# astooke/accel_rl

Measured on AMD Instinct MI355X. Metric: env-steps/sec (whole node), 256-env PPO Atari, higher is better.
Workload: dtype f32; 1 GPU; PPO breakout, 256 envs/GPU, horizon 5, spec-1 CNN (fp32), minibatch 512/GPU x 4 epochs, adam; synthetic fixed-frame emulator; hipGraph rollout; total_envs=256, global_minibatch=512, parallelism=single

## Files before the change

### accel_rl_amd/_build.py

```python
import os
import shutil
import subprocess

PKG_DIR = os.path.dirname(os.path.abspath(__file__))
ROOT = os.path.dirname(PKG_DIR)
CSRC = os.path.join(PKG_DIR, "csrc")
LIB_PATH = os.path.join(PKG_DIR, "libaccel_rl_hip.so")
SOURCES = ["mfma_conv_p1.hip", "mfma_conv_p2.hip", "mfma_conv_p3.hip", "mfma_conv_p4.hip", "mfma_conv_p5.hip", "mfma_conv_p6.hip",
           "mfma_conv_p7.hip", "mfma_conv_p8.hip", "mfma_conv.hip", "img_conv.hip", "batch_ops.hip", "scan.hip", "env.hip", "serve_step.hip", "optim.hip", "learner.hip", "replay.hip",
           "dqn.hip", "lstm.hip", "gru.hip", "noisy.hip", "traj.hip", "handover.hip", "iqn.hip"]
ARCH = "gfx950"


def _flags_stamp():
    return os.path.join(CSRC, "_obj", ".flags")


def _stale():
    if not os.path.exists(LIB_PATH):
        return True
    extra = os.environ.get("ARL_HIPCC_FLAGS", "")
    stamp = _flags_stamp()
    if os.path.exists(stamp) and open(stamp).read().split("||")[-1] != extra:
        return True
    t = os.path.getmtime(LIB_PATH)
    deps = [os.path.join(CSRC, f) for f in os.listdir(CSRC) if f.endswith((".hip", ".h"))]
    deps += [os.path.join(ROOT, "include", h) for h in ("accel_rl_hip.h", "accel_rl_hip_dev.h")]
    return any(os.path.getmtime(d) > t for d in deps)


def build_extension(force=False, verbose=False):
    if not force and not _stale():
        return LIB_PATH
    import fcntl
    lock_path = os.path.join(PKG_DIR, ".build.lock")
    try:
        lock = open(lock_path, "w")
    except PermissionError as e:
        raise RuntimeError("libaccel_rl_hip.so is missing or older than its sources, and %s is not writable: build it "
                           "where the tree can be written (python accel_rl_amd/_build.py)" % PKG_DIR) from e
    with lock:
        fcntl.flock(lock, fcntl.LOCK_EX)
# ... 55 lines not shown
```

### accel_rl_amd/_lib.py

```python
import ctypes as C
import os

import torch

_PKG = os.path.dirname(os.path.abspath(__file__))
LIB_PATH = os.path.join(_PKG, "libaccel_rl_hip.so")

ARL_ABI_VERSION = 4
PROMO_NEP50, PROMO_LEGACY, PROMO_ASSOC = 0, 1, 2
PPO_TIE_THEANO, PPO_TIE_MATH, PPO_TIE_BOTH = 0, 1, 2
OPT_ADAM, OPT_RMSPROP = 0, 1
MAX_ACTIONS = 18
REPLAY_MAX_HORIZON = 16
RAW_H, RAW_W, OBS_H, OBS_W = 210, 160, 104, 80
OPT_PARTIALS = 1024

_vp, _i32, _i64, _f32, _f64 = C.c_void_p, C.c_int32, C.c_int64, C.c_float, C.c_double


class ArlGame(C.Structure):
    _fields_ = [("bank", _vp), ("n_frames", _i32), ("n_actions", _i32),
                ("action_set", _i32 * MAX_ACTIONS), ("start_lives", _i32),
                ("life_period", _i32), ("frame_skip", _i32), ("n_stack", _i32),
                ("clip_reward", _i32), ("episodic_lives", _i32), ("resample_mode", _i32)]
# ... 132 lines not shown
    "arl_pg_head_infer": (_i32, [_vp, _vp, _vp, _i64, _i32, _i32, _vp, _vp, _vp]),
    "arl_pg_head_loss": (_i32, [_vp] * 11 + [_i64, _i32, _i32, _i32, _i32, _f32, _f32, _f32, _i32] + [_vp] * 7),
    "arl_pg_head_loss_parts": (_i32, [_vp] * 11 + [_i64, _i32, _i32, _i32, _i32, _f32, _f32, _f32, _i32] + [_vp] * 7 +
                               [_vp, _i32, _vp]),
    "arl_conv_workspace_bytes": (_i64, []),
    "arl_conv2d_fwd": (_i32, [_vp, _vp, _vp, _vp, C.POINTER(ArlConvGeom), _i32, _vp, _vp]),
    "arl_conv2d_bwd_data": (_i32, [_vp, _vp, _vp, _vp, _vp, C.POINTER(ArlConvGeom), C.POINTER(ArlCorunJob), C.POINTER(_i32), _vp]),
    "arl_conv2d_dgrad_weights": (_i32, [C.POINTER(ArlDgradWt), _i32, _vp]),
    "arl_conv2d_bwd_weight": (_i32, [_vp, _vp, _vp, C.POINTER(ArlConvGeom), _vp, _vp]),
    "arl_conv2d_bwd_weight_parts": (_i32, [_vp, _vp, _vp, C.POINTER(ArlConvGeom), _vp, _i64, C.POINTER(ArlFoldItem),
                                           _vp, C.POINTER(ArlFoldItem), _vp]),
    "arl_fold_many": (_i32, [C.POINTER(ArlFoldItem), _i32, _vp]),
    "arl_conv2d_fwd_parts": (_i32, [_vp, _vp, _vp, _vp, C.POINTER(ArlConvGeom), _i32, _vp, C.POINTER(ArlFoldItem), _vp]),
    "arl_serve_conv1_supported": (_i32, [C.POINTER(ArlGame), C.POINTER(ArlConvGeom)]),
    "arl_rollout_begin_conv1": (_i32, [C.POINTER(ArlGame), C.POINTER(ArlEnvState), C.POINTER(ArlRollout),
                                       C.POINTER(ArlServeConv1), _vp]),
    "arl_env_step_served": (_i32, [C.POINTER(ArlGame), C.POINTER(ArlEnvState), C.POINTER(ArlRollout),
                                   C.POINTER(ArlServeHead), C.POINTER(ArlServeConv1), _vp, _i32, _f64, _f64, _i32, _vp]),
    "arl_conv2d_u8_fwd": (_i32, [_vp, _i64, _vp, _f32, _vp, _vp, _vp, C.POINTER(ArlConvGeom), _i32, _vp]),
    "arl_conv2d_u8_bwd_weight_parts": (_i32, [_vp, _vp, _i64, _vp, _f32, _vp, C.POINTER(ArlConvGeom), _vp, _i64,
                                              C.POINTER(ArlFoldItem), _vp, C.POINTER(ArlFoldItem), _vp]),
    "arl_conv2d_bwd_pair": (_i32, [_vp, _vp, _vp, _vp, _vp, _vp, _vp, C.POINTER(ArlConvGeom), _vp, _i64,
                                   C.POINTER(ArlFoldItem), _vp, C.POINTER(ArlFoldItem), C.POINTER(ArlCorunJob),
                                   C.POINTER(_i32), _vp]),
    "arl_conv2d_bwd_weight_plan": (_i32, [_vp, _vp, _vp, C.POINTER(ArlConvGeom), _vp, _i64, C.POINTER(ArlFoldItem),
                                          _vp, C.POINTER(ArlFoldItem), C.POINTER(ArlWgradPlan)]),
    "arl_conv2d_u8_bwd_weight_plan": (_i32, [_vp, _vp, _i64, _vp, _f32, _vp, C.POINTER(ArlConvGeom), _vp, _i64,
                                             C.POINTER(ArlFoldItem), _vp, C.POINTER(ArlFoldItem),
                                             C.POINTER(ArlWgradPlan)]),
    "arl_conv2d_bwd_pair_plan": (_i32, [_vp, _vp, _vp, _vp, _vp, _vp, _vp, C.POINTER(ArlConvGeom), _vp, _i64,
                                        C.POINTER(ArlFoldItem), _vp, C.POINTER(ArlFoldItem), C.POINTER(ArlCorunJob),
                                        C.POINTER(_i32), C.POINTER(ArlWgradPlan), _vp]),
    "arl_conv2d_bwd_weight_group": (_i32, [C.POINTER(ArlWgradPlan), _i32, _vp]),
    "arl_relu_bwd_bias_parts": (_i32, [_vp, _vp, _i64, _i32, _vp, _vp, C.POINTER(ArlFoldItem), _vp]),
    "arl_replay_append": (_i32, [C.POINTER(ArlReplay), _vp, _vp, _vp, _vp, _i32, _i32, _f64, _i32, _vp]),
    "arl_replay_extract": (_i32, [C.POINTER(ArlReplay), _vp, _vp, _i64, _vp, _vp, _vp, _vp, _vp, _vp]),
    "arl_sumtree_find": (_i32, [_vp, _i32, _vp, _i64, _vp, _vp]),
    "arl_sumtree_add": (_i32, [_vp, _i32, _vp, _vp, _i64, _vp]),
    "arl_sumtree_gather": (_i32, [_vp, _vp, _i64, _f64, _vp, _vp]),
    "arl_sumtree_sample": (_i32, [_vp, _i32, _vp, _i32, _i32, _i32, _vp, _vp, _vp, _vp, _vp, _vp]),
    "arl_sumtree_sample_batch": (_i32, [_vp, _i32, _vp, _i32, _i32, _i32, _vp, _vp, _vp, _vp, _vp, _f64, _vp, _vp, _i32, _vp]),
    "arl_sumtree_update_pow": (_i32, [_vp, _i32, _vp, _vp, _vp, _f64, _i64, _vp]),
    "arl_is_weights": (_i32, [_vp, _i64, _f64, _vp, _vp]),
    "arl_priority_diffs": (_i32, [_vp, _vp, _i64, _f64, _vp, _vp]),
    "arl_catdqn_act": (_i32, [_vp, _vp, _vp, _i64, _i32, _i32, _i32, _i32, _vp, _vp, _vp]),
    "arl_catdqn_loss": (_i32, [_vp] * 8 + [_i64, _i32, _i32, _i32, _i32, _f32, _f32, _f32, _vp, _vp, _vp, _vp]),
    "arl_catdqn_loss_parts": (_i32, [_vp] * 8 + [_i64, _i32, _i32, _i32, _i32, _f32, _f32, _f32, _vp, _vp, _vp, _vp, _i32,
                               _vp]),
    "arl_qrdqn_act": (_i32, [_vp, _vp, _i64, _i32, _i32, _i32, _i32, _vp, _vp, _vp]),
    "arl_qrdqn_loss": (_i32, [_vp] * 7 + [_i64, _i32, _i32, _i32, _i32, _f32, _f32, _vp, _vp, _vp, _vp]),
    "arl_iqn_embed": (_i32, [_vp, _vp, _i64, _i64, _i64, _i32, _vp, _vp, _vp]),
    "arl_iqn_merge_fwd": (_i32, [_vp, _vp, _i64, _i32, _i32, _vp, _vp]),
    "arl_iqn_merge_bwd": (_i32, [_vp, _vp, _vp, _i64, _i32, _i32, _vp, _vp, _vp]),
    "arl_iqn_act": (_i32, [_vp, _vp, _i64, _i32, _i32, _i32, _vp, _vp, _vp, _i64, _vp]),
    "arl_iqn_loss": (_i32, [_vp] * 8 + [_i64, _i32, _i32, _i32, _i32, _f32, _f32, _vp, _vp, _vp, _vp, _i64, _vp]),
    "arl_dqn_act": (_i32, [_vp, _vp, _i64, _i32, _i32, _i32, _vp, _vp, _vp]),
    "arl_dqn_loss": (_i32, [_vp] * 7 + [_i64, _i32, _i32, _i32, _f32, _f32, _vp, _vp, _vp, _vp]),
    "arl_lstm_cell_fwd": (_i32, [_vp, _i64, _vp, _vp, _i64, _i64, _i32, _vp, _i64, _vp, _i64, _vp, _i64, _vp]),
    "arl_lstm_cell_bwd": (_i32, [_vp, _i64, _vp, _vp, _vp, _i64, _vp, _i64, _vp, _i64, _i64, _i32, _vp, _i64, _vp, _vp]),
    "arl_gru_cell_fwd": (_i32, [_vp, _i64, _vp, _vp, _i64, _i64, _i32, _vp, _i64, _vp, _i64, _vp]),
    "arl_gru_cell_bwd": (_i32, [_vp, _i64, _vp, _vp, _vp, _i64, _vp, _i64, _i64, _i32, _vp, _i64, _vp, _i64, _vp, _vp]),
    "arl_rnn_cell_fwd": (_i32, [_vp, _i64, _vp, _i64, _i32, _vp, _i64, _vp]),
    "arl_rnn_cell_bwd": (_i32, [_vp, _i64, _vp, _vp, _i64, _i64, _i32, _vp, _i64, _vp]),
    "arl_seq_handover": (_i32, [_vp, _i64, _vp, _i64, _vp, _vp, _i64, _i64, _i64, _i32, _vp, _vp, _i64, _vp, _i64, _vp]),
    "arl_lstm_cell_bwd_reset": (_i32, [_vp, _i64, _vp, _vp, _vp, _i64, _vp, _i64, _vp, _i64, _i64, _i32, _vp, _i64, _vp,
                                       _vp, _vp, _i64, _i64, _vp]),
# ... 382 lines not shown
    batch, hid = h.shape
    _check(load().arl_pg_head_loss(
        ptr(h), w_head.data_ptr(), b_head.data_ptr(), ptr(actions), ptr(advantages), ptr(returns),
        ptr(old_prob), ptr(valids), ptr(idx), ptr(lr_mult), ptr(inv_count), batch, hid, n_actions,
        kind, int(tie_rule), float(clip_param), float(v_loss_coeff), float(ent_loss_coeff), int(bool(relu_mask_dh)), ptr(dout), ptr(dh),
        dw_head.data_ptr(), db_head.data_ptr(), ptr(loss4), ptr(workspace), stream_ptr(stream)),
        "arl_pg_head_loss")



def conv_geom(batch, in_h, in_w, in_c, out_c, kh, kw, stride, pad_h, pad_w, route=None):
    return ArlConvGeom(batch, in_h, in_w, in_c, out_c, kh, kw, stride, pad_h, pad_w,
                       default_route if route is None else route)


def dense_geom(batch, fan_in, units, route=None):
    return ArlConvGeom(batch, 1, 1, fan_in, units, 1, 1, 1, 0, 0, default_route if route is None else route)


def with_route(geom, route=None):
    g = ArlConvGeom.from_buffer_copy(geom)
    g.route = default_route if route is None else route
    return g


def conv_out_hw(g):
    return ((g.in_h + 2 * g.pad_h - g.kh) // g.stride + 1, (g.in_w + 2 * g.pad_w - g.kw) // g.stride + 1)


def conv_workspace(device):
    return torch.empty(load().arl_conv_workspace_bytes() // 4, dtype=torch.float32, device=device)


def conv2d_fwd(x, w, bias, y, geom, relu, workspace, stream=None):
    for t, n in ((x, "x"), (w, "w"), (y, "y")):
        _want(t, torch.float32, n)
    ho, wo = conv_out_hw(geom)
    assert x.numel() == geom.batch * geom.in_h * geom.in_w * geom.in_c, "x size"
    assert w.numel() == geom.out_c * geom.kh * geom.kw * geom.in_c, "w size"
    assert y.numel() == geom.batch * ho * wo * geom.out_c, "y size"
    _check(load().arl_conv2d_fwd(x.data_ptr(), w.data_ptr(), None if bias is None else bias.data_ptr(),
                                 y.data_ptr(), C.byref(geom), int(bool(relu)), ptr(workspace),
                                 stream_ptr(stream)), "arl_conv2d_fwd")


def conv2d_fwd_parts(x, w, bias, y, geom, relu, workspace, stream=None):
    for t, n in ((x, "x"), (w, "w"), (y, "y")):
        _want(t, torch.float32, n)
    ho, wo = conv_out_hw(geom)
    assert x.numel() == geom.batch * geom.in_h * geom.in_w * geom.in_c, "x size"
    assert w.numel() == geom.out_c * geom.kh * geom.kw * geom.in_c, "w size"
    assert y.numel() == geom.batch * ho * wo * geom.out_c, "y size"
    item = ArlFoldItem()
    _check(load().arl_conv2d_fwd_parts(x.data_ptr(), w.data_ptr(), None if bias is None else bias.data_ptr(),
                                       y.data_ptr(), C.byref(geom), int(bool(relu)), ptr(workspace), C.byref(item),
                                       stream_ptr(stream)), "arl_conv2d_fwd_parts")
    return item


def conv2d_u8_supported(in_h, in_w, out_c, kh, kw, stride, pad_h, pad_w):
    return (pad_h == 0 and pad_w == 0 and stride % 4 == 0 and in_w % 4 == 0 and (in_h * in_w) % 4 == 0 and
            kw in (4, 8, 16) and kh % (16 // kw) == 0 and out_c % 4 == 0 and out_c <= 32)


def _u8_rows(obs, idx, geom):
    _want(obs, torch.uint8, "obs")
    assert obs.is_contiguous() and obs.numel() == obs.shape[0] * geom.in_c * geom.in_h * geom.in_w, "obs shape"
    if idx is not None:
        _want(idx, torch.int32, "idx")
        assert idx.numel() == geom.batch, "idx length"
    else:
        assert obs.shape[0] == geom.batch, "obs rows"


def conv2d_u8_fwd(obs, idx, scale, w, bias, y, geom, relu, stream=None):
    _u8_rows(obs, idx, geom)
    ho, wo = conv_out_hw(geom)
    assert w.numel() == geom.out_c * geom.kh * geom.kw * geom.in_c, "w size"
    assert y.numel() == geom.batch * ho * wo * geom.out_c, "y size"
    _check(load().arl_conv2d_u8_fwd(obs.data_ptr(), obs.shape[0], ptr(idx), float(scale), w.data_ptr(), ptr(bias),
                                    y.data_ptr(), C.byref(geom), int(bool(relu)), stream_ptr(stream)),
           "arl_conv2d_u8_fwd")


def conv2d_dgrad_weights(layers, stream=None):
    assert 0 < len(layers) <= DGRAD_WT_MAX
    items = (ArlDgradWt * len(layers))()
    for it, (w, wt, geom) in zip(items, layers):
        _want(w, torch.float32, "w")
        _want(wt, torch.float32, "wt")
        assert w.numel() == wt.numel() == geom.out_c * geom.kh * geom.kw * geom.in_c, "w / wt size"
        it.w, it.wt, it.geom = ptr(w), ptr(wt), C.pointer(geom)
    _check(load().arl_conv2d_dgrad_weights(items, len(layers), stream_ptr(stream)), "arl_conv2d_dgrad_weights")


def conv2d_bwd_data(dy, w, mask, dx, geom, stream=None, corun=None, wt=None):
    ho, wo = conv_out_hw(geom)
    assert dy.numel() == geom.batch * ho * wo * geom.out_c, "dy size"
    assert dx.numel() == geom.batch * geom.in_h * geom.in_w * geom.in_c, "dx size"
    assert mask is None or mask.numel() == dx.numel()
    taken = _i32(0)
    _check(load().arl_conv2d_bwd_data(dy.data_ptr(), w.data_ptr(), ptr(wt), None if mask is None else mask.data_ptr(),
                                      dx.data_ptr(), C.byref(geom), None if corun is None else C.byref(corun),
                                      C.byref(taken), stream_ptr(stream)), "arl_conv2d_bwd_data")
    return bool(taken.value)


def conv2d_bwd_weight(dy, x, dw, geom, workspace, stream=None):
    ho, wo = conv_out_hw(geom)
    assert dy.numel() == geom.batch * ho * wo * geom.out_c, "dy size"
    assert x.numel() == geom.batch * geom.in_h * geom.in_w * geom.in_c, "x size"
    assert dw.numel() == geom.out_c * geom.kh * geom.kw * geom.in_c, "dw size"
    _check(load().arl_conv2d_bwd_weight(dy.data_ptr(), x.data_ptr(), dw.data_ptr(), C.byref(geom),
                                        ptr(workspace), stream_ptr(stream)), "arl_conv2d_bwd_weight")


class FoldList(object):

    def __init__(self):
        self._items = (ArlFoldItem * FOLD_MAX_ITEMS)()
        self._n = 0
        self._plans = (ArlWgradPlan * WGRAD_GROUP_MAX)()
        self._n_plans = 0
        self.last_dw_in_place = False
        self.corun_taken = False

    def _next(self):
        assert self._n < FOLD_MAX_ITEMS, "too many pending folds"
        self._n += 1
        return C.byref(self._items[self._n - 1])

    def _bias_slot(self, dbias):
        if dbias is None:
            return None, None
# ... 25 lines not shown
        assert dw.numel() == geom.out_c * geom.kh * geom.kw * geom.in_c, "dw size"
        item = self._next()
        pb, ib = self._bias_slot(dbias)
        if defer:
            _check(load().arl_conv2d_bwd_weight_plan(dy.data_ptr(), x.data_ptr(), dw.data_ptr(), C.byref(geom),
                                                     ptr(workspace), workspace.numel() * workspace.element_size(),
                                                     item, pb, ib, self._next_plan(stream)), "arl_conv2d_bwd_weight_plan")
            return self._bias_done(dbias)
        _check(load().arl_conv2d_bwd_weight_parts(dy.data_ptr(), x.data_ptr(), dw.data_ptr(), C.byref(geom),
                                                  ptr(workspace), workspace.numel() * workspace.element_size(),
                                                  item, pb, ib, stream_ptr(stream)), "arl_conv2d_bwd_weight_parts")
        return self._bias_done(dbias)

    def conv2d_u8_bwd_weight(self, dy, obs, idx, scale, dw, geom, workspace, dbias=None, stream=None, defer=False):
        _u8_rows(obs, idx, geom)
        ho, wo = conv_out_hw(geom)
        assert dy.numel() == geom.batch * ho * wo * geom.out_c, "dy size"
        assert dw.numel() == geom.out_c * geom.kh * geom.kw * geom.in_c, "dw size"
        item = self._next()
        pb, ib = self._bias_slot(dbias)
        if defer:
            _check(load().arl_conv2d_u8_bwd_weight_plan(dy.data_ptr(), obs.data_ptr(), obs.shape[0], ptr(idx),
                                                        float(scale), dw.data_ptr(), C.byref(geom), ptr(workspace),
                                                        workspace.numel() * workspace.element_size(), item, pb, ib,
                                                        self._next_plan(stream)), "arl_conv2d_u8_bwd_weight_plan")
            return self._bias_done(dbias)
        _check(load().arl_conv2d_u8_bwd_weight_parts(dy.data_ptr(), obs.data_ptr(), obs.shape[0], ptr(idx),
                                                     float(scale), dw.data_ptr(), C.byref(geom), ptr(workspace),
                                                     workspace.numel() * workspace.element_size(), item, pb, ib,
                                                     stream_ptr(stream)), "arl_conv2d_u8_bwd_weight_parts")
        return self._bias_done(dbias)

    def conv2d_bwd_pair(self, dy, w, mask, dx, x, dw, geom, workspace, dbias=None, stream=None, corun=None, wt=None,
                        defer=False):
        ho, wo = conv_out_hw(geom)
        assert dy.numel() == geom.batch * ho * wo * geom.out_c, "dy size"
        assert x.numel() == dx.numel() == geom.batch * geom.in_h * geom.in_w * geom.in_c, "x / dx size"
        assert dw.numel() == w.numel() == geom.out_c * geom.kh * geom.kw * geom.in_c, "w / dw size"
        item = self._next()
        slot = self._n - 1
        pb, ib = self._bias_slot(dbias)
        taken = _i32(0)
        if defer:
            _check(load().arl_conv2d_bwd_pair_plan(dy.data_ptr(), w.data_ptr(), ptr(wt), ptr(mask), dx.data_ptr(),
                                                   x.data_ptr(), dw.data_ptr(), C.byref(geom), ptr(workspace),
                                                   workspace.numel() * workspace.element_size(), item, pb, ib,
                                                   None if corun is None else C.byref(corun), C.byref(taken),
                                                   self._next_plan(stream), stream_ptr(stream)),
                   "arl_conv2d_bwd_pair_plan")
        else:
            _check(load().arl_conv2d_bwd_pair(dy.data_ptr(), w.data_ptr(), ptr(wt), ptr(mask), dx.data_ptr(), x.data_ptr(),
                                              dw.data_ptr(), C.byref(geom), ptr(workspace),
                                              workspace.numel() * workspace.element_size(), item, pb, ib,
                                              None if corun is None else C.byref(corun), C.byref(taken),
                                              stream_ptr(stream)), "arl_conv2d_bwd_pair")
        self.corun_taken = bool(taken.value)
        self.last_dw_in_place = self._items[slot].splits == 0
        return self._bias_done(dbias)

    def relu_bwd_bias_grad(self, dy, y, rows, channels, dbias, workspace, stream=None):
        _check(load().arl_relu_bwd_bias_parts(dy.data_ptr(), y.data_ptr(), rows, channels, dbias.data_ptr(),
                                              ptr(workspace), self._next(), stream_ptr(stream)),
               "arl_relu_bwd_bias_parts")

    def pg_head_loss(self, h, w_head, b_head, actions, advantages, returns, old_prob, valids, idx, lr_mult,
                     inv_count, n_actions, kind, clip_param, v_loss_coeff, ent_loss_coeff,
                     dout, dh, dw_head, db_head, loss4, workspace, stream=None, relu_mask_dh=False,
                 tie_rule=PPO_TIE_THEANO, dgrad_weights=None):
        batch, hid = h.shape
        assert self._n + 3 <= FOLD_MAX_ITEMS, "too many pending folds"
        first = C.byref(self._items[self._n])
        self._n += 3
        wt_items, n_wt = None, 0
        if dgrad_weights:
            n_wt = len(dgrad_weights)
            assert n_wt <= DGRAD_WT_MAX
# ... 452 lines not shown
```

### accel_rl_amd/csrc/img_conv.hip

```cpp
#include "mfma_conv_impl.h"
#include "img_conv_dev.h"

namespace arlc {

__global__ __launch_bounds__(C1_NT) void conv1_img_kernel(const Conv1ImgArgs a) {
    extern __shared__ __attribute__((aligned(16))) char lds[];
    constexpr int MAXLD = (C1_MAX_IMG / 16 + C1_NT - 1) / C1_NT;
    const int tid = threadIdx.x, lane = tid & 63;
    const int wave = __builtin_amdgcn_readfirstlane(tid >> 6);
    const int half = lane >> 5;
    const int C = a.C, H = a.H, W = a.W, npix = C * H * W, K = C * 64, nsteps = K / 16;
    char* const sW = lds;
    char* const sI = lds + nsteps * 3072;
    const int n16 = npix / 16;
    u32x4 ireg[MAXLD];
    auto img_issue = [&](int img) {
        int row = a.idx ? a.idx[img] : img;
        row = (unsigned)row < (unsigned)a.obs_rows ? row : 0;
        const u32x4* src = reinterpret_cast<const u32x4*>(a.obs + (size_t)row * npix);
#pragma unroll
        for (int i = 0; i < MAXLD; ++i)
            if (tid + C1_NT * i < n16) ireg[i] = src[tid + C1_NT * i];
    };
    auto img_store = [&](int buf, int img) {
// ... 3 lines not shown
            if (tid + C1_NT * i < n16) *reinterpret_cast<u32x4*>(d + (tid + C1_NT * i) * 16) = ireg[i];
        if (a.copy_out) {
            u32x4* o = reinterpret_cast<u32x4*>(a.copy_out + (long long)img * a.copy_stride);
#pragma unroll
            for (int i = 0; i < MAXLD; ++i)
                if (tid + C1_NT * i < n16) o[tid + C1_NT * i] = ireg[i];
        }
    };
    if (a.zero_word && blockIdx.x == 0 && tid == 0) *a.zero_word = 0;
    img_issue(blockIdx.x);
    for (int f = tid; f < nsteps * 64; f += C1_NT) conv1_w_store(sW, f, conv1_w_load(a.w, K, f, a.NF));
    const int rows = a.OH * a.OW, tiles = (rows + 31) / 32;
    float4 bq[4];
    conv1_bias_quads(a.bias, half, bq, a.NF);
    img_store(0, blockIdx.x);
    if (blockIdx.x + gridDim.x < (unsigned)a.n_img) img_issue(blockIdx.x + gridDim.x);
    __syncthreads();
    int buf = 0;
    for (int img = blockIdx.x; img < a.n_img; img += gridDim.x, buf ^= 1) {
        const char* im = sI + buf * npix;
        for (int tp = wave; tp < tiles; tp += C1_NW) conv1_tile(a, im, sW, img, tp, lane, bq);
        if (img + (int)gridDim.x < a.n_img) {
            img_store(buf ^ 1, img + (int)gridDim.x);
            if (img + 2 * (int)gridDim.x < a.n_img) img_issue(img + 2 * gridDim.x);
        }
        __syncthreads();
    }
}

bool g_no_img_kernels = false;

int launch_conv1_img(const unsigned char* obs, int64_t obs_rows, const int32_t* idx, float scale, const float* w, const float* bias, float* y,
                     int64_t batch, int C, int H, int W, int K, int kh, int kw, int stride, int Ho, int Wo, int relu,
                     hipStream_t s, unsigned char* copy_out, long long copy_stride, int* zero_word) {
    const int npix = C * H * W;
    const size_t lds = (size_t)(C * 64 / 16) * 3072 + 2 * (size_t)npix;
    if (g_no_img_kernels || !t_ctx.split || t_ctx.split == 1 || (K != 32 && K != 16) || kh != 8 || kw != 8 || npix % 16 != 0 || npix > C1_MAX_IMG ||
        lds > 160 * 1024 || ((uintptr_t)obs & 15) || (W & 3) || (stride & 3) || batch > 0x7fffffff)
        return -1;
    Conv1ImgArgs a = {obs, idx, w, bias, y, scale, (int)batch, C, H, W, Ho, Wo, stride, relu, K,
                      (int)(obs_rows < 0x7fffffff ? obs_rows : 0x7fffffff), copy_out, copy_stride, zero_word};
    {
        hipError_t e = hipFuncSetAttribute(reinterpret_cast<const void*>(conv1_img_kernel),
                                           hipFuncAttributeMaxDynamicSharedMemorySize, 160 * 1024);
        if (e != hipSuccess) { arl::set_error("hipFuncSetAttribute(conv1_img_kernel): %s", hipGetErrorString(e)); return (int)e; }
    }
    const int cus = 256;
    hipLaunchKernelGGL(conv1_img_kernel, dim3((unsigned)(batch < cus ? batch : cus)), dim3(C1_NT), lds, s, a);
    return arl::check_launch("conv1_img_kernel");
}

int launch_conv1_img_begin(const arl_conv_geom* geom, const unsigned char* obs, int64_t n_img, float scale, const float* w,
                           const float* bias, float* y, int C, int relu, hipStream_t s, unsigned char* copy_out,
                           long long copy_stride, int* zero_word) {
    ARL_ROUTE_SCOPE(geom, nullptr);
    const int st = geom->stride;
    return launch_conv1_img(obs, n_img, nullptr, scale, w, bias, y, n_img, C, geom->in_h, geom->in_w, geom->out_c, geom->kh,
                            geom->kw, st, (geom->in_h - geom->kh) / st + 1, (geom->in_w - geom->kw) / st + 1, relu, s, copy_out,
                            copy_stride, zero_word);
}

}

extern "C" void arl_dev_conv_variant(int32_t v) { arlc::g_no_img_kernels = (v & 1) != 0; }
```

### accel_rl_amd/csrc/img_conv_dev.h

```cpp
#pragma once
#include "mfma_common.h"

namespace arlc {

struct Conv1ImgArgs {
    const unsigned char* obs;
    const int* idx;
    const float* w;
    const float* bias;
    float* y;
    float scale;
    int n_img, C, H, W, OH, OW, stride, relu;
    int NF;
    int obs_rows;
    unsigned char* copy_out;
    long long copy_stride;
    int* zero_word;
};

__device__ __forceinline__ u32x2 bytes_to_bf16x4(unsigned v) {
    const float4 f = bytes_to_f4(v);
    return u32x2{hi_pair(f.x, f.y), hi_pair(f.z, f.w)};
}

struct Conv1WFrag { float4 v0, v1; };
__device__ __forceinline__ Conv1WFrag conv1_w_load(const float* __restrict__ w, const int K, const int f, const int NF = 32) {
    const int s = f >> 6, fl = f & 63;
    if ((fl & 31) >= NF) return Conv1WFrag{make_float4(0.f, 0.f, 0.f, 0.f), make_float4(0.f, 0.f, 0.f, 0.f)};
    const float* src = w + (size_t)(fl & 31) * K + s * 16 + (fl >> 5) * 8;
    return Conv1WFrag{*reinterpret_cast<const float4*>(src), *reinterpret_cast<const float4*>(src + 4)};
}
__device__ __forceinline__ void conv1_w_store(char* sW, const int f, const Conv1WFrag& v) {
    const int s = f >> 6, fl = f & 63;
    unsigned h[4], m[4], l[4];
    split_pair(v.v0.x, v.v0.y, h[0], m[0], l[0]);
    split_pair(v.v0.z, v.v0.w, h[1], m[1], l[1]);
    split_pair(v.v1.x, v.v1.y, h[2], m[2], l[2]);
    split_pair(v.v1.z, v.v1.w, h[3], m[3], l[3]);
    char* d = sW + s * 3072 + fl * 16;
    *reinterpret_cast<u32x4*>(d) = u32x4{h[0], h[1], h[2], h[3]};
    *reinterpret_cast<u32x4*>(d + 1024) = u32x4{m[0], m[1], m[2], m[3]};
    *reinterpret_cast<u32x4*>(d + 2048) = u32x4{l[0], l[1], l[2], l[3]};
}

__device__ __forceinline__ void conv1_bias_quads(const float* __restrict__ bias, const int half, float4 (&bq)[4],
                                                 const int NF = 32) {
#pragma unroll
    for (int q = 0; q < 4; ++q) {
        bq[q] = make_float4(0.f, 0.f, 0.f, 0.f);
        if (bias && 8 * q + 4 * half < NF) bq[q] = *reinterpret_cast<const float4*>(bias + 8 * q + 4 * half);
    }
}

__device__ __forceinline__ void conv1_tile(const Conv1ImgArgs& a, const char* im, const char* sW, const int img,
                                           const int tp, const int lane, const float4 (&bq)[4]) {
    constexpr int KH = 8;
    const int N = a.NF;
    const int l31 = lane & 31, half = lane >> 5;
    const int H = a.H, W = a.W, nsteps = a.C * 64 / 16;
    const int rows = a.OH * a.OW;
    const int m = tp * 32 + l31;
    const int mm = m < rows ? m : 0;
    const int oy = mm / a.OW, ox = mm - oy * a.OW;
    const unsigned off = (unsigned)((oy * a.stride + half) * W + ox * a.stride);
    f32x16 acc;
#pragma unroll
    for (int v = 0; v < 16; ++v) acc[v] = 0.f;
    const char* wl = sW + lane * 16;
#pragma unroll 2
    for (int s = 0; s < nsteps; ++s) {
        const unsigned po = (unsigned)(((s / (KH / 2)) * H + 2 * (s % (KH / 2))) * W);
        u32x4 fb[3];
#pragma unroll
        for (int pl = 0; pl < 3; ++pl) fb[pl] = *reinterpret_cast<const u32x4*>(wl + s * 3072 + pl * 1024);
        const unsigned* q = reinterpret_cast<const unsigned*>(im + po + off);
        const u32x2 lo = bytes_to_bf16x4(q[0]), hi = bytes_to_bf16x4(q[1]);
        const u32x4 fa = u32x4{lo.x, lo.y, hi.x, hi.y};
#pragma unroll
        for (int pl = 2; pl >= 0; --pl) acc = mfma_bf16(fb[pl], fa, acc);
    }
    if (m < rows) {
        float* dst = a.y + ((size_t)img * rows + m) * N + 4 * half;
#pragma unroll
        for (int q = 0; q < 4; ++q) {
            if (8 * q + 4 * half >= N) continue;
            float4 v = make_float4(acc[4 * q] * a.scale + bq[q].x, acc[4 * q + 1] * a.scale + bq[q].y,
                                   acc[4 * q + 2] * a.scale + bq[q].z, acc[4 * q + 3] * a.scale + bq[q].w);
            if (a.relu) { v.x = fmaxf(v.x, 0.f); v.y = fmaxf(v.y, 0.f); v.z = fmaxf(v.z, 0.f); v.w = fmaxf(v.w, 0.f); }
            *reinterpret_cast<float4*>(dst + 8 * q) = v;
        }
    }
}

constexpr int C1_NW = 16, C1_NT = C1_NW * 64, C1_MAX_IMG = 40960;

}
```

### accel_rl_amd/csrc/mfma_common.h

```cpp

#pragma once
#include "arl_optim_dev.h"

#if defined(__HIP_DEVICE_COMPILE__) && !defined(__gfx950__)
#error "accel_rl_amd's MFMA kernels are written for gfx950 (MI355X) only: build with --offload-arch=gfx950"
#endif

#include <stdlib.h>
#include <type_traits>

namespace arlc {

typedef float f32x16 __attribute__((ext_vector_type(16)));
typedef float f32x4 __attribute__((ext_vector_type(4)));

struct GatherDesc {
    const float* src;
    unsigned src_bytes;
    int Hs, Ws, Cs;
    int out_h, out_w;
    int mul, add_y, add_x;
    int taps_x, step;
    int taps_y, rmin, dmin, origin;
    unsigned mg_w, mg_h;
    const unsigned char* src8;
    const int* idx;
    float scale;
    int plane, img_bytes, kh8, kw8;
};

struct WeightDesc {
    const float* w;
    unsigned w_bytes;
    int ld, kc, taps_x, i0, j0, si, kw, c;
    int cls;
};

struct OutDesc {
    float* out;
    const float* bias;
    const float* mask;
    unsigned out_bytes;
    int relu, dense;
    int OH, OW, omul, oadd_y, oadd_x;
};

struct GemmArgs {
    GatherDesc g;
    WeightDesc b;
    OutDesc o;
    int M, N, K;
    int k_per_split;
    int64_t split_stride;
    unsigned long long* trace;
    int n_par;
    int xcd;
    struct Parity {
        int M, out_h, out_w, add_y, add_x, rmin, dmin, origin, i0, j0, oadd_y, oadd_x;
        unsigned src_bytes, mg_w, mg_h;
    } par[4];
};

#define ARL_ARG1(x) asm volatile("" :: "s"(x))
__device__ __forceinline__ void pin_gemm_args(const struct GemmArgs& a);

__device__ __forceinline__ int xcd_chunk(int id, int n) {
    const int q = n >> 3, r = n & 7, x = id & 7, j = id >> 3;
    return (x < r ? x * (q + 1) : r * (q + 1) + (x - r) * q) + j;
}

__device__ __forceinline__ void pin_gemm_args(const GemmArgs& a) {
    asm volatile("" :: "s"(a.g.src), "s"(a.g.src_bytes), "s"(a.g.Hs), "s"(a.g.Ws), "s"(a.g.Cs), "s"(a.g.out_h), "s"(a.g.out_w),
                 "s"(a.g.mul), "s"(a.g.add_y), "s"(a.g.add_x), "s"(a.g.taps_x), "s"(a.g.step), "s"(a.g.taps_y), "s"(a.g.rmin),
                 "s"(a.g.dmin), "s"(a.g.origin), "s"(a.g.mg_w), "s"(a.g.mg_h));
    asm volatile("" :: "s"(a.b.w), "s"(a.b.w_bytes), "s"(a.b.ld), "s"(a.b.kc), "s"(a.b.taps_x), "s"(a.b.i0), "s"(a.b.j0),
                 "s"(a.b.si), "s"(a.b.kw), "s"(a.b.c), "s"(a.b.cls));
    asm volatile("" :: "s"(a.o.out), "s"(a.o.bias), "s"(a.o.mask), "s"(a.o.out_bytes), "s"(a.o.relu), "s"(a.o.dense), "s"(a.o.OH),
// ... 32 lines not shown
                const int rc = i * 32 + (v & 3) + 8 * (v >> 2);
                float val = acc[i][j][v] + bj;
                if (relu) val = fmaxf(val, 0.f);
                if (full || row0 + rc < rows_total)
                    __builtin_amdgcn_raw_buffer_store_b32(__float_as_uint(val), rs, voff, (unsigned)(rc * N) << 2, 0);
            }
    }
}

constexpr unsigned HI16 = 0xffff0000u;
__device__ __forceinline__ unsigned hi_pair(float x0, float x1) {
    return __builtin_amdgcn_perm(__float_as_uint(x1), __float_as_uint(x0), 0x07060302u);
}
__device__ __forceinline__ float lo_part(float x) { return x - __uint_as_float(__float_as_uint(x) & HI16); }
__device__ __forceinline__ void split_pair(float x0, float x1, unsigned& h, unsigned& m, unsigned& l) {
    h = hi_pair(x0, x1);
    const float r0 = lo_part(x0), r1 = lo_part(x1);
    m = hi_pair(r0, r1);
    l = hi_pair(lo_part(r0), lo_part(r1));
}
typedef unsigned int u32x2 __attribute__((ext_vector_type(2)));
typedef __bf16 bf16x2_t __attribute__((ext_vector_type(2)));
typedef float f32x2_t __attribute__((ext_vector_type(2)));
__device__ __forceinline__ unsigned rne_pair(float x0, float x1) {
    const f32x2_t v = {x0, x1};
    return __builtin_bit_cast(unsigned, __builtin_convertvector(v, bf16x2_t));
}
constexpr int planes_of(int split) { return split == 1 ? 1 : 3; }
template <int NP> __device__ __forceinline__ void split_pair_n(float x0, float x1, unsigned& h, unsigned& m, unsigned& l) {
    if constexpr (NP == 1) h = rne_pair(x0, x1);
    else split_pair(x0, x1, h, m, l);
}

template <int TM, int TN, bool SCALED = false>
__device__ __forceinline__ void store_tiles_quads(const f32x16 (&acc)[TM][TN], __amdgpu_buffer_rsrc_t rs,
                                                  const long long (&row_off)[TM], int N, int col_base, int lane,
                                                  const float4 (&bias_q)[TN][4], const float* mask, int relu,
                                                  const float4 (*pre)[TM] = nullptr, float scale = 1.f) {
    const int half = lane >> 5;
#pragma unroll
    for (int j = 0; j < TN; ++j) {
        float4 mk[4][TM];
        if (mask && pre) {
#pragma unroll
            for (int q = 0; q < 4; ++q)
#pragma unroll
                for (int i = 0; i < TM; ++i) mk[q][i] = pre[q][i];
        } else if (mask) {
#pragma unroll
            for (int q = 0; q < 4; ++q)
#pragma unroll
                for (int i = 0; i < TM; ++i) {
                    const int n = col_base + j * 32 + 8 * q + 4 * half;
                    mk[q][i] = make_float4(1.f, 1.f, 1.f, 1.f);
                    if (row_off[i] >= 0 && n < N) mk[q][i] = *reinterpret_cast<const float4*>(mask + row_off[i] + n);
                }
        }
#pragma unroll
        for (int q = 0; q < 4; ++q) {
            const int n = col_base + j * 32 + 8 * q + 4 * half;
            const float4 bq = bias_q[j][q];
#pragma unroll
            for (int i = 0; i < TM; ++i) {
                const bool ok = row_off[i] >= 0 && n < N;
                float4 val = SCALED
                    ? make_float4(acc[i][j][4 * q] * scale + bq.x, acc[i][j][4 * q + 1] * scale + bq.y,
                                  acc[i][j][4 * q + 2] * scale + bq.z, acc[i][j][4 * q + 3] * scale + bq.w)
                    : make_float4(acc[i][j][4 * q] + bq.x, acc[i][j][4 * q + 1] + bq.y,
                                  acc[i][j][4 * q + 2] + bq.z, acc[i][j][4 * q + 3] + bq.w);
                if (relu) { val.x = fmaxf(val.x, 0.f); val.y = fmaxf(val.y, 0.f); val.z = fmaxf(val.z, 0.f); val.w = fmaxf(val.w, 0.f); }
                const unsigned voff = ok ? (unsigned)((row_off[i] + n) << 2) : OOB;
                if (mask) {
                    const float4 m = mk[q][i];
                    if (!(m.x > 0.f)) val.x = 0.f;
                    if (!(m.y > 0.f)) val.y = 0.f;
                    if (!(m.z > 0.f)) val.z = 0.f;
                    if (!(m.w > 0.f)) val.w = 0.f;
                }
                u32x4 raw = {__float_as_uint(val.x), __float_as_uint(val.y), __float_as_uint(val.z), __float_as_uint(val.w)};
                __builtin_amdgcn_raw_buffer_store_b128(raw, rs, voff, 0, 0);
            }
        }
    }
}

struct WgradArgs {
    const float* dy;
    GatherDesc g;
    float* part;
    unsigned dy_bytes;
    int K_out, N, Mred;
    int m_per_split;
    int adv_b, adv_y, adv_x;
    float* bias_part;
    unsigned long long* trace;
    int xcd;
};

__device__ __forceinline__ float4 buf_ld4s(__amdgpu_buffer_rsrc_t rsrc, unsigned voff, unsigned soff) {
    const u32x4 v = __builtin_amdgcn_raw_buffer_load_b128(rsrc, voff, soff, 0);
    return make_float4(__uint_as_float(v.x), __uint_as_float(v.y), __uint_as_float(v.z), __uint_as_float(v.w));
}
__device__ __forceinline__ u32x4 buf_ld4u(__amdgpu_buffer_rsrc_t rsrc, unsigned voff, unsigned soff) {
    return __builtin_amdgcn_raw_buffer_load_b128(rsrc, voff, soff, 0);
}
__device__ __forceinline__ u32x2 buf_ld2s(__amdgpu_buffer_rsrc_t rsrc, unsigned voff, unsigned soff) {
    return __builtin_amdgcn_raw_buffer_load_b64(rsrc, voff, soff, 0);
}
__device__ __forceinline__ unsigned buf_ld1s(__amdgpu_buffer_rsrc_t rsrc, unsigned voff, unsigned soff) {
    return __builtin_amdgcn_raw_buffer_load_b32(rsrc, voff, soff, 0);
}
__device__ __forceinline__ float4 bytes_to_f4(unsigned v) {
    return make_float4((float)(v & 0xffu), (float)((v >> 8) & 0xffu), (float)((v >> 16) & 0xffu), (float)(v >> 24));
// ... 42 lines not shown
```

### accel_rl_amd/csrc/mfma_conv.hip

```cpp
#include "mfma_conv_impl.h"
#include "dgrad_wt_dev.h"

using namespace arlc;

namespace arlc {
thread_local CallCtx t_ctx = {9, nullptr, false};
unsigned long long* g_trace = nullptr;
bool g_force_generic = false;
int g_fwd_tile = -1;
}

namespace {
constexpr int FOLD_WIDE = 128, FOLD_THREADS = 1024;
int g_fold_wide = FOLD_WIDE;
bool g_dgrad_wt = true;

struct FoldSlot { int64_t i; int zg, zgn, row0, o; };
__device__ __forceinline__ FoldSlot fold_slot(int splits, int local_block, int wide_from) {
    FoldSlot f;
    const int tid = threadIdx.x;
    f.o = tid & 15;
    if (splits >= wide_from) { f.zg = tid >> 4; f.zgn = 64; f.row0 = 0; f.i = (int64_t)local_block * 16 + f.o; }
    else {
        const int grp = tid >> 8;
// ... 48 lines not shown
    }
}

struct FoldManyArgs {
    arl_fold_item items[ARL_FOLD_MAX_ITEMS];
    int block_start[ARL_FOLD_MAX_ITEMS + 1];
    int n, wide_from;
};

__global__ __launch_bounds__(FOLD_THREADS) void fold_many_kernel(const FoldManyArgs a) {
    __shared__ float4 lds[64][16];
    int it = 0;
    while (it + 1 < a.n && (int)blockIdx.x >= a.block_start[it + 1]) ++it;
    const float4* part = reinterpret_cast<const float4*>(a.items[it].part);
    float4* out = reinterpret_cast<float4*>(a.items[it].out);
    const int64_t total4 = a.items[it].total >> 2;
    const int splits = a.items[it].splits;
    const FoldSlot f = fold_slot(splits, (int)blockIdx.x - a.block_start[it], a.wide_from);
    const float4 s = fold_sum(part, splits, total4, f, lds);
    const int64_t i = f.i;
    if (f.zg == 0 && i < total4) {
        const int64_t valid = a.items[it].valid;
        if (valid <= 0 || 4 * i + 3 < valid) {
            out[i] = s;
        } else {
            float* o1 = reinterpret_cast<float*>(out + i);
            if (4 * i < valid) o1[0] = s.x;
            if (4 * i + 1 < valid) o1[1] = s.y;
            if (4 * i + 2 < valid) o1[2] = s.z;
        }
    }
}

int launch_fold(const float* part, int splits, int64_t total, const float* bias, int n_bias, int relu,
                float* out, hipStream_t s, const float* mask = nullptr) {
    const int64_t total4 = total >> 2;
    hipLaunchKernelGGL(fold_splits_kernel, dim3((unsigned)fold_blocks(splits, total4)), dim3(FOLD_THREADS), 0, s,
                       (const float4*)part, splits, total4, (const float4*)bias, n_bias >> 2, relu,
                       (const float4*)mask, (float4*)out, g_fold_wide);
    return arl::check_launch("fold_splits_kernel");
}

}

extern "C" int64_t arl_conv_workspace_bytes(void) { return (int64_t)64 << 20; }

extern "C" void arl_dev_conv_trace_buffer(void* device_u64_or_null) { g_trace = (unsigned long long*)device_u64_or_null; }

extern "C" void arl_dev_conv_force_generic(int32_t on) { g_force_generic = on != 0; }

extern "C" void arl_dev_fold_wide_from(int32_t splits) { g_fold_wide = splits > 0 ? splits : FOLD_WIDE; }

extern "C" void arl_dev_fwd_tile(int32_t v) { g_fwd_tile = ((v >= 0 && v <= 2) || v == 6 || v == 7) ? v : -1; }

extern "C" void arl_dev_dgrad_wt(int32_t on) { g_dgrad_wt = on != 0; }

extern "C" int arl_corun_job_init(arl_corun_job* job, const arl_opt_state* opt, int32_t method, float learning_rate,
                                  float avg_factor, float beta1_or_rho, float beta2, float epsilon, int32_t k,
                                  float* step_pp, double* norm_parts, int64_t hole_first, int64_t hole_count) {
    ARL_REQUIRE(job, ARL_E_ARG, "null pointer");
    CorunJob* j = reinterpret_cast<CorunJob*>(job);
    int rc = arl::make_opt_seg(&j->seg, opt, method, learning_rate, avg_factor, beta1_or_rho, beta2, epsilon, k,
                               step_pp, norm_parts, hole_first, hole_count, 1, &j->blocks);
    if (rc) return rc;
    j->host_blocks = 256;
    if (const char* e = getenv("ARL_CORUN_BLOCKS")) j->host_blocks = atoi(e) > 0 ? atoi(e) : 256;
    return 0;
}

extern "C" int arl_corun_job_run(const arl_corun_job* job, void* stream) {
    ARL_REQUIRE(job, ARL_E_ARG, "null pointer");
    const CorunJob* j = reinterpret_cast<const CorunJob*>(job);
    return arl::launch_opt_seg(j->seg, j->blocks, (hipStream_t)stream);
}

namespace {
int fwd_impl(const float* x, const float* w, const float* bias_or_null, float* y, const arl_conv_geom* geom, int32_t relu,
             void* workspace, void* stream, arl_fold_item* parts = nullptr) {
    Geom g;
    int rc = check_geom(geom, &g);
    if (rc) return rc;
    ARL_REQUIRE(x && w && y && workspace, ARL_E_ARG, "null pointer");
    ARL_REQUIRE(arl::aligned16(x) && arl::aligned16(w) && arl::aligned16(y) && arl::aligned16(workspace) &&
                    (!bias_or_null || arl::aligned16(bias_or_null)), ARL_E_ALIGN, "16-byte alignment");
    hipStream_t s = (hipStream_t)stream;
    GemmArgs a = {};
    a.g.src = x; a.g.Hs = g.H; a.g.Ws = g.W; a.g.Cs = g.C; a.g.out_h = g.Ho; a.g.out_w = g.Wo;
    a.g.mul = g.stride; a.g.add_y = -g.pad_h; a.g.add_x = -g.pad_w; a.g.taps_x = g.kw; a.g.step = 1;
    a.M = (int)(g.batch * g.Ho * g.Wo); a.N = g.K; a.K = g.kh * g.kw * g.C;
    a.g.src_bytes = (unsigned)(g.batch * g.H * g.W * g.C * 4);
    a.b.w = w; a.b.ld = a.K; a.b.w_bytes = (unsigned)((int64_t)a.N * a.K * 4);
    a.o.dense = 1; a.trace = g_trace; a.xcd = 1;
    int splits = 1, per = round_up(a.K, BKT);
    const bool small = a.N >= 128 && (int64_t)a.M * a.N <= (int64_t)1 << 20;
    const bool small32 = small && !g_split;
    if (small) plan_split(((a.M + (small32 ? 31 : 63)) / (small32 ? 32 : 64)) * ((a.N + 63) / 64), a.K, &splits, &per, 3 * TARGET_WGS);
    const int tiles128 = ((a.M + 127) / 128) * ((a.N + 127) / 128);
    if (!small && a.N >= 128 && tiles128 * 4 <= TARGET_WGS * 3) plan_split(tiles128, a.K, &splits, &per, TARGET_WGS);
    auto cu_fill = [](int t) { return (double)t / (double)(((t + TARGET_WGS - 1) / TARGET_WGS) * TARGET_WGS); };
    const int tiles64 = ((a.M + 63) / 64) * ((a.N + 63) / 64);
    const bool fill64 = !small && a.N >= 128 && splits == 1 && g_split && g_fwd_tile != 7 &&
                        (g_fwd_tile == 6 || 0.85 * cu_fill(tiles64) > cu_fill(tiles128));
    a.k_per_split = per;
    if (splits > 1) {
        ARL_REQUIRE((int64_t)splits * a.M * a.N * 4 <= arl_conv_workspace_bytes(), ARL_E_RANGE, "workspace too small");
        a.o.out = (float*)workspace; a.split_stride = (int64_t)a.M * a.N;
    } else {
        a.o.out = y; a.o.bias = bias_or_null; a.o.relu = relu;
    }
    constexpr int FBK = 32;
    const bool single_tap = g.C % FBK == 0;
    const bool multi_tap = !single_tap && FBK % g.C == 0 && g.kw % (FBK / g.C) == 0;
    const bool has_pad = g.pad_h > 0 || g.pad_w > 0;
    const bool fast = !g_force_generic && a.K % FBK == 0 && per % FBK == 0 && (single_tap || multi_tap) &&
                      (!has_pad || g.kh * g.kw <= 32) && a.N % 4 == 0;
    if (fast) {
        a.o.out_bytes = (unsigned)((int64_t)a.M * a.N * 4);
        a.g.mg_w = div_magic((int64_t)a.M + 256, a.g.out_w); a.g.mg_h = div_magic((int64_t)a.M + 256, a.g.out_h);
        a.g.taps_y = g.kh; a.g.dmin = 0;
        a.g.rmin = (a.g.add_y * g.W + a.g.add_x) * g.C;
        a.g.origin = a.g.rmin + a.g.dmin;
        a.g.src_bytes = (unsigned)(g.batch * g.H * g.W * g.C * 4 - (int64_t)a.g.origin * 4);
        if (a.N <= 16 && a.K % 16 == 0 && per % 16 == 0 && (g.C % 16 == 0 || (16 % g.C == 0 && g.kw % (16 / g.C) == 0)))
            rc = launch_igemm<4, 1, 2, 1, 16, true, true>(a, splits, multi_tap, has_pad, s);
        else if (g_split && a.N <= 32) rc = launch_igemm_split<4, 1, 1, 1, FBK, true, false, 2>(a, multi_tap, has_pad, s, splits);
        else if (g_split && a.N <= 64) {
            const int v = (g_fwd_tile >= 0 && g_fwd_tile <= 2) ? g_fwd_tile : (2 * ((a.M + 127) / 128) <= TARGET_WGS ? 1 : 0);
            if (v == 1) rc = launch_igemm_split<4, 1, 1, 1, FBK, true, false, 2>(a, multi_tap, has_pad, s, splits);
            else if (v == 2) rc = launch_igemm_split<2, 2, 1, 1, FBK, true, false, 3>(a, multi_tap, has_pad, s, splits);
            else rc = launch_igemm_split<4, 1, 1, 2, FBK, true, false, 2>(a, multi_tap, has_pad, s, splits);
        }
        else if (g_split && (small || fill64)) rc = launch_igemm_split<2, 2, 1, 1, FBK, true, false, 3>(a, multi_tap, has_pad, s, splits);
        else if (g_split) rc = launch_igemm_split<2, 2, 2, 2, FBK, true, false, 1>(a, multi_tap, has_pad, s, splits);
        else if (a.N <= 32 && a.K % 16 == 0 && per % 16 == 0 && (g.C % 16 == 0 || (16 % g.C == 0 && g.kw % (16 / g.C) == 0)))
            rc = launch_igemm<4, 1, 1, 1, 16, true>(a, splits, multi_tap, has_pad, s);
        else if (a.N <= 32) rc = launch_igemm<4, 1, 1, 1, FBK, true>(a, splits, multi_tap, has_pad, s);
        else if (a.N <= 64 && splits == 1) rc = launch_n64<true>(a, multi_tap, has_pad, s);
        else if (a.N <= 64) rc = launch_igemm<2, 2, 1, 1, FBK, true>(a, splits, multi_tap, has_pad, s);
        else if (small32) rc = launch_igemm_occ<1, 4, 2, 1, 32, true, true, 5>(a, multi_tap, has_pad, s, splits);
        else if (small) rc = launch_igemm<2, 2, 1, 1, FBK, true>(a, splits, multi_tap, has_pad, s);
        else rc = launch_igemm<2, 2, 2, 2, FBK, true>(a, splits, multi_tap, has_pad, s);
    } else {
        if (a.N <= 32) rc = launch_rowgather<4, 1, 2, 1, 16, true>(a, splits, s);
        else if (a.N <= 64) rc = launch_rowgather<2, 2, 2, 1, 16, true>(a, splits, s);
        else if (small) rc = launch_rowgather<2, 2, 1, 1, 16, true>(a, splits, s);
        else rc = launch_rowgather<2, 2, 2, 2, 16, true>(a, splits, s);
    }
    if (parts) {
        parts->part = splits == 1 ? y : (const float*)workspace; parts->out = y; parts->total = (int64_t)a.M * a.N;
        parts->splits = splits == 1 ? 0 : splits; parts->valid = 0;
        return rc;
    }
    if (rc || splits == 1) return rc;
    return launch_fold((const float*)workspace, splits, (int64_t)a.M * a.N, bias_or_null, a.N, relu, y, s);
}
}

namespace arlc {
int fold_wide_from() { return g_fold_wide; }
}

extern "C" int arl_conv2d_fwd_parts(const float* x, const float* w, const float* bias_or_null, float* y,
                                    const arl_conv_geom* geom, int32_t relu, void* workspace, arl_fold_item* item,
                                    void* stream) {
    ARL_REQUIRE(item, ARL_E_ARG, "null pointer");
    ARL_ROUTE_SCOPE(geom, nullptr);
    return fwd_impl(x, w, bias_or_null, y, geom, relu, workspace, stream, item);
}

extern "C" int arl_conv2d_fwd(const float* x, const float* w, const float* bias_or_null, float* y,
                              const arl_conv_geom* geom, int32_t relu, void* workspace, void* stream) {
    ARL_ROUTE_SCOPE(geom, nullptr);
    return fwd_impl(x, w, bias_or_null, y, geom, relu, workspace, stream);
}

namespace {
int dgrad_impl(const float* dy, const float* w, const float* mask_or_null, float* dx, const arl_conv_geom* geom,
               DgradPlan* plan_only, void* stream, void* workspace = nullptr, int64_t workspace_bytes = 0,
               const float* wt = nullptr) {
    Geom g;
    int rc = check_geom(geom, &g);
    if (rc) return rc;
    ARL_REQUIRE(dy && w && dx, ARL_E_ARG, "null pointer");
    ARL_REQUIRE(g.kh % g.stride == 0 && g.kw % g.stride == 0, ARL_E_RANGE,
                "data gradient needs kernel size divisible by stride");
    ARL_REQUIRE(arl::aligned16(dy) && arl::aligned16(w) && arl::aligned16(dx) &&
                    (!mask_or_null || arl::aligned16(mask_or_null)) && (!wt || arl::aligned16(wt)), ARL_E_ALIGN,
                "16-byte alignment");
    hipStream_t s = (hipStream_t)stream;
    const int st = g.stride;
    constexpr int FBK = 32;
    const int taps_y = g.kh / st, taps_x = g.kw / st;
    const bool has_pad = !(g.kh == 1 && g.kw == 1 && g.pad_h == 0 && g.pad_w == 0);
    const bool fast = !g_force_generic && g.K % FBK == 0 && taps_y * taps_x <= 32 && st * st <= 4 && g.C % 4 == 0;
    auto describe = [&](int ph, int pw) {
        const int i0 = (ph + g.pad_h) % st, j0 = (pw + g.pad_w) % st;
        GemmArgs a = {};
        a.g.src = dy; a.g.Hs = g.Ho; a.g.Ws = g.Wo; a.g.Cs = g.K;
        a.g.out_h = (g.H - ph + st - 1) / st; a.g.out_w = (g.W - pw + st - 1) / st;
        a.g.mul = 1; a.g.add_y = (ph + g.pad_h - i0) / st; a.g.add_x = (pw + g.pad_w - j0) / st;
        a.g.taps_x = taps_x; a.g.taps_y = taps_y; a.g.step = -1;
        a.M = (int)(g.batch * a.g.out_h * a.g.out_w); a.N = g.C; a.K = taps_y * taps_x * g.K;
        a.g.src_bytes = (unsigned)(g.batch * g.Ho * g.Wo * g.K * 4);
        a.b.w_bytes = (unsigned)((int64_t)g.K * g.kh * g.kw * g.C * 4);
        a.b.w = w; a.b.ld = g.kh * g.kw * g.C; a.b.kc = g.K; a.b.taps_x = taps_x;
        a.b.i0 = i0; a.b.j0 = j0; a.b.si = st; a.b.kw = g.kw; a.b.c = g.C;
        a.o.out = dx; a.o.mask = mask_or_null; a.o.dense = (st == 1);
        a.o.out_bytes = (unsigned)(g.batch * g.H * g.W * g.C * 4);
        a.o.OH = g.H; a.o.OW = g.W; a.o.omul = st; a.o.oadd_y = ph; a.o.oadd_x = pw;
        a.k_per_split = round_up(a.K, BKT);
        a.trace = g_trace; a.xcd = 1;
        if (fast) {
            a.g.rmin = (a.g.add_y * g.Wo + a.g.add_x) * g.K;
            a.g.dmin = -((taps_y - 1) * g.Wo + (taps_x - 1)) * g.K;
            a.g.origin = a.g.rmin + a.g.dmin;
            a.g.src_bytes = (unsigned)(g.batch * g.Ho * g.Wo * g.K * 4 - (int64_t)a.g.origin * 4);
            a.g.mg_w = div_magic((int64_t)a.M + 256, a.g.out_w); a.g.mg_h = div_magic((int64_t)a.M + 256, a.g.out_h);
        }
        return a;
    };
    if (fast) {
        GemmArgs a = describe(0, 0);
        if (st > 1) {
            int n = 0, max_m = 0;
            for (int ph = 0; ph < st && ph < g.H; ++ph)
                for (int pw = 0; pw < st && pw < g.W; ++pw) {
                    const GemmArgs q = describe(ph, pw);
                    GemmArgs::Parity& e = a.par[n++];
                    e.M = q.M; e.out_h = q.g.out_h; e.out_w = q.g.out_w; e.add_y = q.g.add_y; e.add_x = q.g.add_x;
                    e.mg_w = q.g.mg_w; e.mg_h = q.g.mg_h;
                    e.rmin = q.g.rmin; e.dmin = q.g.dmin; e.origin = q.g.origin; e.src_bytes = q.g.src_bytes;
                    e.i0 = q.b.i0; e.j0 = q.b.j0; e.oadd_y = q.o.oadd_y; e.oadd_x = q.o.oadd_x;
                    if (q.M > max_m) max_m = q.M;
                }
            a.n_par = n; a.M = max_m;
            a.xcd = 0;
        }
        const bool small = st == 1 && a.N > 64 && (int64_t)a.M * a.N <= ((int64_t)1 << 20) && a.N % 4 == 0;
        if (plan_only) {
            plan_only->a = a; plan_only->fast = true; plan_only->has_pad = has_pad;
            plan_only->cfg = a.N <= 32 ? 0 : a.N <= 64 ? 1 : small ? 3 : 2;
            return 0;
        }
        if (small) {
            int splits = 1, per = a.k_per_split;
            if (workspace) plan_split(((a.M + 63) / 64) * ((a.N + 63) / 64), a.K, &splits, &per, 3 * TARGET_WGS);
            if ((int64_t)splits * a.M * a.N * 4 > workspace_bytes) { splits = 1; per = round_up(a.K, BKT); }
            a.k_per_split = per;
            if (splits > 1) {
                a.o.out = (float*)workspace; a.o.mask = nullptr; a.split_stride = (int64_t)a.M * a.N;
            }
            if (g_split) rc = launch_igemm_split<2, 2, 1, 1, FBK, false, false, 3>(a, false, has_pad, s, splits);
            else rc = launch_igemm<2, 2, 1, 1, FBK, false>(a, splits, false, has_pad, s);
            if (rc || splits == 1) return rc;
            return launch_fold((const float*)workspace, splits, (int64_t)a.M * a.N, nullptr, 4, 0, dx, s, mask_or_null);
        }
        if (wt && g_split && a.N > 16 && a.N <= 64 && g_dgrad_wt) {
            a.b.w = wt; a.b.ld = a.K; a.b.cls = a.N * a.K;
            const int tiles = ((a.M + 127) / 128) * (a.n_par ? a.n_par : 1);
            const int v = a.N <= 32 || ((g_fwd_tile >= 0 && g_fwd_tile <= 2) ? (g_fwd_tile == 1) : (2 * tiles <= TARGET_WGS));
            if (v) rc = launch_igemm_split<4, 1, 1, 1, FBK, true, false, 2>(a, false, has_pad, s);
            else rc = launch_igemm_split<4, 1, 1, 2, FBK, true, false, 2>(a, false, has_pad, s);
            return rc;
        }
        if (a.N <= 16) rc = launch_igemm<4, 1, 2, 1, 16, false, true>(a, 1, false, has_pad, s);
        else if (g_split && a.N <= 32) rc = launch_igemm_split<4, 1, 1, 1, FBK, false, false, 2>(a, false, has_pad, s);
        else if (g_split && a.N <= 64) {
            const int tiles = ((a.M + 127) / 128) * (a.n_par ? a.n_par : 1);
            const int v = (g_fwd_tile >= 0 && g_fwd_tile <= 2) ? (g_fwd_tile == 1) : (2 * tiles <= TARGET_WGS);
            if (v) rc = launch_igemm_split<4, 1, 1, 1, FBK, false, false, 2>(a, false, has_pad, s);
            else rc = launch_igemm_split<4, 1, 1, 2, FBK, false, false, 2>(a, false, has_pad, s);
        }
        else if (g_split) rc = launch_igemm_split<2, 2, 2, 2, FBK, false, false, 1>(a, false, has_pad, s);
        else if (a.N <= 32 && a.N > 16) rc = launch_igemm_occ<2, 2, 2, 1, 32, false, true, 5>(a, false, has_pad, s);
        else if (a.N <= 32) rc = launch_igemm<4, 1, 1, 1, 16, false>(a, 1, false, has_pad, s);
        else if (a.N <= 64) rc = launch_n64<false>(a, false, has_pad, s);
        else rc = launch_igemm<2, 2, 2, 2, FBK, false>(a, 1, false, has_pad, s);
        return rc;
    }
    if (plan_only) { plan_only->fast = false; return 0; }
    for (int ph = 0; ph < st && ph < g.H; ++ph) {
        for (int pw = 0; pw < st && pw < g.W; ++pw) {
            const GemmArgs a = describe(ph, pw);
            const bool uni = g.K % 16 == 0;
            if (a.N <= 32) rc = uni ? launch_rowgather<4, 1, 2, 1, 16, false, true>(a, 1, s) : launch_rowgather<4, 1, 2, 1, 16, false, false>(a, 1, s);
            else if (a.N <= 64) rc = uni ? launch_rowgather<2, 2, 2, 1, 16, false, true>(a, 1, s) : launch_rowgather<2, 2, 2, 1, 16, false, false>(a, 1, s);
            else rc = uni ? launch_rowgather<2, 2, 2, 2, 16, false, true>(a, 1, s) : launch_rowgather<2, 2, 2, 2, 16, false, false>(a, 1, s);
            if (rc) return rc;
        }
    }
    return 0;
}

int launch_wgrad_plan(const WgradPlan& p, hipStream_t s) {
    constexpr int FBK = 32;
    const WgradArgs& a = p.a;
    const int K = a.K_out, splits = p.splits;
    if (p.kind == WPLAN_U8) {
        if (p.cfg == 1) return launch_wgrad_split<1, 4, 1, 2, FBK, true, 2>(a, splits, false, s);
        if (p.cfg == 2) return launch_wgrad_split<1, 4, 1, 1, FBK, true, 2>(a, splits, false, s);
        const int bm = K <= 16 ? 16 : 32, bn = 128;
        const size_t lds = (size_t)2 * FBK * (bm + bn) * sizeof(float);
        const dim3 grid((a.N + bn - 1) / bn, (K + bm - 1) / bm, splits);
        if (p.cfg == 0) hipLaunchKernelGGL((wgrad_u8_kernel<1, 4, 1, 1, FBK, true>), grid, dim3(256), lds, s, a);
        else hipLaunchKernelGGL((wgrad_u8_kernel<1, 4, 1, 1, FBK, false>), grid, dim3(256), lds, s, a);
        return arl::check_launch("wgrad_u8_kernel");
    }
    if (p.fast) {
        if (K <= 16) return launch_wgrad_fast<1, 4, 1, 1, FBK, true>(a, splits, p.has_pad, s);
        if (g_split && K <= 32) return launch_wgrad_split<1, 4, 1, 1, FBK, false, 2>(a, splits, p.has_pad, s);
        if (g_split && K <= 64) return launch_wgrad_split<2, 2, 1, 1, FBK, false, 2>(a, splits, p.has_pad, s);
        if (g_split) return launch_wgrad_split<2, 2, 2, 2, FBK, false, 1>(a, splits, p.has_pad, s);
        if (K <= 32) return launch_wgrad_fast<1, 4, 1, 1, FBK>(a, splits, p.has_pad, s);
// ... 53 lines not shown
        ARL_REQUIRE((used + (int64_t)splits * a.K_out) * 4 <= workspace_bytes, ARL_E_RANGE, "workspace too small");
        a.bias_part = (float*)workspace + used;
        *bias_part_out = a.bias_part;
    }
    if (fast) {
        a.g.taps_y = g.kh; a.g.dmin = 0;
        a.g.rmin = (a.g.add_y * g.W + a.g.add_x) * g.C;
        a.g.origin = a.g.rmin;
        a.g.src_bytes = (unsigned)(g.batch * g.H * g.W * g.C * 4 - (int64_t)a.g.origin * 4);
        const int img = g.Ho * g.Wo;
        a.adv_b = WG_ROWS / img;
        a.adv_y = (WG_ROWS % img) / g.Wo;
        a.adv_x = (WG_ROWS % img) % g.Wo;
    }
    WgradPlan p = {};
    p.a = a; p.fast = fast; p.has_pad = has_pad; p.cfg = g.K <= 32 ? 0 : g.K <= 64 ? 1 : 2;
    p.splits = splits; p.total = total; p.kind = WPLAN_F32; p.route = g_split;
    *splits_out = splits;
    *total_out = total;
    if (plan_only) { *plan_only = p; return 0; }
    return launch_wgrad_plan(p, s);
}
}

extern "C" int arl_conv2d_bwd_data(const float* dy, const float* w, const float* wt_or_null, const float* mask_or_null,
                                   float* dx, const arl_conv_geom* geom, const arl_corun_job* job_or_null,
                                   int32_t* job_taken_or_null, void* stream) {
    ARL_ROUTE_SCOPE(geom, job_or_null);
    const int rc = dgrad_impl(dy, w, mask_or_null, dx, geom, nullptr, stream, nullptr, 0, wt_or_null);
    if (job_taken_or_null) *job_taken_or_null = t_ctx.corun_taken ? 1 : 0;
    return rc;
}

extern "C" int arl_conv2d_bwd_weight(const float* dy, const float* x, float* dw, const arl_conv_geom* geom,
                                     void* workspace, void* stream) {
    ARL_ROUTE_SCOPE(geom, nullptr);
    int splits = 1;
    int64_t total = 0;
    int rc = wgrad_impl(dy, x, dw, geom, workspace, arl_conv_workspace_bytes(), &splits, &total, nullptr, nullptr, stream);
    if (rc || splits == 1) return rc;
    return launch_fold((const float*)workspace, splits, total, nullptr, 4, 0, dw, (hipStream_t)stream);
}

namespace {
void bias_item(arl_fold_item* item, const float* bias_part, float* dbias, int splits, int channels) {
    item->part = bias_part; item->out = dbias; item->total = channels;
    item->splits = bias_part ? splits : -1;
    item->valid = 0;
}
int wgrad_parts_impl(const float* dy, const float* x, float* dw, const arl_conv_geom* geom,
                     void* workspace, int64_t workspace_bytes, arl_fold_item* item,
                     float* dbias_or_null, arl_fold_item* bias_item_or_null, void* stream,
                     WgradPlan* plan_only = nullptr) {
    ARL_REQUIRE(item && (!dbias_or_null || bias_item_or_null), ARL_E_ARG, "null pointer");
    ARL_REQUIRE(!dbias_or_null || arl::aligned16(dbias_or_null), ARL_E_ALIGN, "16-byte alignment");
    int splits = 1;
    int64_t total = 0;
    float* bias_part = nullptr;
    int rc = wgrad_impl(dy, x, dw, geom, workspace, workspace_bytes, &splits, &total,
                        dbias_or_null ? &bias_part : nullptr, plan_only, stream);
    item->part = (const float*)workspace; item->out = dw; item->total = total;
    item->splits = splits > 1 ? splits : 0;
    item->valid = 0;
    if (dbias_or_null) bias_item(bias_item_or_null, bias_part, dbias_or_null, splits, geom->out_c);
    return rc;
}
// ... 18 lines not shown
                            reinterpret_cast<WgradPlan*>(plan));
}

namespace {
struct U8Geom { int H, W, C, K, kh, kw, stride, Ho, Wo; int64_t batch; };

int check_u8(const uint8_t* obs, int64_t obs_rows, const arl_conv_geom* g, U8Geom* o) {
    ARL_REQUIRE(obs && g && obs_rows > 0, ARL_E_ARG, "null pointer");
    ARL_REQUIRE(g->batch > 0 && g->in_h > 0 && g->in_w > 0 && g->in_c > 0 && g->out_c > 0 && g->kh > 0 && g->kw > 0 &&
                    g->stride > 0, ARL_E_ARG, "conv: bad geometry");
    const int cpr = g->kw / 4;
    ARL_REQUIRE(g->pad_h == 0 && g->pad_w == 0 && g->stride % 4 == 0 && g->in_w % 4 == 0 &&
                    (g->in_h * g->in_w) % 4 == 0 && (g->kw == 4 || g->kw == 8 || g->kw == 16) && g->kh % (4 / cpr) == 0 &&
                    g->out_c % 4 == 0 && g->out_c <= 32 && ((uintptr_t)obs & 3) == 0,
                ARL_E_RANGE, "u8 conv: needs pad 0, stride % 4 == 0, width % 4 == 0, kw in {4, 8, 16}, <= 32 filters");
    o->H = g->in_h; o->W = g->in_w; o->C = g->in_c; o->K = g->out_c; o->kh = g->kh; o->kw = g->kw; o->stride = g->stride;
    o->Ho = (g->in_h - g->kh) / g->stride + 1; o->Wo = (g->in_w - g->kw) / g->stride + 1; o->batch = g->batch;
    const int64_t lim = (int64_t)OOB / 4;
    ARL_REQUIRE(o->Ho > 0 && o->Wo > 0 && g->batch * (int64_t)o->Ho * o->Wo * g->out_c < lim &&
                    obs_rows * (int64_t)g->in_c * g->in_h * g->in_w < (int64_t)OOB,
                ARL_E_RANGE, "conv: tensor larger than the 32-bit buffer offsets address");
    return 0;
}

void fill_u8(GatherDesc* d, const uint8_t* obs, int64_t obs_rows, const int32_t* idx, float scale, const U8Geom& g) {
    d->src8 = obs; d->idx = idx; d->scale = scale;
    d->plane = g.H * g.W; d->img_bytes = g.C * g.H * g.W; d->kh8 = g.kh; d->kw8 = g.kw;
    d->src_bytes = (unsigned)(obs_rows * d->img_bytes);
    d->Hs = g.H; d->Ws = g.W; d->Cs = 1; d->out_h = g.Ho; d->out_w = g.Wo;
    d->mul = g.stride; d->add_y = 0; d->add_x = 0; d->taps_x = g.kw; d->taps_y = g.kh; d->step = 1;
}
}

extern "C" int arl_conv2d_u8_fwd(const uint8_t* obs, int64_t obs_rows, const int32_t* idx_or_null, float scale,
                                 const float* w, const float* bias_or_null, float* y, const arl_conv_geom* geom,
                                 int32_t relu, void* stream) {
    ARL_REQUIRE(w && y, ARL_E_ARG, "null pointer");
    U8Geom g;
    int rc = check_u8(obs, obs_rows, geom, &g);
    if (rc) return rc;
    ARL_ROUTE_SCOPE(geom, nullptr);
    ARL_REQUIRE(arl::aligned16(w) && arl::aligned16(y) && (!bias_or_null || arl::aligned16(bias_or_null)), ARL_E_ALIGN,
                "16-byte alignment");
    if (!g_trace) {
        rc = launch_conv1_img(obs, obs_rows, idx_or_null, scale, w, bias_or_null, y, g.batch, g.C, g.H, g.W, g.K, g.kh, g.kw, g.stride,
                              g.Ho, g.Wo, relu, (hipStream_t)stream);
        if (rc >= 0) return rc;
    }
    GemmArgs a = {};
    fill_u8(&a.g, obs, obs_rows, idx_or_null, scale, g);
    a.M = (int)(g.batch * g.Ho * g.Wo); a.N = g.K; a.K = g.C * g.kh * g.kw;
    a.b.w = w; a.b.ld = a.K; a.b.w_bytes = (unsigned)((int64_t)a.N * a.K * 4);
    a.o.dense = 1; a.o.out = y; a.o.bias = bias_or_null; a.o.relu = relu;
    a.o.out_bytes = (unsigned)((int64_t)a.M * a.N * 4);
    a.k_per_split = a.K;
    a.g.mg_w = div_magic((int64_t)a.M + 256, a.g.out_w); a.g.mg_h = div_magic((int64_t)a.M + 256, a.g.out_h);
    a.trace = g_trace; a.xcd = 1;
    constexpr int BK = 16, BM = 128;
    const dim3 grid((a.M + BM - 1) / BM, 1, 1);
    if (a.N <= 16) {
        const size_t lds = (size_t)2 * (BM * (BK + 4) + 16 * (BK + 4)) * sizeof(float);
        hipLaunchKernelGGL((igemm_u8_kernel<4, 1, 2, 1, BK, true>), grid, dim3(256), lds, (hipStream_t)stream, a);
    } else if (g_split && g.kh % (8 / (g.kw >> 2)) == 0) {
        return launch_igemm_split<4, 1, 2, 1, 32, true, true, 2>(a, false, false, (hipStream_t)stream);
    } else if (g.kh % (8 / (g.kw >> 2)) == 0) {
        constexpr int PBM = 64, PBK = 32;
        const dim3 pgrid((a.M + PBM - 1) / PBM, 1, 1);
        const arl::OptSeg none = {};
        const size_t lds = (size_t)2 * (PBM * (PBK + 4) + 32 * (PBK + 4)) * sizeof(float);
        hipLaunchKernelGGL((igemm_occ_kernel<2, 2, 2, 1, PBK, true, false, false, true, 5, false, true>), pgrid, dim3(256),
                           lds, (hipStream_t)stream, a, none);
        return arl::check_launch("igemm_occ_kernel (u8)");
    } else {
        const size_t lds = (size_t)2 * (BM * (BK + 4) + 32 * (BK + 4)) * sizeof(float);
        hipLaunchKernelGGL((igemm_u8_kernel<4, 1, 1, 1, BK, false>), grid, dim3(256), lds, (hipStream_t)stream, a);
    }
    return arl::check_launch("igemm_u8_kernel");
}

namespace {
int wgrad_u8_impl(const float* dy, const uint8_t* obs, int64_t obs_rows, const int32_t* idx_or_null, float scale, float* dw,
                  const arl_conv_geom* geom, void* workspace, int64_t workspace_bytes, arl_fold_item* item,
                  float* dbias_or_null, arl_fold_item* bias_item_or_null, WgradPlan* plan_only, void* stream) {
    ARL_REQUIRE(dy && dw && workspace && item && (!dbias_or_null || bias_item_or_null), ARL_E_ARG, "null pointer");
    U8Geom g;
    int rc = check_u8(obs, obs_rows, geom, &g);
    if (rc) return rc;
    ARL_ROUTE_SCOPE(geom, nullptr);
    ARL_REQUIRE(arl::aligned16(dy) && arl::aligned16(dw) && arl::aligned16(workspace) &&
                    (!dbias_or_null || arl::aligned16(dbias_or_null)), ARL_E_ALIGN, "16-byte alignment");
    WgradArgs a = {};
    a.dy = dy;
    fill_u8(&a.g, obs, obs_rows, idx_or_null, scale, g);
    a.K_out = g.K; a.N = g.C * g.kh * g.kw; a.Mred = (int)(g.batch * g.Ho * g.Wo);
    a.dy_bytes = (unsigned)((int64_t)a.Mred * g.K * 4);
    a.trace = g_trace; a.xcd = 1;
    const bool wide = g.K > 16 && g_split && g.kw % 8 == 0 && a.N % 256 == 0;
    const int bm = g.K <= 16 ? 16 : 32, bn = wide ? 256 : 128;
    const int tiles = ((a.K_out + bm - 1) / bm) * ((a.N + bn - 1) / bn);
    int splits, per;
    plan_split(tiles, a.Mred, &splits, &per, (g.K <= 16 ? 4 : 2) * TARGET_WGS);
    a.m_per_split = per;
    const int64_t total = (int64_t)a.K_out * a.N;
    const int64_t used = splits > 1 ? (int64_t)splits * total : 0;
    ARL_REQUIRE((used + (int64_t)splits * a.K_out) * 4 <= workspace_bytes, ARL_E_RANGE, "workspace too small");
    a.part = splits > 1 ? (float*)workspace : dw;
    if (dbias_or_null) a.bias_part = (float*)workspace + used;
    const int img = g.Ho * g.Wo;
    a.adv_b = WG_ROWS / img; a.adv_y = (WG_ROWS % img) / g.Wo; a.adv_x = (WG_ROWS % img) % g.Wo;
    WgradPlan p = {};
// ... 4 lines not shown
    item->splits = splits > 1 ? splits : 0;
    item->valid = 0;
    if (dbias_or_null) bias_item(bias_item_or_null, a.bias_part, dbias_or_null, splits, g.K);
    if (plan_only) { *plan_only = p; return 0; }
    return launch_wgrad_plan(p, (hipStream_t)stream);
}
}

extern "C" int arl_conv2d_u8_bwd_weight_parts(const float* dy, const uint8_t* obs, int64_t obs_rows,
                                              const int32_t* idx_or_null, float scale, float* dw,
                                              const arl_conv_geom* geom, void* workspace, int64_t workspace_bytes,
                                              arl_fold_item* item, float* dbias_or_null,
                                              arl_fold_item* bias_item_or_null, void* stream) {
    return wgrad_u8_impl(dy, obs, obs_rows, idx_or_null, scale, dw, geom, workspace, workspace_bytes, item, dbias_or_null,
                         bias_item_or_null, nullptr, stream);
}

extern "C" int arl_conv2d_u8_bwd_weight_plan(const float* dy, const uint8_t* obs, int64_t obs_rows,
                                             const int32_t* idx_or_null, float scale, float* dw,
                                             const arl_conv_geom* geom, void* workspace, int64_t workspace_bytes,
                                             arl_fold_item* item, float* dbias_or_null,
                                             arl_fold_item* bias_item_or_null, arl_wgrad_plan* plan) {
    ARL_REQUIRE(plan, ARL_E_ARG, "null pointer");
    *plan = arl_wgrad_plan{};
    return wgrad_u8_impl(dy, obs, obs_rows, idx_or_null, scale, dw, geom, workspace, workspace_bytes, item, dbias_or_null,
                         bias_item_or_null, reinterpret_cast<WgradPlan*>(plan), nullptr);
}


namespace {
int pair_impl(const float* dy, const float* w, const float* wt_or_null, const float* mask_or_null, float* dx, const float* x,
              float* dw, const arl_conv_geom* geom, void* workspace, int64_t workspace_bytes, arl_fold_item* item,
              float* dbias_or_null, arl_fold_item* bias_item_or_null, const arl_corun_job* job_or_null,
              int32_t* job_taken_or_null, WgradPlan* defer, void* stream) {
    ARL_REQUIRE(item && geom && (!dbias_or_null || bias_item_or_null), ARL_E_ARG, "null pointer");
    if (job_taken_or_null) *job_taken_or_null = 0;
    ARL_ROUTE_SCOPE(geom, job_or_null);
    ARL_REQUIRE(!dbias_or_null || arl::aligned16(dbias_or_null), ARL_E_ALIGN, "16-byte alignment");
    DgradPlan dp = {};
    WgradPlan wp = {};
    int splits = 1;
    int64_t total = 0;
    float* bias_part = nullptr;
    int rc = dgrad_impl(dy, w, mask_or_null, dx, geom, &dp, stream);
    if (rc) return rc;
    rc = wgrad_impl(dy, x, dw, geom, workspace, workspace_bytes, &splits, &total,
                    dbias_or_null ? &bias_part : nullptr, &wp, stream);
    if (rc) return rc;
    const bool has_pad = dp.has_pad || wp.has_pad;
    const int64_t dgrad_tiles = (int64_t)((dp.a.M + 127) / 128) * ((dp.a.N + 127) / 128) * (dp.a.n_par ? dp.a.n_par : 1);
    const bool paired = dp.fast && wp.fast && dp.cfg == 2 && wp.cfg == 2 && dgrad_tiles <= 2 * TARGET_WGS &&
                        (!has_pad || geom->kh * geom->kw <= 32) && !g_trace;
    if (!paired) {
        const int64_t half = (workspace_bytes / 2) & ~(int64_t)15;
        rc = dgrad_impl(dy, w, mask_or_null, dx, geom, nullptr, stream, (char*)workspace + half, workspace_bytes - half,
                        wt_or_null);
        if (job_taken_or_null) *job_taken_or_null = t_ctx.corun_taken ? 1 : 0;
        if (rc) return rc;
        return wgrad_parts_impl(dy, x, dw, geom, workspace, half, item, dbias_or_null, bias_item_or_null, stream, defer);
    }
    hipStream_t s = (hipStream_t)stream;
    if (g_split) rc = launch_pair<2, 2, 2, 2, 2, 2, 2, 2, 16>(dp, wp, has_pad, s);
    else rc = launch_pair<2, 2, 2, 2, 2, 2, 2, 2>(dp, wp, has_pad, s);
    item->part = (const float*)workspace; item->out = dw; item->total = wp.total;
    item->splits = wp.splits > 1 ? wp.splits : 0;
    item->valid = 0;
    if (dbias_or_null) bias_item(bias_item_or_null, bias_part, dbias_or_null, wp.splits, geom->out_c);
    return rc;
}
}

extern "C" int arl_conv2d_bwd_pair(const float* dy, const float* w, const float* wt_or_null, const float* mask_or_null,
                                   float* dx, const float* x, float* dw, const arl_conv_geom* geom, void* workspace,
                                   int64_t workspace_bytes, arl_fold_item* item, float* dbias_or_null,
                                   arl_fold_item* bias_item_or_null, const arl_corun_job* job_or_null,
                                   int32_t* job_taken_or_null, void* stream) {
    return pair_impl(dy, w, wt_or_null, mask_or_null, dx, x, dw, geom, workspace, workspace_bytes, item, dbias_or_null,
                     bias_item_or_null, job_or_null, job_taken_or_null, nullptr, stream);
}

extern "C" int arl_conv2d_bwd_pair_plan(const float* dy, const float* w, const float* wt_or_null, const float* mask_or_null,
                                        float* dx, const float* x, float* dw, const arl_conv_geom* geom, void* workspace,
                                        int64_t workspace_bytes, arl_fold_item* item, float* dbias_or_null,
                                        arl_fold_item* bias_item_or_null, const arl_corun_job* job_or_null,
                                        int32_t* job_taken_or_null, arl_wgrad_plan* plan, void* stream) {
    ARL_REQUIRE(plan, ARL_E_ARG, "null pointer");
    *plan = arl_wgrad_plan{};
    return pair_impl(dy, w, wt_or_null, mask_or_null, dx, x, dw, geom, workspace, workspace_bytes, item, dbias_or_null,
                     bias_item_or_null, job_or_null, job_taken_or_null, reinterpret_cast<WgradPlan*>(plan), stream);
}

extern "C" int arl_conv2d_bwd_weight_group(const arl_wgrad_plan* plans, int32_t n, void* stream) {
    ARL_REQUIRE(plans || n == 0, ARL_E_ARG, "null pointer");
    ARL_REQUIRE(n >= 0 && n <= ARL_WGRAD_GROUP_MAX, ARL_E_RANGE, "0 .. ARL_WGRAD_GROUP_MAX plans");
    hipStream_t s = (hipStream_t)stream;
    const WgradPlan* pl[ARL_WGRAD_GROUP_MAX];
    for (int i = 0; i < n; ++i) pl[i] = reinterpret_cast<const WgradPlan*>(&plans[i]);
    auto body_of = [](const WgradPlan& p) {
        if (!p.route || g_trace) return -1;
        if (p.kind == WPLAN_U8) return p.cfg == 1 ? 2 : p.cfg == 2 ? 3 : -1;
        return p.kind == WPLAN_F32 && p.fast && p.cfg == 1 ? (p.has_pad ? 1 : 0) : -1;
    };
    int route = 0, n_el = 0, el[ARL_WGRAD_GROUP_MAX];
    for (int i = 0; i < n; ++i) {
        if (pl[i]->kind != WPLAN_F32 && pl[i]->kind != WPLAN_U8) continue;
        if (body_of(*pl[i]) >= 0 && !route) route = pl[i]->route;
        if (body_of(*pl[i]) >= 0 && pl[i]->route == route) el[n_el++] = i;
    }
    for (int i = 0; i < n; ++i) {
        if (pl[i]->kind != WPLAN_F32 && pl[i]->kind != WPLAN_U8) continue;
        bool grouped = false;
        for (int k = 0; k < n_el; ++k) grouped = grouped || el[k] == i;
        if (grouped && n_el > 1) continue;
        const CallScope scope(pl[i]->route);
        const int rc = launch_wgrad_plan(*pl[i], s);
        if (rc) return rc;
    }
    if (n_el < 2) return 0;
    for (int i = 1; i < n_el; ++i)
        for (int k = i; k > 0 && group_blocks(*pl[el[k]]) > group_blocks(*pl[el[k - 1]]); --k) std::swap(el[k], el[k - 1]);
    WgradGroupArgs g = {};
    size_t lds = 0;
// ... 87 lines not shown
```

### accel_rl_amd/csrc/mfma_dispatch.h

```cpp
#pragma once
#include "mfma_generic.h"
#include "mfma_igemm.h"
#include "mfma_wgrad.h"
#include "mfma_pair.h"

namespace arlc {

template <int WGM, int WGN, int TM, int TN, int BK, bool B_KC, bool TAP_UNIFORM = false>
int launch_rowgather(const GemmArgs& a, int splits, hipStream_t s) {
    constexpr int BM = WGM * TM * 32, BN = WGN * TN * 32;
    constexpr int A_SZ = BM * (BK + 4), B_SZ = B_KC ? BN * (BK + 4) : BK * BN;
    const size_t lds = (size_t)2 * (A_SZ + B_SZ) * sizeof(float);
    dim3 grid((a.M + BM - 1) / BM, (a.N + BN - 1) / BN, splits);
    hipLaunchKernelGGL((rowgather_gemm_kernel<WGM, WGN, TM, TN, BK, B_KC, TAP_UNIFORM>), grid, dim3(256), lds, s, a);
    return arl::check_launch("rowgather_gemm_kernel");
}

template <int WGM, int WGN, int TM, int TN, int BK>
int launch_wgrad(const WgradArgs& a, int splits, hipStream_t s) {
    constexpr int BM = WGM * TM * 32, BN = WGN * TN * 32;
    const size_t lds = (size_t)2 * BK * (BM + BN) * sizeof(float);
    dim3 grid((a.N + BN - 1) / BN, (a.K_out + BM - 1) / BM, splits);
    hipLaunchKernelGGL((wgrad_kernel<WGM, WGN, TM, TN, BK>), grid, dim3(256), lds, s, a);
    return arl::check_launch("wgrad_kernel");
// ... 60 lines not shown
}

template <int WGM, int WGN, int TM, int TN, int BK, bool B_KC, bool N16, int MINW>
int launch_igemm_occ(const GemmArgs& a, bool multi_tap, bool has_pad, hipStream_t s, int splits = 1) {
    constexpr int BM = WGM * TM * (N16 ? 16 : 32), BN = N16 ? WGN * 16 : WGN * TN * 32;
    constexpr int A_SZ = BM * (BK + 4), B_SZ = B_KC ? BN * (BK + 4) : BK * (N16 ? BN + 4 : BN);
    const size_t lds = (size_t)2 * (A_SZ + B_SZ) * sizeof(float);
    static_assert(lds_fits(2 * (A_SZ + B_SZ)), "<= 64 KiB of LDS");
    dim3 grid((a.M + BM - 1) / BM, (a.N + BN - 1) / BN, a.n_par ? a.n_par : splits);
    arl::OptSeg c = {};
    if constexpr (!B_KC) {
        if (!multi_tap && corun_take(&c, &grid)) {
            if (has_pad) hipLaunchKernelGGL((igemm_occ_kernel<WGM, WGN, TM, TN, BK, B_KC, false, true, N16, MINW, true>), grid, dim3(256), lds, s, a, c);
            else hipLaunchKernelGGL((igemm_occ_kernel<WGM, WGN, TM, TN, BK, B_KC, false, false, N16, MINW, true>), grid, dim3(256), lds, s, a, c);
            return arl::check_launch("igemm_occ_kernel (co-run)");
        }
    }
#define ARL_IGEMM_OCC(MT, HP) \
    hipLaunchKernelGGL((igemm_occ_kernel<WGM, WGN, TM, TN, BK, B_KC, MT, HP, N16, MINW>), grid, dim3(256), lds, s, a, c)
    if (multi_tap && has_pad) ARL_IGEMM_OCC(true, true);
    else if (multi_tap) ARL_IGEMM_OCC(true, false);
    else if (has_pad) ARL_IGEMM_OCC(false, true);
    else ARL_IGEMM_OCC(false, false);
#undef ARL_IGEMM_OCC
    return arl::check_launch("igemm_occ_kernel");
}

#ifdef ARL_NO_SPLIT6
#define ARL_BY_MODE(X1, X6, X9) do { X9; } while (0)
#else
#define ARL_BY_MODE(X1, X6, X9) do { if (g_split == 1) { X1; } else if (g_split == 6) { X6; } else { X9; } } while (0)
#endif

template <int WGM, int WGN, int TM, int TN, int BK, bool B_KC, bool U8, int MINW>
int launch_igemm_split(const GemmArgs& a, bool multi_tap, bool has_pad, hipStream_t s, int splits = 1) {
    constexpr int BM = WGM * TM * 32, BN = WGN * TN * 32;
    const int npl = planes_of(g_split);
    const size_t lds = (size_t)2 * ((U8 ? 1 : npl) * BM + npl * BN) * BK * 2;
    const size_t lds_dir = (size_t)2 * npl * BN * BK * 2;
    (void)lds_dir;
    dim3 grid((a.M + BM - 1) / BM, (a.N + BN - 1) / BN, a.n_par ? a.n_par : splits);
    arl::OptSeg c = {};
    int rc = 0;
#define ARL_SPLIT_K(MT, HP, SPL, CO, AD)                                                                   \
    do {                                                                                                   \
        auto k = igemm_split_kernel<WGM, WGN, TM, TN, BK, B_KC, MT, HP, U8, SPL, MINW, CO, AD>;            \
        const size_t lds_k = (AD) ? lds_dir : lds;                                                         \
        rc = allow_big_lds(k, lds_k + (CO ? 64 : 0));                                                      \
        if (!rc) hipLaunchKernelGGL(k, grid, dim3(256), lds_k, s, a, c);                                   \
    } while (0)
#define ARL_SPLIT_PIN(MT, HP, SPL, CO)                                                                     \
    do {                                                                                                   \
        constexpr bool AD = WGN == 1 && (U8 || !(MT));                                                     \
        ARL_SPLIT_K(MT, HP, SPL, CO, AD);                                                                  \
    } while (0)
#define ARL_SPLIT_MODE(MT, HP, CO)                                                                         \
    do {                                                                                                   \
        ARL_BY_MODE(ARL_SPLIT_PIN(MT, HP, 1, CO), ARL_SPLIT_PIN(MT, HP, 6, CO), ARL_SPLIT_PIN(MT, HP, 9, CO));                           \
    } while (0)
    if constexpr (U8) {
        ARL_SPLIT_MODE(false, false, false);
    } else {
        if constexpr (!B_KC || (WGM == 4 && WGN == 1 && TM == 1)) {
            if (!multi_tap && corun_take(&c, &grid)) {
                if (has_pad) ARL_SPLIT_MODE(false, true, true); else ARL_SPLIT_MODE(false, false, true);
                return rc ? rc : arl::check_launch("igemm_split_kernel (co-run)");
            }
        }
        if (multi_tap && has_pad) ARL_SPLIT_MODE(true, true, false);
        else if (multi_tap) ARL_SPLIT_MODE(true, false, false);
        else if (has_pad) ARL_SPLIT_MODE(false, true, false);
        else ARL_SPLIT_MODE(false, false, false);
    }
#undef ARL_SPLIT_PIN
#undef ARL_SPLIT_MODE
#undef ARL_SPLIT_K
    return rc ? rc : arl::check_launch("igemm_split_kernel");
}

template <int WGM, int WGN, int TM, int TN, int BK, bool M16 = false>
int launch_wgrad_fast(const WgradArgs& a, int splits, bool has_pad, hipStream_t s) {
    constexpr int BM = M16 ? 16 : WGM * TM * 32, BN = WGN * TN * 32;
    const size_t lds = (size_t)2 * BK * (BM + BN) * sizeof(float);
    dim3 grid((a.N + BN - 1) / BN, (a.K_out + BM - 1) / BM, splits);
    int rc;
    if (has_pad) {
        auto k = wgrad_fast_kernel<WGM, WGN, TM, TN, BK, true, M16>;
        rc = allow_big_lds(k, lds + 4096);
        if (!rc) hipLaunchKernelGGL(k, grid, dim3(256), lds, s, a);
    } else {
        auto k = wgrad_fast_kernel<WGM, WGN, TM, TN, BK, false, M16>;
        rc = allow_big_lds(k, lds + 4096);
        if (!rc) hipLaunchKernelGGL(k, grid, dim3(256), lds, s, a);
    }
    return rc ? rc : arl::check_launch("wgrad_fast_kernel");
}

template <int WGM, int WGN, int TM, int TN, int BK, bool U8, int MINW>
int launch_wgrad_split(const WgradArgs& a, int splits, bool has_pad, hipStream_t s) {
    constexpr int BM = WGM * TM * 32, BN = WGN * TN * 32;
    const int npl = planes_of(g_split);
    const size_t lds = (size_t)2 * (npl * BM + (U8 ? 1 : npl) * BN) * BK * 2;
    dim3 grid((a.N + BN - 1) / BN, (a.K_out + BM - 1) / BM, splits);
    int rc = 0;
#define ARL_WSPLIT(HP, SPL)                                                                                \
// ... 44 lines not shown
        g->batch * (int64_t)g->in_h * g->in_w * g->in_c >= lim ||
        (int64_t)g->out_c * g->kh * g->kw * g->in_c >= lim) {
        arl::set_error("conv: tensor larger than the 2 GiB the 32-bit buffer offsets address");
        return ARL_E_RANGE;
    }
    return 0;
}

inline int round_up(int x, int q) { return (x + q - 1) / q * q; }

inline unsigned div_magic(int64_t rows, int d) {
    if (d <= 1 || rows * (int64_t)d >= ((int64_t)1 << 32)) return 0;
    return (unsigned)((((uint64_t)1 << 32) + (uint64_t)d - 1) / (uint64_t)d);
}

template <bool B_KC>
int launch_n64(const GemmArgs& a, bool multi_tap, bool has_pad, hipStream_t s) {
    return launch_igemm_occ<1, 4, 2, 1, 32, B_KC, true, 5>(a, multi_tap, has_pad, s);
}

inline void plan_split(int tiles, int red, int* splits, int* per, int want = TARGET_WGS) {
    int s = tiles >= want ? 1 : want / tiles;
    const int max_s = (red + 4 * BKT - 1) / (4 * BKT);
    if (s > max_s) s = max_s;
    if (s < 1) s = 1;
    *per = round_up((red + s - 1) / s, BKT);
    *splits = (red + *per - 1) / *per;
}

struct DgradPlan { GemmArgs a; bool fast, has_pad; int cfg; };
constexpr int WPLAN_F32 = 1, WPLAN_U8 = 2;
struct WgradPlan { WgradArgs a; bool fast, has_pad; int cfg, splits; int64_t total; int kind, route; };

template <int DWGM, int DWGN, int DTM, int DTN, int WWGM, int WWGN, int WTM, int WTN, int BK = 32>
int launch_pair(const DgradPlan& d, const WgradPlan& w, bool has_pad, hipStream_t s) {
    constexpr int DBM = DWGM * DTM * 32, DBN = DWGN * DTN * 32, WBM = WWGM * WTM * 32, WBN = WWGN * WTN * 32;
    const size_t lds_d = (size_t)2 * (DBM * (BK + 4) + BK * DBN) * sizeof(float);
    const size_t lds_w = (size_t)2 * BK * (WBM + WBN) * sizeof(float);
    const size_t lds = lds_d > lds_w ? lds_d : lds_w;
    const int dgx = (d.a.M + DBM - 1) / DBM, dgy = (d.a.N + DBN - 1) / DBN, dgz = d.a.n_par ? d.a.n_par : 1;
    const int wgx = (w.a.N + WBN - 1) / WBN, wgy = (w.a.K_out + WBM - 1) / WBM, wgz = w.splits;
    const int n_ig = dgx * dgy * dgz, n_wg = wgx * wgy * wgz;
    int rc;
    if (g_split) {
        const size_t lds_s = (size_t)2 * planes_of(g_split) * ((DBM + DBN) > (WBM + WBN) ? (DBM + DBN) : (WBM + WBN)) * BK * 2;
#define ARL_PSPLIT(HP, SPL)                                                                                \
    do {                                                                                                   \
        auto k = bwd_pair_kernel<DWGM, DWGN, DTM, DTN, WWGM, WWGN, WTM, WTN, BK, HP, SPL>;                 \
        rc = allow_big_lds(k, lds_s + 4096);                                                               \
        if (!rc) hipLaunchKernelGGL(k, dim3(n_ig + n_wg), dim3(256), lds_s, s, d.a, w.a, dgx, dgy, n_ig, wgx, wgy); \
    } while (0)
        if (has_pad) ARL_BY_MODE(ARL_PSPLIT(true, 1), ARL_PSPLIT(true, 6), ARL_PSPLIT(true, 9));
        else ARL_BY_MODE(ARL_PSPLIT(false, 1), ARL_PSPLIT(false, 6), ARL_PSPLIT(false, 9));
#undef ARL_PSPLIT
    } else if (has_pad) {
        auto k = bwd_pair_kernel<DWGM, DWGN, DTM, DTN, WWGM, WWGN, WTM, WTN, BK, true>;
        rc = allow_big_lds(k, lds + 4096);
        if (!rc) hipLaunchKernelGGL(k, dim3(n_ig + n_wg), dim3(256), lds, s, d.a, w.a, dgx, dgy, n_ig, wgx, wgy);
    } else {
        auto k = bwd_pair_kernel<DWGM, DWGN, DTM, DTN, WWGM, WWGN, WTM, WTN, BK, false>;
        rc = allow_big_lds(k, lds + 4096);
        if (!rc) hipLaunchKernelGGL(k, dim3(n_ig + n_wg), dim3(256), lds, s, d.a, w.a, dgx, dgy, n_ig, wgx, wgy);
    }
    return rc ? rc : arl::check_launch("bwd_pair_kernel");
}


int launch_conv1_img(const unsigned char* obs, int64_t obs_rows, const int32_t* idx, float scale, const float* w, const float* bias, float* y,
                     int64_t batch, int C, int H, int W, int K, int kh, int kw, int stride, int Ho, int Wo, int relu,
                     hipStream_t s, unsigned char* copy_out = nullptr, long long copy_stride = 0, int* zero_word = nullptr);

#define ARL_GA const GemmArgs&, bool, bool, hipStream_t, int
#define ARL_P1(T) \
    T int launch_igemm_split<4, 1, 2, 1, 32, true, true, 2>(ARL_GA); \
    T int launch_igemm_split<4, 1, 1, 2, 32, true, false, 2>(ARL_GA); \
    T int launch_igemm_split<4, 1, 1, 1, 32, true, false, 2>(ARL_GA);
#define ARL_P2(T) \
    T int launch_igemm_split<2, 2, 2, 2, 32, true, false, 1>(ARL_GA); \
    T int launch_igemm_split<2, 2, 1, 1, 32, true, false, 3>(ARL_GA); \
    T int launch_igemm_split<2, 2, 1, 1, 32, false, false, 3>(ARL_GA);
#define ARL_P3(T) \
    T int launch_igemm_split<4, 1, 1, 2, 32, false, false, 2>(ARL_GA); \
    T int launch_igemm_split<4, 1, 1, 1, 32, false, false, 2>(ARL_GA); \
    T int launch_igemm_split<2, 2, 2, 2, 32, false, false, 1>(ARL_GA);
#define ARL_P4(T) \
    T int launch_wgrad_split<2, 2, 2, 2, 32, false, 1>(const WgradArgs&, int, bool, hipStream_t); \
    T int launch_wgrad_split<2, 2, 1, 1, 32, false, 2>(const WgradArgs&, int, bool, hipStream_t); \
    T int launch_wgrad_split<1, 4, 1, 1, 32, false, 2>(const WgradArgs&, int, bool, hipStream_t); \
    T int launch_wgrad_split<1, 4, 1, 1, 32, true, 2>(const WgradArgs&, int, bool, hipStream_t); \
    T int launch_wgrad_split<1, 4, 1, 2, 32, true, 2>(const WgradArgs&, int, bool, hipStream_t);
#define ARL_P5(T) \
    T int launch_pair<2, 2, 2, 2, 2, 2, 2, 2, 32>(const DgradPlan&, const WgradPlan&, bool, hipStream_t); \
    T int launch_pair<2, 2, 2, 2, 2, 2, 2, 2, 16>(const DgradPlan&, const WgradPlan&, bool, hipStream_t);
#define ARL_P6(T) \
    T int launch_igemm<2, 2, 1, 1, 32, true, false>(const GemmArgs&, int, bool, bool, hipStream_t); \
    T int launch_igemm<2, 2, 1, 1, 32, false, false>(const GemmArgs&, int, bool, bool, hipStream_t); \
    T int launch_igemm<2, 2, 2, 2, 32, true, false>(const GemmArgs&, int, bool, bool, hipStream_t); \
    T int launch_igemm<2, 2, 2, 2, 32, false, false>(const GemmArgs&, int, bool, bool, hipStream_t); \
    T int launch_igemm<4, 1, 2, 1, 16, true, true>(const GemmArgs&, int, bool, bool, hipStream_t); \
    T int launch_igemm<4, 1, 2, 1, 16, false, true>(const GemmArgs&, int, bool, bool, hipStream_t); \
    T int launch_igemm<4, 1, 1, 1, 32, true, false>(const GemmArgs&, int, bool, bool, hipStream_t); \
    T int launch_igemm<4, 1, 1, 1, 16, true, false>(const GemmArgs&, int, bool, bool, hipStream_t); \
    T int launch_igemm<4, 1, 1, 1, 16, false, false>(const GemmArgs&, int, bool, bool, hipStream_t);
#define ARL_P7(T) \
    T int launch_igemm_occ<2, 2, 2, 1, 32, false, true, 5>(ARL_GA); \
    T int launch_igemm_occ<1, 4, 2, 1, 32, true, true, 5>(ARL_GA); \
    T int launch_igemm_occ<1, 4, 2, 1, 32, false, true, 5>(ARL_GA); \
    T int launch_wgrad_fast<2, 2, 2, 2, 32, false>(const WgradArgs&, int, bool, hipStream_t); \
    T int launch_wgrad_fast<2, 2, 1, 1, 32, false>(const WgradArgs&, int, bool, hipStream_t); \
    T int launch_wgrad_fast<1, 4, 1, 1, 32, false>(const WgradArgs&, int, bool, hipStream_t); \
    T int launch_wgrad_fast<1, 4, 1, 1, 32, true>(const WgradArgs&, int, bool, hipStream_t);
#ifndef ARL_CONV_PART
#define ARL_CONV_PART 0
#endif
int launch_wgrad_group(const WgradGroupArgs& g, int groups, size_t lds, hipStream_t s);
#if ARL_CONV_PART == 8
int launch_wgrad_group(const WgradGroupArgs& g, int groups, size_t lds, hipStream_t s) {
    int rc = 0;
#define ARL_WGROUP(SPL)                                                                                    \
    do {                                                                                                   \
        auto k = wgrad_group_kernel<SPL>;                                                                  \
        rc = allow_big_lds(k, lds + 4096);                                                                 \
        if (!rc) hipLaunchKernelGGL(k, dim3((unsigned)groups * 8), dim3(256), lds, s, g);                  \
    } while (0)
    ARL_BY_MODE(ARL_WGROUP(1), ARL_WGROUP(6), ARL_WGROUP(9));
#undef ARL_WGROUP
    return rc ? rc : arl::check_launch("wgrad_group_kernel");
}
#endif
#define ARL_T_DEF template
#define ARL_T_EXT extern template
#if ARL_CONV_PART == 1
ARL_P1(ARL_T_DEF)
#else
ARL_P1(ARL_T_EXT)
#endif
#if ARL_CONV_PART == 2
ARL_P2(ARL_T_DEF)
#else
ARL_P2(ARL_T_EXT)
#endif
#if ARL_CONV_PART == 3
ARL_P3(ARL_T_DEF)
#else
ARL_P3(ARL_T_EXT)
#endif
#if ARL_CONV_PART == 4
ARL_P4(ARL_T_DEF)
#else
ARL_P4(ARL_T_EXT)
#endif
#if ARL_CONV_PART == 5
ARL_P5(ARL_T_DEF)
#else
ARL_P5(ARL_T_EXT)
#endif
#if ARL_CONV_PART == 6
ARL_P6(ARL_T_DEF)
#else
ARL_P6(ARL_T_EXT)
#endif
#if ARL_CONV_PART == 7
ARL_P7(ARL_T_DEF)
#else
ARL_P7(ARL_T_EXT)
#endif

}
```

### accel_rl_amd/csrc/mfma_igemm.h

```cpp
#pragma once
#include "mfma_common.h"

namespace arlc {

template <int WGM, int WGN, int TM, int TN, int BK, bool B_KC, bool MULTI_TAP, bool HAS_PAD, bool N16 = false,
          bool U8 = false, int SPLIT = 0, bool ADIR = false>
__device__ __forceinline__ void igemm_body(const GemmArgs& a, const int bx, const int by, const int bz, float* smem) {
    constexpr bool SP = SPLIT != 0;
    static_assert(!ADIR || (SP && WGN == 1 && !MULTI_TAP), "direct operand: split kernels, one wave per row tile");
    constexpr int MT = N16 ? 16 : 32;
    constexpr int BM = WGM * TM * MT, BN = N16 ? WGN * 16 : WGN * TN * 32, CH = BK / 4;
    constexpr int LDA = BK + 4;
    constexpr int LDB = B_KC ? BK + 4 : (N16 ? BN + 4 : BN);
    static_assert(!N16 || (TN == 1 && BK % 16 == 0), "16-wide tiles: one column tile per wave");
    static_assert(!SP || (!N16 && BK % 16 == 0), "split products: 32-wide tiles, two LDS stages");
    constexpr int ROWS_PER_PASS = 256 / CH;
    constexpr int RA = (BM + ROWS_PER_PASS - 1) / ROWS_PER_PASS;
    constexpr int A_SZ = BM * LDA, B_SZ = B_KC ? BN * LDB : BK * LDB;
    constexpr int NST = 2;
    constexpr int NB4 = B_KC ? BN * CH : BK * BN / 4;
    constexpr int NPAIR = (BK / 2) * (BN / 4);
    constexpr int RB = (SP && !B_KC) ? 2 * ((NPAIR + 255) / 256) : (NB4 + 255) / 256;
    static_assert(WGM * WGN == 4 && BK % 8 == 0, "tile shape");
    float* sA = smem;
    float* sB = smem + NST * A_SZ;
    constexpr int PA = U8 ? 1 : planes_of(SPLIT), PB = planes_of(SPLIT), ROWB = BK * 2, NS = BK / 8;
    constexpr int LPA = ADIR ? 0 : PA;
    constexpr int SPA = BM * ROWB, SPB = BN * ROWB, STAGE = LPA * SPA + PB * SPB;
    char* const sS = reinterpret_cast<char*>(smem);

    const int tid = threadIdx.x, lane = tid & 63, wave = tid >> 6;
    const int wm = wave / WGN, wn = wave % WGN;
    const int l31 = lane & 31, half = lane >> 5;
    const int m0 = bx * BM, n0 = by * BN;
    GatherDesc g = a.g;
    int M = a.M, w_i0 = a.b.i0, w_j0 = a.b.j0, oadd_y = a.o.oadd_y, oadd_x = a.o.oadd_x;
    if (a.n_par) {
        const GemmArgs::Parity& q = a.par[bz];
        M = q.M; g.out_h = q.out_h; g.out_w = q.out_w; g.add_y = q.add_y; g.add_x = q.add_x;
        g.mg_w = q.mg_w; g.mg_h = q.mg_h;
        g.rmin = q.rmin; g.dmin = q.dmin; g.origin = q.origin; g.src_bytes = q.src_bytes;
        w_i0 = q.i0; w_j0 = q.j0; oadd_y = q.oadd_y; oadd_x = q.oadd_x;
        if (m0 >= M) return;
    }
    const int kbeg = a.n_par ? 0 : bz * a.k_per_split;
    const int kend = (kbeg + a.k_per_split < a.K) ? kbeg + a.k_per_split : a.K;
    const int Cs = g.Cs, taps_x = g.taps_x, Ws = g.Ws, step = g.step;
// ... 299 lines not shown
#pragma unroll
            for (int v = 0; v < 16; ++v) acc[i][j][v] = 0.f;
#pragma unroll
        for (int v = 0; v < 4; ++v) acc16[i][v] = 0.f;
    }

    float4 bias_q[TN][4];
#pragma unroll
    for (int j = 0; j < TN; ++j)
#pragma unroll
        for (int q = 0; q < 4; ++q) {
            const int n = N16 ? n0 + wn * 16 + 4 * quad : n0 + wn * TN * 32 + j * 32 + 8 * q + 4 * half;
            bias_q[j][q] = make_float4(0.f, 0.f, 0.f, 0.f);
            if (a.o.bias && n < a.N && (!N16 || q == 0)) bias_q[j][q] = *reinterpret_cast<const float4*>(a.o.bias + n);
        }
    long long row_off[TM];
    auto decode_out_rows = [&]() {
#pragma unroll
        for (int i = 0; i < TM; ++i) {
            const int m = m0 + (wm * TM + i) * MT + (N16 ? l15 : l31);
            if (a.o.dense) {
                row_off[i] = m < M ? (long long)m * a.N : -1;
            } else {
                const int t = div_u(m, g.out_w, g.mg_w), ox = m - t * g.out_w;
                const int b = div_u(t, g.out_h, g.mg_h), oy = t - b * g.out_h;
                row_off[i] = m < M ? ((long long)(b * a.o.OH + oy * a.o.omul + oadd_y) * a.o.OW + ox * a.o.omul + oadd_x) * a.N
                                   : -1;
            }
        }
    };
    constexpr bool PRE_MASK = TN == 1 && TM <= 2;
    if (PRE_MASK) decode_out_rows();
    float4 mk_pre[4][TM];
    auto issue_mask_loads = [&]() {
        if (!(PRE_MASK && a.o.mask)) return;
#pragma unroll
        for (int q = 0; q < (N16 ? 1 : 4); ++q)
#pragma unroll
            for (int i = 0; i < TM; ++i) {
                const int n = N16 ? n0 + wn * 16 + 4 * quad : n0 + wn * TN * 32 + 8 * q + 4 * half;
                mk_pre[q][i] = make_float4(1.f, 1.f, 1.f, 1.f);
                if (row_off[i] >= 0 && n < a.N) mk_pre[q][i] = *reinterpret_cast<const float4*>(a.o.mask + row_off[i] + n);
            }
    };
    const int nk = (kend - kbeg) / BK;
    constexpr int STEPS = (N16 || SP) ? BK / 16 : BK / 8;
    auto mfma_steps = [&](auto buf_c, auto lo_c, auto hi_c) {
        constexpr int buf = decltype(buf_c)::value, LO = decltype(lo_c)::value, HI = decltype(hi_c)::value;
        if constexpr (SP) {
            const char* cA = sS + buf * STAGE + (wm * TM * 32) * ROWB + l31 * ROWB;
            const char* cB = sS + buf * STAGE + LPA * SPA + (B_KC ? (wn * TN * 32) * ROWB + l31 * ROWB
                                                                  : (half * 4 * BN + wn * TN * 32 + l31) * 4);
            const int swz = kc_swz<NS>(l31);
#pragma unroll
            for (int ks = LO; ks < HI; ++ks) {
                const int slot = ((2 * ks + half) ^ swz) << 4;
                u32x4 fa[TM][3], fb[TN][3];
#pragma unroll
                for (int i = 0; i < TM; ++i)
#pragma unroll
                    for (int pl = 0; pl < PA; ++pl) {
                        if constexpr (ADIR) fa[i][pl] = fd_[buf][i][ks][pl];
                        else fa[i][pl] = *reinterpret_cast<const u32x4*>(cA + pl * SPA + i * 32 * ROWB + slot);
                    }
#pragma unroll
                for (int j = 0; j < TN; ++j)
#pragma unroll
// ... 167 lines not shown
            k_tile(C1{}, kt + 1);
        }
    }
    }

    if (a.trace) tr2 = __builtin_readcyclecounter();
    float* out = a.o.out + (a.n_par ? 0 : (int64_t)bz * a.split_stride);
    {
        const __amdgpu_buffer_rsrc_t rsO = make_rsrc(out, a.o.out_bytes);
        if (!PRE_MASK) decode_out_rows();
        if constexpr (N16) {
            const int n = n0 + wn * 16 + 4 * quad;
            const float4 bq = bias_q[0][0];
#pragma unroll
            for (int i = 0; i < TM; ++i) {
                const bool ok = row_off[i] >= 0 && n < a.N;
                float4 val = U8 ? make_float4(acc16[i][0] * g.scale + bq.x, acc16[i][1] * g.scale + bq.y,
                                              acc16[i][2] * g.scale + bq.z, acc16[i][3] * g.scale + bq.w)
                                : make_float4(acc16[i][0] + bq.x, acc16[i][1] + bq.y, acc16[i][2] + bq.z, acc16[i][3] + bq.w);
                if (a.o.relu) { val.x = fmaxf(val.x, 0.f); val.y = fmaxf(val.y, 0.f); val.z = fmaxf(val.z, 0.f); val.w = fmaxf(val.w, 0.f); }
                if (a.o.mask) {
                    float4 mk = make_float4(1.f, 1.f, 1.f, 1.f);
                    if (PRE_MASK) mk = mk_pre[0][i < TM ? i : 0];
                    else if (ok) mk = *reinterpret_cast<const float4*>(a.o.mask + row_off[i] + n);
                    if (!(mk.x > 0.f)) val.x = 0.f;
                    if (!(mk.y > 0.f)) val.y = 0.f;
                    if (!(mk.z > 0.f)) val.z = 0.f;
                    if (!(mk.w > 0.f)) val.w = 0.f;
                }
                u32x4 raw = {__float_as_uint(val.x), __float_as_uint(val.y), __float_as_uint(val.z), __float_as_uint(val.w)};
                __builtin_amdgcn_raw_buffer_store_b128(raw, rsO, ok ? (unsigned)((row_off[i] + n) << 2) : OOB, 0, 0);
            }
        } else {
            store_tiles_quads<TM, TN, U8>(acc, rsO, row_off, a.N, n0 + wn * TN * 32, lane, bias_q, a.o.mask, a.o.relu,
                                          PRE_MASK ? mk_pre : nullptr, g.scale);
        }
    }
    if (a.trace && tid == 0) {
        unsigned long long* t = a.trace + ((size_t)(bz * gridDim.y + by) * gridDim.x + bx) * 8;
        t[0] = tr0; t[1] = tr1; t[2] = tr2; t[3] = __builtin_readcyclecounter();
        t[4] = rt0; t[5] = __builtin_amdgcn_s_memrealtime();
#ifdef ARL_PROLOGUE_STAMPS
        if constexpr (SP) { t[6] = st_a; t[7] = st_b; }
        else
#endif
        {
        t[6] = __builtin_amdgcn_s_getreg((31 << 11) | 4);
        t[7] = __builtin_amdgcn_s_getreg((31 << 11) | 20);
        }
    }
}

template <int WGM, int WGN, int TM, int TN, int BK, bool B_KC, bool MULTI_TAP, bool HAS_PAD, bool N16 = false>
__global__ __launch_bounds__(256) void igemm_kernel(const GemmArgs a) {
    extern __shared__ __attribute__((aligned(16))) float smem[];
    igemm_body<WGM, WGN, TM, TN, BK, B_KC, MULTI_TAP, HAS_PAD, N16>(a, blockIdx.x, blockIdx.y, blockIdx.z, smem);
}

template <int WGM, int WGN, int TM, int TN, int BK, bool B_KC, bool MULTI_TAP, bool HAS_PAD, bool U8, int SPLIT, int MINW,
          bool CORUN = false, bool ADIR = false>
__global__ __launch_bounds__(256, MINW) void igemm_split_kernel(const GemmArgs a, const arl::OptSeg c) {
    extern __shared__ __attribute__((aligned(16))) float smem[];
    pin_gemm_args(a);
    int bx = blockIdx.x;
    if constexpr (CORUN) {
        if (bx < c.co_blocks) {
            __shared__ double lds[8];
            if (blockIdx.y || blockIdx.z) return;
            if (c.method == ARL_OPT_ADAM) arl::opt_update_block<ARL_OPT_ADAM>(c, bx, c.co_blocks, lds);
            else arl::opt_update_block<ARL_OPT_RMSPROP>(c, bx, c.co_blocks, lds);
            return;
        }
        bx -= c.co_blocks;
    }
    int by = blockIdx.y, bz = blockIdx.z;
    if (!CORUN && a.xcd) {
        const int gx = gridDim.x, gy = gridDim.y;
        const int t = xcd_chunk((bz * gy + by) * gx + bx, gx * gy * (int)gridDim.z);
        bx = t % gx;
        const int u = t / gx;
        by = u % gy; bz = u / gy;
    }
    igemm_body<WGM, WGN, TM, TN, BK, B_KC, MULTI_TAP, HAS_PAD, false, U8, SPLIT, ADIR>(a, bx, by, bz, smem);
}

template <int WGM, int WGN, int TM, int TN, int BK, bool B_KC, bool MULTI_TAP, bool HAS_PAD, bool N16, int MINW, bool CORUN = false,
          bool U8 = false>
__global__ __launch_bounds__(256, MINW) void igemm_occ_kernel(const GemmArgs a, const arl::OptSeg c) {
    extern __shared__ __attribute__((aligned(16))) float smem[];
    if constexpr (CORUN) {
        if ((int)blockIdx.x < c.co_blocks) {
            __shared__ double lds[8];
            if (blockIdx.y || blockIdx.z) return;
            if (c.method == ARL_OPT_ADAM) arl::opt_update_block<ARL_OPT_ADAM>(c, (int)blockIdx.x, c.co_blocks, lds);
            else arl::opt_update_block<ARL_OPT_RMSPROP>(c, (int)blockIdx.x, c.co_blocks, lds);
            return;
        }
        igemm_body<WGM, WGN, TM, TN, BK, B_KC, MULTI_TAP, HAS_PAD, N16, U8>(a, blockIdx.x - c.co_blocks, blockIdx.y, blockIdx.z, smem);
        return;
    }
    igemm_body<WGM, WGN, TM, TN, BK, B_KC, MULTI_TAP, HAS_PAD, N16, U8>(a, blockIdx.x, blockIdx.y, blockIdx.z, smem);
}

template <int WGM, int WGN, int TM, int TN, int BK, bool N16>
__global__ __launch_bounds__(256) void igemm_u8_kernel(const GemmArgs a) {
    extern __shared__ __attribute__((aligned(16))) float smem[];
    igemm_body<WGM, WGN, TM, TN, BK, true, false, false, N16, true>(a, blockIdx.x, blockIdx.y, blockIdx.z, smem);
}

}
```

### accel_rl_amd/csrc/mfma_pair.h

```cpp
#pragma once
#include "mfma_igemm.h"
#include "mfma_wgrad.h"

namespace arlc {

template <int DWGM, int DWGN, int DTM, int DTN, int WWGM, int WWGN, int WTM, int WTN, int BK, bool HAS_PAD, int SPLIT = 0>
__global__ __launch_bounds__(256) void bwd_pair_kernel(const GemmArgs a, const WgradArgs w, const int dgx, const int dgy,
                                                       const int n_ig, const int wgx, const int wgy) {
    extern __shared__ __attribute__((aligned(16))) float smem[];
    int id = blockIdx.x;
    if (a.xcd) id = xcd_chunk(id, (int)gridDim.x);
    if (id < n_ig) {
        const int bx = id % dgx, t = id / dgx;
        igemm_body<DWGM, DWGN, DTM, DTN, BK, false, false, HAS_PAD, false, false, SPLIT>(a, bx, t % dgy, t / dgy, smem);
    } else {
        id -= n_ig;
        if (a.xcd) {
            const int by = id % wgy, t = id / wgy;
            wgrad_fast_body<WWGM, WWGN, WTM, WTN, BK, HAS_PAD, false, false, SPLIT>(w, t % wgx, by, t / wgx, smem);
        } else {
            const int bx = id % wgx, t = id / wgx;
            wgrad_fast_body<WWGM, WWGN, WTM, WTN, BK, HAS_PAD, false, false, SPLIT>(w, bx, t % wgy, t / wgy, smem);
        }
    }
}

}
```

### accel_rl_amd/policies/atari_cnn_policy.py

```python
import ctypes as C
import os

import numpy as np
import torch

from accel_rl_amd import _lib
from accel_rl_amd.distributions import Categorical
from accel_rl_amd.spaces import Discrete
from accel_rl_amd.util.seed import layer_rng

KIND_A2C, KIND_PPO = 0, 1


def _glorot_uniform(shape):
    receptive = int(np.prod(shape[2:]))
    fan_in, fan_out = shape[1] * receptive, shape[0] * receptive
    a = np.sqrt(6. / (fan_in + fan_out))
    return layer_rng().uniform(low=-a, high=a, size=shape).astype(np.float32)


def _norm_c(shape, std):
    out = np.random.randn(*shape).astype(np.float32)
    out *= std / np.sqrt(np.square(out).sum(axis=0, keepdims=True))
    return out
# ... 187 lines not shown
    def _scaled(self, obs_u8, idx=None, tag=""):
        if self._u8:
            return ObsRows(obs_u8, idx)
        return self._scaled_f32(obs_u8, idx, tag)

    def _scaled_f32(self, obs_u8, idx=None, tag=""):
        b = obs_u8.shape[0] if idx is None else idx.shape[0]
        c, h, w = self._obs_shape
        if c == 4:
            out = self._buffer(("x" + tag, b), (b, c, h, w), channels_last=True)
            _lib.gather_scale_obs_nhwc(obs_u8, idx, out, self._scale)
            return out
        tmp = self._buffer(("x_nchw" + tag, b), (b, c, h, w))
        _lib.gather_scale_obs(obs_u8, idx, tmp, self._scale)
        out = self._buffer(("x" + tag, b), (b, self._c_pad, h, w), channels_last=True)
        if self._c_pad != c:
            out.zero_()
        out[:, :c].copy_(tmp)
        return out

    def _layer_geoms(self, b):
        key = (b, _lib.default_route)
        gs = self._geoms.get(key)
        if gs is None:
            c, h, w = self._obs_shape
            conv = []
            for nf, ci, sz, st, pad, ho, wo in self._conv_geom:
                conv.append(_lib.conv_geom(b, h, w, ci, nf, sz, sz, st, pad[0], pad[1]))
                h, w = ho, wo
            dense = [_lib.dense_geom(b, fan_in, hs) for hs, fan_in in self._hid_geom]
            gs = self._geoms[key] = (conv, dense)
        return gs

    def _trunk(self, x, w=None, tag=""):
        b = x.shape[0]
        w = self._w if w is None else w
        conv_g, dense_g = self._layer_geoms(b)
        acts, a = [], x
        for i, (nf, ci, sz, st, pad, ho, wo) in enumerate(self._conv_geom):
            z = self._buffer(("act" + tag, i, b), (b, ho, wo, nf))
            if isinstance(a, ObsRows):
                _lib.conv2d_u8_fwd(a.obs, a.idx, self._scale, w[0], w[1], z, conv_g[0], True)
            else:
                _lib.conv2d_fwd(a, w[2 * i], w[2 * i + 1], z, conv_g[i], True, self._conv_ws)
            acts.append(z)
            a = z
        hids, k = [], 2 * self._n_conv
        for j, (hs, fan_in) in enumerate(self._hid_geom):
            hcur = self._buffer(("hid" + tag, j, b), (b, hs))
            _lib.conv2d_fwd(a, w[k], w[k + 1], hcur, dense_g[j], True, self._conv_ws)
            hids.append(hcur)
            a = hcur
            k += 2
        return acts, hids

    def prob_value(self, observations, rows=None):
        with torch.no_grad():
            x = self._scaled(observations, rows)
            b = x.shape[0]
            _, hids = self._trunk(x)
            prob = torch.empty((b, self.n_act), dtype=torch.float32, device=self.device)
            value = torch.empty(b, dtype=torch.float32, device=self.device)
            _lib.pg_head_infer(hids[-1], self.params[-2], self.params[-1], prob, value)
            return prob, value

    def serve_supported(self):
        return (type(self).prob_value is AtariCnnPolicy.prob_value and self._n_hid >= 1 and
                self._hid_geom[-1][0] <= 1024 and self.n_act <= _lib.MAX_ACTIONS)

    def serve_conv1(self, game, b):
        conv_g, _ = self._layer_geoms(b)
        if not (self._u8 and _lib.serve_conv1_supported(game, conv_g[0])):
            return None, None
        nf, ci, sz, st, pad, ho, wo = self._conv_geom[0]
        y1 = self._buffer(("act", 0, b), (b, ho, wo, nf))
        conv1 = _lib.ArlServeConv1()
        conv1.geom = C.pointer(conv_g[0])
# ... 22 lines not shown
                a = z
            k = 2 * self._n_conv
            for j, (hs, fan_in) in enumerate(self._hid_geom):
                hcur = self._buffer(("hid", j, b), (b, hs))
                if j + 1 < self._n_hid:
                    _lib.conv2d_fwd(a, w[k], w[k + 1], hcur, dense_g[j], True, self._conv_ws)
                else:
                    item = _lib.conv2d_fwd_parts(a, w[k], w[k + 1], hcur, dense_g[j], True, self._conv_ws)
                a = hcur
                k += 2
            head = _lib.ArlServeHead()
            head.hidden = item
            head.hidden_bias, head.hidden_relu, head.hid = w[k - 1].data_ptr(), 1, self._hid_geom[-1][0]
            head.w_head, head.b_head = w[self._k_head].data_ptr(), w[self._k_head + 1].data_ptr()
            conv1 = None
            if want_next and self._u8 and _lib.serve_conv1_supported(game, conv_g[0]):
                conv1 = _lib.ArlServeConv1()
                conv1.geom = C.pointer(conv_g[0])
                conv1.w, conv1.bias, conv1.y = w[0].data_ptr(), w[1].data_ptr(), y1.data_ptr()
                conv1.scale, conv1.relu = self._scale, 1
            return head, conv1, (y1 if conv1 is not None else None)

    def loss_and_grads(self, mb, kind, clip_param, v_loss_coeff, ent_loss_coeff, lr_mult,
                       inv_count=None, tie_rule=_lib.PPO_TIE_THEANO):
        with torch.no_grad():
            idx = mb.get("idx")
            rows = mb["observations"].shape[0] if idx is None else idx.shape[0]
            limit = self.rows_per_pass()
            if limit and rows >= 3 * limit:
                return self._loss_and_grads_in_passes(mb, rows, limit, kind, clip_param, v_loss_coeff, ent_loss_coeff,
                                                      lr_mult, inv_count, tie_rule)
            x = self._scaled(mb["observations"], idx)
            b = x.shape[0]
            acts, hids = self._trunk(x)
            g, k_head = self.grads, self._k_head
            hid = self._hid_geom[-1][0]
            dout = self._buffer(("dout", b), (b, self.n_act + 1))
            dh = self._buffer(("dh", b), (b, hid))
            loss4 = self._buffer(("loss", b), (4,))
            wts = self._dgrad_weight_items(b) if os.environ.get("ARL_WT_IN_HEAD", "1") != "0" else []
            self._folds.pg_head_loss(hids[-1], self.params[k_head], self.params[k_head + 1], mb["actions"],
                              mb["advantages"], mb["returns"], mb.get("old_prob"), mb.get("valids"),
                              idx, lr_mult, inv_count, self.n_act, kind, clip_param, v_loss_coeff,
                              ent_loss_coeff, dout, dh, g[k_head], g[k_head + 1], loss4, self._loss_ws,
                              relu_mask_dh=True, tie_rule=tie_rule, dgrad_weights=wts)
            self._wt_fresh = bool(wts)
            try:
                self._backward_trunk(x, acts, hids, dh, masked=True, split_hook=mb.get("split_hook"),
                                     dense_w_hook=mb.get("dense_w_hook"))
            finally:
                self._wt_fresh = False
            return loss4

    max_rows_per_pass = None
    CACHE_BYTES = 256 << 20

    def rows_per_pass(self):
        if not isinstance(self.max_rows_per_pass, str):
            return self.max_rows_per_pass
        per_row = int(np.prod(self._obs_shape)) + 8 * sum(nf * ho * wo for nf, ci, sz, st, pad, ho, wo in self._conv_geom)
        return max(256, (self.CACHE_BYTES // per_row + 128) // 256 * 256)

    def _loss_and_grads_in_passes(self, mb, rows, limit, kind, clip_param, v_loss_coeff, ent_loss_coeff, lr_mult,
                                  inv_count, tie_rule=_lib.PPO_TIE_THEANO):
        idx = mb.get("idx")
        if idx is None:
            idx = self._buffer(("all_rows", rows), (rows,), dtype=torch.int32)
            idx.copy_(torch.arange(rows, dtype=torch.int32, device=self.device))
        if inv_count is None:
            inv_count = self._buffer(("inv_rows", rows), (1,))
            inv_count.fill_(1.0 / rows)
        if not getattr(self, "_passes_logged", False):
            self._passes_logged = True
            from accel_rl_amd.util import logger
            logger.log("AtariCnnPolicy: minibatches of %d rows are walked in passes of %d (gradients accumulated in a fixed "
                       "order; max_rows_per_pass = None keeps one pass)" % (rows, limit))
        acc = self._buffer(("grad_acc",), tuple(self.flat_grads.shape))
        loss_acc = self._buffer(("loss_acc",), (4,))
        one = dict((k, v) for k, v in mb.items() if k not in ("split_hook", "dense_w_hook"))
        saved, self.max_rows_per_pass = self.max_rows_per_pass, None
        try:
            for k, lo in enumerate(range(0, rows, limit)):
                one["idx"] = idx[lo:min(lo + limit, rows)]
                loss4 = self.loss_and_grads(one, kind, clip_param, v_loss_coeff, ent_loss_coeff, lr_mult, inv_count,
# ... 38 lines not shown

    def _backward_convs(self, x, acts, d_act, masked=False, corun=None):
        b = x.shape[0]
        conv_g, _ = self._layer_geoms(b)
        if not getattr(self, "_wt_fresh", False):
            items = self._dgrad_weight_items(b)
            if items:
                _lib.conv2d_dgrad_weights(items)
        group = os.environ.get("ARL_WGRAD_GROUP", "1") != "0"
        for i in range(self._n_conv - 1, -1, -1):
            nf, ci, sz, st, pad, ho, wo = self._conv_geom[i]
            d_in = self._buffer(("dx_conv", i, b), tuple(acts[i - 1].shape)) if i > 0 else None
            self._layer_grads(d_act, masked, acts[i], b * ho * wo, nf, 2 * i, conv_g[i], acts[i - 1] if i > 0 else x, d_in,
                              corun=corun if i > 0 else None,
                              wt=self._wt.get(i) if _lib.default_route != _lib.ROUTE_FP32 else None, defer=group)
            if corun is not None and i > 0 and self._folds.corun_taken:
                corun = None
            d_act, masked = d_in, True
        self._folds.run_wgrads()
        if corun is not None:
            _lib.corun_job_run(corun)
        self._folds.run()

    def _layer_grads(self, d, masked, y, rows, channels, k, geom, inp, d_in, corun=None, wt=None, defer=False):
        folds, g = self._folds, self.grads
        if not masked:
            folds.relu_bwd_bias_grad(d, y, rows, channels, g[k + 1], self._fold_ws(("db", k)))
        dbias = g[k + 1] if masked else None
        if isinstance(inp, ObsRows):
            done = folds.conv2d_u8_bwd_weight(d, inp.obs, inp.idx, self._scale, self._g[k], geom,
                                              self._fold_ws(("dw", k)), dbias=dbias, defer=defer)
        elif d_in is not None:
            done = folds.conv2d_bwd_pair(d, self._w[k], inp, d_in, inp, self._g[k], geom, self._fold_ws(("dw", k)),
                                         dbias=dbias, corun=corun, wt=wt, defer=defer)
        else:
            done = folds.conv2d_bwd_weight(d, inp, self._g[k], geom, self._fold_ws(("dw", k)), dbias=dbias, defer=defer)
        if not done:
            folds.relu_bwd_bias_grad(d, y, rows, channels, g[k + 1], self._fold_ws(("db", k)))

    def _fold_ws(self, key):
        ws = self._fold_workspaces.get(key)
        if ws is None:
            ws = self._fold_workspaces[key] = (_lib.relu_bwd_workspace(self.device) if key[0] == "db"
                                               else _lib.conv_workspace(self.device))
        return ws

    def dist_info(self, observations, state_infos=None):
        return dict(prob=self.prob_value(observations)[0])

    def value(self, observations, state_infos=None):
        return self.prob_value(observations)[1]

    def dist_info_value(self, observations, state_infos=None):
        prob, value = self.prob_value(observations)
        return dict(prob=prob, value=value)

    def _sample(self, prob):
        b = prob.shape[0]
        u = torch.from_numpy(np.random.rand(b)).to(self.device)
        acts = torch.empty(b, dtype=torch.uint8, device=self.device)
        _lib.sample_categorical(prob.contiguous(), u, acts)
        return acts

    def get_actions(self, observations):
        prob, value = self.prob_value(observations)
        return self._sample(prob), dict(prob=prob, value=value)

# ... 66 lines not shown
```

### include/accel_rl_hip.h

```cpp
#ifndef ACCEL_RL_HIP_H
#define ACCEL_RL_HIP_H

#include <stdint.h>

#ifdef __cplusplus
extern "C" {
#endif

#define ARL_ABI_VERSION 4

#define ARL_E_ARG      (-1)
#define ARL_E_RANGE    (-2)
#define ARL_E_ALIGN    (-3)

#define ARL_PROMO_NEP50   0
#define ARL_PROMO_LEGACY  1
#define ARL_PROMO_ASSOC   2

int         arl_abi_version(void);
const char* arl_last_error(void);


int arl_gae_scan(const float* rewards, const float* values, const uint8_t* dones,
                 const float* last_values, double discount, double gae_lambda,
// ... 244 lines not shown

int arl_conv2d_bwd_pair(const float* dy, const float* w, const float* wt_or_null, const float* mask_or_null, float* dx,
                        const float* x, float* dw, const arl_conv_geom* geom, void* workspace,
                        int64_t workspace_bytes, arl_fold_item* item, float* dbias_or_null,
                        arl_fold_item* bias_item_or_null, const struct arl_corun_job* job_or_null,
                        int32_t* job_taken_or_null, void* stream);

int arl_conv2d_u8_fwd(const uint8_t* obs, int64_t obs_rows, const int32_t* idx_or_null, float scale,
                      const float* w, const float* bias_or_null, float* y, const arl_conv_geom* geom,
                      int32_t relu, void* stream);
int arl_conv2d_u8_bwd_weight_parts(const float* dy, const uint8_t* obs, int64_t obs_rows,
                                   const int32_t* idx_or_null, float scale, float* dw,
                                   const arl_conv_geom* geom, void* workspace, int64_t workspace_bytes,
                                   arl_fold_item* item, float* dbias_or_null,
                                   arl_fold_item* bias_item_or_null, void* stream);

#define ARL_WGRAD_GROUP_MAX 4
typedef struct arl_wgrad_plan { int64_t opaque[32]; } arl_wgrad_plan;
int arl_conv2d_bwd_weight_plan(const float* dy, const float* x, float* dw, const arl_conv_geom* geom,
                               void* workspace, int64_t workspace_bytes, arl_fold_item* item,
                               float* dbias_or_null, arl_fold_item* bias_item_or_null, arl_wgrad_plan* plan);
int arl_conv2d_u8_bwd_weight_plan(const float* dy, const uint8_t* obs, int64_t obs_rows,
                                  const int32_t* idx_or_null, float scale, float* dw,
                                  const arl_conv_geom* geom, void* workspace, int64_t workspace_bytes,
                                  arl_fold_item* item, float* dbias_or_null,
                                  arl_fold_item* bias_item_or_null, arl_wgrad_plan* plan);
int arl_conv2d_bwd_pair_plan(const float* dy, const float* w, const float* wt_or_null, const float* mask_or_null,
                             float* dx, const float* x, float* dw, const arl_conv_geom* geom, void* workspace,
                             int64_t workspace_bytes, arl_fold_item* item, float* dbias_or_null,
                             arl_fold_item* bias_item_or_null, const struct arl_corun_job* job_or_null,
                             int32_t* job_taken_or_null, arl_wgrad_plan* plan, void* stream);
int arl_conv2d_bwd_weight_group(const arl_wgrad_plan* plans, int32_t n, void* stream);


#define ARL_REPLAY_MAX_HORIZON 16

typedef struct arl_replay {
    int64_t  n_env;
    int32_t  size;
    int32_t  n_stack;
    int32_t  frame_bytes;
    int32_t  reward_horizon;
    uint8_t* frames;
    uint8_t* n_blanks;
    uint8_t* acts;
    uint8_t* terminals;
    float*   rewards;
    float*   returns;
} arl_replay;

int arl_replay_append(const arl_replay* rb, const uint8_t* observations, const uint8_t* actions,
                      const float* rewards, const uint8_t* dones, int32_t horizon, int32_t idx,
                      double discount, int32_t promo, void* stream);

int arl_replay_extract(const arl_replay* rb, const int32_t* env_idxs, const int32_t* step_idxs,
                       int64_t batch, uint8_t* obs, uint8_t* next_obs, uint8_t* actions,
                       float* returns, uint8_t* terminals, void* stream);

int arl_sumtree_find(const double* tree, int32_t levels, const double* uniforms, int64_t n,
                     int32_t* tree_idxs, void* stream);
int arl_sumtree_add(double* tree, int32_t levels, const int32_t* tree_idxs, const double* diffs,
                    int64_t n, void* stream);
int arl_sumtree_gather(const double* tree, const int32_t* tree_idxs, int64_t n, double scale,
                       double* out, void* stream);

int arl_sumtree_sample(const double* tree, int32_t levels, const double* uniforms, int32_t m, int32_t n,
// ... 260 lines not shown
```

Before: 385,900 env-steps/s.

## Pack ReLU masks into bitfields in conv forward and consume them in backward-data

The conv forward epilogues (MFMA implicit-GEMM and the image conv1 kernel) now also emit a 1-bit-per-element positivity mask packed via ballot/permlane swaps. The backward data and pair kernels read this bitmask instead of re-reading the full fp32 activation to gate the ReLU gradient. This cuts mask read bandwidth by 32x in backward, at the cost of extra stores and bit logic in the forward epilogue, more template instantiations, and new source files. It is enabled by default through ARL_RELU_BITS.

```diff
diff --git a/accel_rl_amd/_build.py b/accel_rl_amd/_build.py
--- a/accel_rl_amd/_build.py
+++ b/accel_rl_amd/_build.py
@@ -7,7 +7,7 @@
 CSRC = os.path.join(PKG_DIR, "csrc")
 LIB_PATH = os.path.join(PKG_DIR, "libaccel_rl_hip.so")
 SOURCES = ["mfma_conv_p1.hip", "mfma_conv_p2.hip", "mfma_conv_p3.hip", "mfma_conv_p4.hip", "mfma_conv_p5.hip", "mfma_conv_p6.hip",
-           "mfma_conv_p7.hip", "mfma_conv_p8.hip", "mfma_conv.hip", "img_conv.hip", "batch_ops.hip", "scan.hip", "env.hip", "serve_step.hip", "optim.hip", "learner.hip", "replay.hip",
+           "mfma_conv_p7.hip", "mfma_conv_p8.hip", "mfma_conv_p9.hip", "mfma_conv_p10.hip", "mfma_conv.hip", "img_conv.hip", "batch_ops.hip", "scan.hip", "env.hip", "serve_step.hip", "optim.hip", "learner.hip", "replay.hip",
            "dqn.hip", "lstm.hip", "gru.hip", "noisy.hip", "traj.hip", "handover.hip", "iqn.hip"]
 ARCH = "gfx950"
 
diff --git a/accel_rl_amd/_lib.py b/accel_rl_amd/_lib.py
--- a/accel_rl_amd/_lib.py
+++ b/accel_rl_amd/_lib.py
@@ -188,6 +188,17 @@
                                         C.POINTER(ArlFoldItem), _vp, C.POINTER(ArlFoldItem), C.POINTER(ArlCorunJob),
                                         C.POINTER(_i32), C.POINTER(ArlWgradPlan), _vp]),
     "arl_conv2d_bwd_weight_group": (_i32, [C.POINTER(ArlWgradPlan), _i32, _vp]),
+    "arl_relu_bits_pack": (_i32, [_vp, _i64, _i32, _vp, _vp]),
+    "arl_conv2d_fwd_bits": (_i32, [_vp, _vp, _vp, _vp, C.POINTER(ArlConvGeom), _i32, _vp, _vp, _vp]),
+    "arl_conv2d_u8_fwd_bits": (_i32, [_vp, _i64, _vp, _f32, _vp, _vp, _vp, C.POINTER(ArlConvGeom), _i32, _vp, _vp]),
+    "arl_conv2d_bwd_data_bits": (_i32, [_vp, _vp, _vp, _vp, _vp, _vp, C.POINTER(ArlConvGeom), C.POINTER(ArlCorunJob),
+                                        C.POINTER(_i32), _vp]),
+    "arl_conv2d_bwd_pair_bits": (_i32, [_vp, _vp, _vp, _vp, _vp, _vp, _vp, _vp, C.POINTER(ArlConvGeom), _vp, _i64,
+                                        C.POINTER(ArlFoldItem), _vp, C.POINTER(ArlFoldItem), C.POINTER(ArlCorunJob),
+                                        C.POINTER(_i32), _vp]),
+    "arl_conv2d_bwd_pair_plan_bits": (_i32, [_vp, _vp, _vp, _vp, _vp, _vp, _vp, _vp, C.POINTER(ArlConvGeom), _vp, _i64,
+                                             C.POINTER(ArlFoldItem), _vp, C.POINTER(ArlFoldItem),
+                                             C.POINTER(ArlCorunJob), C.POINTER(_i32), C.POINTER(ArlWgradPlan), _vp]),
     "arl_relu_bwd_bias_parts": (_i32, [_vp, _vp, _i64, _i32, _vp, _vp, C.POINTER(ArlFoldItem), _vp]),
     "arl_replay_append": (_i32, [C.POINTER(ArlReplay), _vp, _vp, _vp, _vp, _i32, _i32, _f64, _i32, _vp]),
     "arl_replay_extract": (_i32, [C.POINTER(ArlReplay), _vp, _vp, _i64, _vp, _vp, _vp, _vp, _vp, _vp]),
@@ -636,13 +647,36 @@
     return torch.empty(load().arl_conv_workspace_bytes() // 4, dtype=torch.float32, device=device)
 
 
-def conv2d_fwd(x, w, bias, y, geom, relu, workspace, stream=None):
+def relu_bits_enabled():
+    return os.environ.get("ARL_RELU_BITS", "1") != "0"
+
+
+def _want_bits(bits, numel, name):
+    if bits.dtype != torch.int32:
+        raise TypeError("%s must be torch.int32 words, got %s" % (name, bits.dtype))
+    assert numel % 32 == 0 and bits.is_contiguous() and bits.numel() == numel // 32, "%s size" % name
+
+
+def relu_bits_pack(y, rows, n, bits, stream=None):
+    _want(y, torch.float32, "y")
+    assert y.is_contiguous() and y.numel() == rows * n, "y size"
+    _want_bits(bits, rows * n, "bits")
+    _check(load().arl_relu_bits_pack(y.data_ptr(), rows, n, bits.data_ptr(), stream_ptr(stream)), "arl_relu_bits_pack")
+
+
+def conv2d_fwd(x, w, bias, y, geom, relu, workspace, stream=None, bits=None):
     for t, n in ((x, "x"), (w, "w"), (y, "y")):
         _want(t, torch.float32, n)
     ho, wo = conv_out_hw(geom)
     assert x.numel() == geom.batch * geom.in_h * geom.in_w * geom.in_c, "x size"
     assert w.numel() == geom.out_c * geom.kh * geom.kw * geom.in_c, "w size"
     assert y.numel() == geom.batch * ho * wo * geom.out_c, "y size"
+    if bits is not None:
+        _want_bits(bits, y.numel(), "bits")
+        _check(load().arl_conv2d_fwd_bits(x.data_ptr(), w.data_ptr(), None if bias is None else bias.data_ptr(),
+                                          y.data_ptr(), C.byref(geom), int(bool(relu)), ptr(workspace), bits.data_ptr(),
+                                          stream_ptr(stream)), "arl_conv2d_fwd_bits")
+        return
     _check(load().arl_conv2d_fwd(x.data_ptr(), w.data_ptr(), None if bias is None else bias.data_ptr(),
                                  y.data_ptr(), C.byref(geom), int(bool(relu)), ptr(workspace),
                                  stream_ptr(stream)), "arl_conv2d_fwd")
@@ -677,11 +711,17 @@
         assert obs.shape[0] == geom.batch, "obs rows"
 
 
-def conv2d_u8_fwd(obs, idx, scale, w, bias, y, geom, relu, stream=None):
+def conv2d_u8_fwd(obs, idx, scale, w, bias, y, geom, relu, stream=None, bits=None):
     _u8_rows(obs, idx, geom)
     ho, wo = conv_out_hw(geom)
     assert w.numel() == geom.out_c * geom.kh * geom.kw * geom.in_c, "w size"
     assert y.numel() == geom.batch * ho * wo * geom.out_c, "y size"
+    if bits is not None:
+        _want_bits(bits, y.numel(), "bits")
+        _check(load().arl_conv2d_u8_fwd_bits(obs.data_ptr(), obs.shape[0], ptr(idx), float(scale), w.data_ptr(), ptr(bias),
+                                             y.data_ptr(), C.byref(geom), int(bool(relu)), bits.data_ptr(),
+                                             stream_ptr(stream)), "arl_conv2d_u8_fwd_bits")
+        return
     _check(load().arl_conv2d_u8_fwd(obs.data_ptr(), obs.shape[0], ptr(idx), float(scale), w.data_ptr(), ptr(bias),
                                     y.data_ptr(), C.byref(geom), int(bool(relu)), stream_ptr(stream)),
            "arl_conv2d_u8_fwd")
@@ -698,12 +738,18 @@
     _check(load().arl_conv2d_dgrad_weights(items, len(layers), stream_ptr(stream)), "arl_conv2d_dgrad_weights")
 
 
-def conv2d_bwd_data(dy, w, mask, dx, geom, stream=None, corun=None, wt=None):
+def conv2d_bwd_data(dy, w, mask, dx, geom, stream=None, corun=None, wt=None, mask_bits=None):
     ho, wo = conv_out_hw(geom)
     assert dy.numel() == geom.batch * ho * wo * geom.out_c, "dy size"
     assert dx.numel() == geom.batch * geom.in_h * geom.in_w * geom.in_c, "dx size"
     assert mask is None or mask.numel() == dx.numel()
     taken = _i32(0)
+    if mask_bits is not None:
+        _want_bits(mask_bits, dx.numel() if geom.in_c % 32 == 0 else 32 * mask_bits.numel(), "mask_bits")
+        _check(load().arl_conv2d_bwd_data_bits(dy.data_ptr(), w.data_ptr(), ptr(wt), ptr(mask), mask_bits.data_ptr(),
+                                               dx.data_ptr(), C.byref(geom), None if corun is None else C.byref(corun),
+                                               C.byref(taken), stream_ptr(stream)), "arl_conv2d_bwd_data_bits")
+        return bool(taken.value)
     _check(load().arl_conv2d_bwd_data(dy.data_ptr(), w.data_ptr(), ptr(wt), None if mask is None else mask.data_ptr(),
                                       dx.data_ptr(), C.byref(geom), None if corun is None else C.byref(corun),
                                       C.byref(taken), stream_ptr(stream)), "arl_conv2d_bwd_data")
@@ -795,7 +841,7 @@
         return self._bias_done(dbias)
 
     def conv2d_bwd_pair(self, dy, w, mask, dx, x, dw, geom, workspace, dbias=None, stream=None, corun=None, wt=None,
-                        defer=False):
+                        defer=False, mask_bits=None):
         ho, wo = conv_out_hw(geom)
         assert dy.numel() == geom.batch * ho * wo * geom.out_c, "dy size"
         assert x.numel() == dx.numel() == geom.batch * geom.in_h * geom.in_w * geom.in_c, "x / dx size"
@@ -804,7 +850,17 @@
         slot = self._n - 1
         pb, ib = self._bias_slot(dbias)
         taken = _i32(0)
-        if defer:
+        if mask_bits is not None:
+            _want_bits(mask_bits, dx.numel() if geom.in_c % 32 == 0 else 32 * mask_bits.numel(), "mask_bits")
+            args = (dy.data_ptr(), w.data_ptr(), ptr(wt), ptr(mask), mask_bits.data_ptr(), dx.data_ptr(), x.data_ptr(),
+                    dw.data_ptr(), C.byref(geom), ptr(workspace), workspace.numel() * workspace.element_size(), item, pb, ib,
+                    None if corun is None else C.byref(corun), C.byref(taken))
+            if defer:
+                _check(load().arl_conv2d_bwd_pair_plan_bits(*(args + (self._next_plan(stream), stream_ptr(stream)))),
+                       "arl_conv2d_bwd_pair_plan_bits")
+            else:
+                _check(load().arl_conv2d_bwd_pair_bits(*(args + (stream_ptr(stream),))), "arl_conv2d_bwd_pair_bits")
+        elif defer:
             _check(load().arl_conv2d_bwd_pair_plan(dy.data_ptr(), w.data_ptr(), ptr(wt), ptr(mask), dx.data_ptr(),
                                                    x.data_ptr(), dw.data_ptr(), C.byref(geom), ptr(workspace),
                                                    workspace.numel() * workspace.element_size(), item, pb, ib,
diff --git a/accel_rl_amd/csrc/img_conv.hip b/accel_rl_amd/csrc/img_conv.hip
--- a/accel_rl_amd/csrc/img_conv.hip
+++ b/accel_rl_amd/csrc/img_conv.hip
@@ -59,14 +59,15 @@
 
 int launch_conv1_img(const unsigned char* obs, int64_t obs_rows, const int32_t* idx, float scale, const float* w, const float* bias, float* y,
                      int64_t batch, int C, int H, int W, int K, int kh, int kw, int stride, int Ho, int Wo, int relu,
-                     hipStream_t s, unsigned char* copy_out, long long copy_stride, int* zero_word) {
+                     hipStream_t s, unsigned char* copy_out, long long copy_stride, int* zero_word, uint32_t* bits_out) {
     const int npix = C * H * W;
     const size_t lds = (size_t)(C * 64 / 16) * 3072 + 2 * (size_t)npix;
     if (g_no_img_kernels || !t_ctx.split || t_ctx.split == 1 || (K != 32 && K != 16) || kh != 8 || kw != 8 || npix % 16 != 0 || npix > C1_MAX_IMG ||
         lds > 160 * 1024 || ((uintptr_t)obs & 15) || (W & 3) || (stride & 3) || batch > 0x7fffffff)
         return -1;
     Conv1ImgArgs a = {obs, idx, w, bias, y, scale, (int)batch, C, H, W, Ho, Wo, stride, relu, K,
-                      (int)(obs_rows < 0x7fffffff ? obs_rows : 0x7fffffff), copy_out, copy_stride, zero_word};
+                      (int)(obs_rows < 0x7fffffff ? obs_rows : 0x7fffffff), copy_out, copy_stride, zero_word,
+                      K == 32 ? bits_out : nullptr, (unsigned)(batch * Ho * Wo * 4)};
     {
         hipError_t e = hipFuncSetAttribute(reinterpret_cast<const void*>(conv1_img_kernel),
                                            hipFuncAttributeMaxDynamicSharedMemorySize, 160 * 1024);
diff --git a/accel_rl_amd/csrc/img_conv_dev.h b/accel_rl_amd/csrc/img_conv_dev.h
--- a/accel_rl_amd/csrc/img_conv_dev.h
+++ b/accel_rl_amd/csrc/img_conv_dev.h
@@ -16,6 +16,8 @@
     unsigned char* copy_out;
     long long copy_stride;
     int* zero_word;
+    unsigned* bits;
+    unsigned bits_bytes;
 };
 
 __device__ __forceinline__ u32x2 bytes_to_bf16x4(unsigned v) {
@@ -81,6 +83,7 @@
     }
     if (m < rows) {
         float* dst = a.y + ((size_t)img * rows + m) * N + 4 * half;
+        unsigned bw = 0u;
 #pragma unroll
         for (int q = 0; q < 4; ++q) {
             if (8 * q + 4 * half >= N) continue;
@@ -88,6 +91,12 @@
                                    acc[4 * q + 2] * a.scale + bq[q].z, acc[4 * q + 3] * a.scale + bq[q].w);
             if (a.relu) { v.x = fmaxf(v.x, 0.f); v.y = fmaxf(v.y, 0.f); v.z = fmaxf(v.z, 0.f); v.w = fmaxf(v.w, 0.f); }
             *reinterpret_cast<float4*>(dst + 8 * q) = v;
+            if (a.bits) bw |= pos_bits(v, 8 * q + 4 * half);
+        }
+        if (a.bits) {
+            const unsigned word = or_halves(bw);
+            const __amdgpu_buffer_rsrc_t rb = make_rsrc(reinterpret_cast<const float*>(a.bits), a.bits_bytes);
+            __builtin_amdgcn_raw_buffer_store_b32(word, rb, half == 0 ? (unsigned)(img * rows + m) << 2 : OOB, 0, 0);
         }
     }
 }
diff --git a/accel_rl_amd/csrc/mfma_common.h b/accel_rl_amd/csrc/mfma_common.h
--- a/accel_rl_amd/csrc/mfma_common.h
+++ b/accel_rl_amd/csrc/mfma_common.h
@@ -43,6 +43,9 @@
     unsigned out_bytes;
     int relu, dense;
     int OH, OW, omul, oadd_y, oadd_x;
+    const unsigned* mask_bits;
+    unsigned* bits_out;
+    unsigned bits_bytes;
 };
 
 struct GemmArgs {
@@ -141,14 +144,28 @@
     else split_pair(x0, x1, h, m, l);
 }
 
-template <int TM, int TN, bool SCALED = false>
+constexpr int ARL_BITS_OUT = 1, ARL_BITS_MASK = 2;
+__device__ __forceinline__ unsigned or_halves(unsigned x) {
+    const auto r = __builtin_amdgcn_permlane32_swap(x, x, false, false);
+    return r[0] | r[1];
+}
+__device__ __forceinline__ float keep_if(unsigned w, int bit, float v) { return ((w >> bit) & 1u) ? v : 0.f; }
+__device__ __forceinline__ unsigned pos_bits(const float4& v, int at) {
+    return ((v.x > 0.f ? 1u : 0u) | (v.y > 0.f ? 2u : 0u) | (v.z > 0.f ? 4u : 0u) | (v.w > 0.f ? 8u : 0u)) << at;
+}
+template <int TM, int TN, bool SCALED = false, int BITS = 0>
 __device__ __forceinline__ void store_tiles_quads(const f32x16 (&acc)[TM][TN], __amdgpu_buffer_rsrc_t rs,
                                                   const long long (&row_off)[TM], int N, int col_base, int lane,
                                                   const float4 (&bias_q)[TN][4], const float* mask, int relu,
-                                                  const float4 (*pre)[TM] = nullptr, float scale = 1.f) {
+                                                  const float4 (*pre)[TM] = nullptr, float scale = 1.f,
+                                                  const unsigned (*mbits)[TN] = nullptr, bool use_bits = false,
+                                                  unsigned* bits_out = nullptr, unsigned bits_bytes = 0) {
     const int half = lane >> 5;
 #pragma unroll
     for (int j = 0; j < TN; ++j) {
+        unsigned bw[TM];
+#pragma unroll
+        for (int i = 0; i < TM; ++i) bw[i] = 0u;
         float4 mk[4][TM];
         if (mask && pre) {
 #pragma unroll
@@ -179,15 +196,32 @@
                                   acc[i][j][4 * q + 2] + bq.z, acc[i][j][4 * q + 3] + bq.w);
                 if (relu) { val.x = fmaxf(val.x, 0.f); val.y = fmaxf(val.y, 0.f); val.z = fmaxf(val.z, 0.f); val.w = fmaxf(val.w, 0.f); }
                 const unsigned voff = ok ? (unsigned)((row_off[i] + n) << 2) : OOB;
-                if (mask) {
+                if (BITS == ARL_BITS_MASK && use_bits) {
+                    const unsigned wv = mbits[i][j] >> (4 * half);
+                    val.x = keep_if(wv, 8 * q, val.x);
+                    val.y = keep_if(wv, 8 * q + 1, val.y);
+                    val.z = keep_if(wv, 8 * q + 2, val.z);
+                    val.w = keep_if(wv, 8 * q + 3, val.w);
+                } else if (mask) {
                     const float4 m = mk[q][i];
                     if (!(m.x > 0.f)) val.x = 0.f;
                     if (!(m.y > 0.f)) val.y = 0.f;
                     if (!(m.z > 0.f)) val.z = 0.f;
                     if (!(m.w > 0.f)) val.w = 0.f;
                 }
+                if (BITS == ARL_BITS_OUT && bits_out) bw[i] |= pos_bits(val, 8 * q + 4 * half);
                 u32x4 raw = {__float_as_uint(val.x), __float_as_uint(val.y), __float_as_uint(val.z), __float_as_uint(val.w)};
                 __builtin_amdgcn_raw_buffer_store_b128(raw, rs, voff, 0, 0);
+            }
+        }
+        if (BITS == ARL_BITS_OUT && bits_out) {
+            const __amdgpu_buffer_rsrc_t rb = make_rsrc(reinterpret_cast<const float*>(bits_out), bits_bytes);
+            const int n = col_base + j * 32;
+#pragma unroll
+            for (int i = 0; i < TM; ++i) {
+                const unsigned word = or_halves(bw[i]);
+                const bool ok = row_off[i] >= 0 && n < N && half == 0;
+                __builtin_amdgcn_raw_buffer_store_b32(word, rb, ok ? (unsigned)((row_off[i] + n) >> 5) << 2 : OOB, 0, 0);
             }
         }
     }
diff --git a/accel_rl_amd/csrc/mfma_conv.hip b/accel_rl_amd/csrc/mfma_conv.hip
--- a/accel_rl_amd/csrc/mfma_conv.hip
+++ b/accel_rl_amd/csrc/mfma_conv.hip
@@ -104,6 +104,21 @@
     }
 }
 
+__global__ __launch_bounds__(256) void relu_bits_pack_kernel(const float* __restrict__ y, int64_t total,
+                                                             unsigned* __restrict__ bits) {
+    const int64_t i = (int64_t)blockIdx.x * 256 + threadIdx.x;
+    const float v = i < total ? y[i] : 0.f;
+    const unsigned long long b = __ballot(v > 0.f);
+    const int64_t e0 = i & ~(int64_t)63;
+    if ((threadIdx.x & 63) == 0 && e0 < total) bits[e0 >> 5] = (unsigned)b;
+    if ((threadIdx.x & 63) == 32 && e0 + 32 < total) bits[(e0 >> 5) + 1] = (unsigned)(b >> 32);
+}
+
+int launch_pack(const float* y, int64_t total, uint32_t* bits, hipStream_t s) {
+    hipLaunchKernelGGL(relu_bits_pack_kernel, dim3((unsigned)((total + 255) / 256)), dim3(256), 0, s, y, total, bits);
+    return arl::check_launch("relu_bits_pack_kernel");
+}
+
 int launch_fold(const float* part, int splits, int64_t total, const float* bias, int n_bias, int relu,
                 float* out, hipStream_t s, const float* mask = nullptr) {
     const int64_t total4 = total >> 2;
@@ -148,11 +163,14 @@
 
 namespace {
 int fwd_impl(const float* x, const float* w, const float* bias_or_null, float* y, const arl_conv_geom* geom, int32_t relu,
-             void* workspace, void* stream, arl_fold_item* parts = nullptr) {
+             void* workspace, void* stream, arl_fold_item* parts = nullptr, uint32_t* bits_out = nullptr) {
     Geom g;
     int rc = check_geom(geom, &g);
     if (rc) return rc;
     ARL_REQUIRE(x && w && y && workspace, ARL_E_ARG, "null pointer");
+    ARL_REQUIRE(!bits_out || (g.K % 32 == 0 && ((uintptr_t)bits_out & 3) == 0), ARL_E_RANGE,
+                "packed rectifier bits: out_c % 32 == 0, 4-byte aligned");
+    bool emitted = false;
     ARL_REQUIRE(arl::aligned16(x) && arl::aligned16(w) && arl::aligned16(y) && arl::aligned16(workspace) &&
                     (!bias_or_null || arl::aligned16(bias_or_null)), ARL_E_ALIGN, "16-byte alignment");
     hipStream_t s = (hipStream_t)stream;
@@ -193,14 +211,18 @@
         a.g.rmin = (a.g.add_y * g.W + a.g.add_x) * g.C;
         a.g.origin = a.g.rmin + a.g.dmin;
         a.g.src_bytes = (unsigned)(g.batch * g.H * g.W * g.C * 4 - (int64_t)a.g.origin * 4);
+        if (bits_out && g_split && splits == 1 && !multi_tap && a.N > 16 && a.N <= 64 && !(a.N > 32 && g_fwd_tile == 2)) {
+            a.o.bits_out = bits_out; a.o.bits_bytes = (unsigned)((int64_t)a.M * a.N / 8);
+            emitted = true;
+        }
         if (a.N <= 16 && a.K % 16 == 0 && per % 16 == 0 && (g.C % 16 == 0 || (16 % g.C == 0 && g.kw % (16 / g.C) == 0)))
             rc = launch_igemm<4, 1, 2, 1, 16, true, true>(a, splits, multi_tap, has_pad, s);
-        else if (g_split && a.N <= 32) rc = launch_igemm_split<4, 1, 1, 1, FBK, true, false, 2>(a, multi_tap, has_pad, s, splits);
+        else if (g_split && a.N <= 32) rc = launch_row_tiles<1, true>(a, multi_tap, has_pad, s, splits);
         else if (g_split && a.N <= 64) {
             const int v = (g_fwd_tile >= 0 && g_fwd_tile <= 2) ? g_fwd_tile : (2 * ((a.M + 127) / 128) <= TARGET_WGS ? 1 : 0);
-            if (v == 1) rc = launch_igemm_split<4, 1, 1, 1, FBK, true, false, 2>(a, multi_tap, has_pad, s, splits);
+            if (v == 1) rc = launch_row_tiles<1, true>(a, multi_tap, has_pad, s, splits);
             else if (v == 2) rc = launch_igemm_split<2, 2, 1, 1, FBK, true, false, 3>(a, multi_tap, has_pad, s, splits);
-            else rc = launch_igemm_split<4, 1, 1, 2, FBK, true, false, 2>(a, multi_tap, has_pad, s, splits);
+            else rc = launch_row_tiles<2, true>(a, multi_tap, has_pad, s, splits);
         }
         else if (g_split && (small || fill64)) rc = launch_igemm_split<2, 2, 1, 1, FBK, true, false, 3>(a, multi_tap, has_pad, s, splits);
         else if (g_split) rc = launch_igemm_split<2, 2, 2, 2, FBK, true, false, 1>(a, multi_tap, has_pad, s, splits);
@@ -223,8 +245,9 @@
         parts->splits = splits == 1 ? 0 : splits; parts->valid = 0;
         return rc;
     }
-    if (rc || splits == 1) return rc;
-    return launch_fold((const float*)workspace, splits, (int64_t)a.M * a.N, bias_or_null, a.N, relu, y, s);
+    if (!rc && splits > 1) rc = launch_fold((const float*)workspace, splits, (int64_t)a.M * a.N, bias_or_null, a.N, relu, y, s);
+    if (!rc && bits_out && !emitted) rc = launch_pack(y, (int64_t)a.M * a.N, bits_out, s);
+    return rc;
 }
 }
 
@@ -246,14 +269,39 @@
     return fwd_impl(x, w, bias_or_null, y, geom, relu, workspace, stream);
 }
 
+extern "C" int arl_conv2d_fwd_bits(const float* x, const float* w, const float* bias_or_null, float* y,
+                                   const arl_conv_geom* geom, int32_t relu, void* workspace, uint32_t* bits_out_or_null,
+                                   void* stream) {
+    ARL_ROUTE_SCOPE(geom, nullptr);
+    return fwd_impl(x, w, bias_or_null, y, geom, relu, workspace, stream, nullptr, bits_out_or_null);
+}
+
+extern "C" int arl_relu_bits_pack(const float* y, int64_t rows, int32_t n, uint32_t* bits, void* stream) {
+    ARL_REQUIRE(y && bits, ARL_E_ARG, "null pointer");
+    ARL_REQUIRE(rows > 0 && n > 0 && n % 32 == 0 && rows * (int64_t)n < ((int64_t)1 << 31) && ((uintptr_t)y & 3) == 0 &&
+                    ((uintptr_t)bits & 3) == 0, ARL_E_RANGE, "packed rectifier bits: n % 32 == 0, rows * n < 2^31");
+    return launch_pack(y, rows * (int64_t)n, bits, (hipStream_t)stream);
+}
+
 namespace {
 int dgrad_impl(const float* dy, const float* w, const float* mask_or_null, float* dx, const arl_conv_geom* geom,
                DgradPlan* plan_only, void* stream, void* workspace = nullptr, int64_t workspace_bytes = 0,
-               const float* wt = nullptr) {
+               const float* wt = nullptr, const uint32_t* mask_bits = nullptr) {
     Geom g;
     int rc = check_geom(geom, &g);
     if (rc) return rc;
     ARL_REQUIRE(dy && w && dx, ARL_E_ARG, "null pointer");
+    ARL_REQUIRE(((uintptr_t)mask_bits & 3) == 0, ARL_E_ALIGN, "4-byte alignment");
+    auto pick_mask = [&](GemmArgs& a, bool can) {
+        if (mask_bits && can && g.C % 32 == 0) {
+            a.o.mask_bits = mask_bits; a.o.mask = nullptr;
+            a.o.bits_bytes = (unsigned)(g.batch * g.H * g.W * g.C / 8);
+        } else if (mask_bits && !mask_or_null) {
+            arl::set_error("packed rectifier bits: this launch reads the fp32 mask (in_c %% 32, tile shape or split fold)");
+            return ARL_E_RANGE;
+        }
+        return 0;
+    };
     ARL_REQUIRE(g.kh % g.stride == 0 && g.kw % g.stride == 0, ARL_E_RANGE,
                 "data gradient needs kernel size divisible by stride");
     ARL_REQUIRE(arl::aligned16(dy) && arl::aligned16(w) && arl::aligned16(dx) &&
@@ -310,8 +358,9 @@
         }
         const bool small = st == 1 && a.N > 64 && (int64_t)a.M * a.N <= ((int64_t)1 << 20) && a.N % 4 == 0;
         if (plan_only) {
+            plan_only->cfg = a.N <= 32 ? 0 : a.N <= 64 ? 1 : small ? 3 : 2;
+            if (plan_only->cfg == 2 && (rc = pick_mask(a, g_split != 0))) return rc;
             plan_only->a = a; plan_only->fast = true; plan_only->has_pad = has_pad;
-            plan_only->cfg = a.N <= 32 ? 0 : a.N <= 64 ? 1 : small ? 3 : 2;
             return 0;
         }
         if (small) {
@@ -319,6 +368,7 @@
             if (workspace) plan_split(((a.M + 63) / 64) * ((a.N + 63) / 64), a.K, &splits, &per, 3 * TARGET_WGS);
             if ((int64_t)splits * a.M * a.N * 4 > workspace_bytes) { splits = 1; per = round_up(a.K, BKT); }
             a.k_per_split = per;
+            if ((rc = pick_mask(a, false))) return rc;
             if (splits > 1) {
                 a.o.out = (float*)workspace; a.o.mask = nullptr; a.split_stride = (int64_t)a.M * a.N;
             }
@@ -328,20 +378,22 @@
             return launch_fold((const float*)workspace, splits, (int64_t)a.M * a.N, nullptr, 4, 0, dx, s, mask_or_null);
         }
         if (wt && g_split && a.N > 16 && a.N <= 64 && g_dgrad_wt) {
+            if ((rc = pick_mask(a, true))) return rc;
             a.b.w = wt; a.b.ld = a.K; a.b.cls = a.N * a.K;
             const int tiles = ((a.M + 127) / 128) * (a.n_par ? a.n_par : 1);
             const int v = a.N <= 32 || ((g_fwd_tile >= 0 && g_fwd_tile <= 2) ? (g_fwd_tile == 1) : (2 * tiles <= TARGET_WGS));
-            if (v) rc = launch_igemm_split<4, 1, 1, 1, FBK, true, false, 2>(a, false, has_pad, s);
-            else rc = launch_igemm_split<4, 1, 1, 2, FBK, true, false, 2>(a, false, has_pad, s);
+            if (v) rc = launch_row_tiles<1, true>(a, false, has_pad, s);
+            else rc = launch_row_tiles<2, true>(a, false, has_pad, s);
             return rc;
         }
+        if ((rc = pick_mask(a, g_split && a.N > 16 && a.N <= 64))) return rc;
         if (a.N <= 16) rc = launch_igemm<4, 1, 2, 1, 16, false, true>(a, 1, false, has_pad, s);
-        else if (g_split && a.N <= 32) rc = launch_igemm_split<4, 1, 1, 1, FBK, false, false, 2>(a, false, has_pad, s);
+        else if (g_split && a.N <= 32) rc = launch_row_tiles<1, false>(a, false, has_pad, s);
         else if (g_split && a.N <= 64) {
             const int tiles = ((a.M + 127) / 128) * (a.n_par ? a.n_par : 1);
             const int v = (g_fwd_tile >= 0 && g_fwd_tile <= 2) ? (g_fwd_tile == 1) : (2 * tiles <= TARGET_WGS);
-            if (v) rc = launch_igemm_split<4, 1, 1, 1, FBK, false, false, 2>(a, false, has_pad, s);
-            else rc = launch_igemm_split<4, 1, 1, 2, FBK, false, false, 2>(a, false, has_pad, s);
+            if (v) rc = launch_row_tiles<1, false>(a, false, has_pad, s);
+            else rc = launch_row_tiles<2, false>(a, false, has_pad, s);
         }
         else if (g_split) rc = launch_igemm_split<2, 2, 2, 2, FBK, false, false, 1>(a, false, has_pad, s);
         else if (a.N <= 32 && a.N > 16) rc = launch_igemm_occ<2, 2, 2, 1, 32, false, true, 5>(a, false, has_pad, s);
@@ -351,6 +403,10 @@
         return rc;
     }
     if (plan_only) { plan_only->fast = false; return 0; }
+    {
+        GemmArgs none = {};
+        if ((rc = pick_mask(none, false))) return rc;
+    }
     for (int ph = 0; ph < st && ph < g.H; ++ph) {
         for (int pw = 0; pw < st && pw < g.W; ++pw) {
             const GemmArgs a = describe(ph, pw);
@@ -470,6 +526,15 @@
     return rc;
 }
 
+extern "C" int arl_conv2d_bwd_data_bits(const float* dy, const float* w, const float* wt_or_null, const float* mask_or_null,
+                                        const uint32_t* mask_bits_or_null, float* dx, const arl_conv_geom* geom,
+                                        const arl_corun_job* job_or_null, int32_t* job_taken_or_null, void* stream) {
+    ARL_ROUTE_SCOPE(geom, job_or_null);
+    const int rc = dgrad_impl(dy, w, mask_or_null, dx, geom, nullptr, stream, nullptr, 0, wt_or_null, mask_bits_or_null);
+    if (job_taken_or_null) *job_taken_or_null = t_ctx.corun_taken ? 1 : 0;
+    return rc;
+}
+
 extern "C" int arl_conv2d_bwd_weight(const float* dy, const float* x, float* dw, const arl_conv_geom* geom,
                                      void* workspace, void* stream) {
     ARL_ROUTE_SCOPE(geom, nullptr);
@@ -554,9 +619,35 @@
 }
 }
 
+namespace {
+int u8_fwd_launch(const uint8_t* obs, int64_t obs_rows, const int32_t* idx_or_null, float scale, const float* w,
+                  const float* bias_or_null, float* y, const arl_conv_geom* geom, int32_t relu, void* stream,
+                  uint32_t* bits_out, bool* emitted);
+}
+
 extern "C" int arl_conv2d_u8_fwd(const uint8_t* obs, int64_t obs_rows, const int32_t* idx_or_null, float scale,
                                  const float* w, const float* bias_or_null, float* y, const arl_conv_geom* geom,
                                  int32_t relu, void* stream) {
+    bool emitted = false;
+    return u8_fwd_launch(obs, obs_rows, idx_or_null, scale, w, bias_or_null, y, geom, relu, stream, nullptr, &emitted);
+}
+
+extern "C" int arl_conv2d_u8_fwd_bits(const uint8_t* obs, int64_t obs_rows, const int32_t* idx_or_null, float scale,
+                                      const float* w, const float* bias_or_null, float* y, const arl_conv_geom* geom,
+                                      int32_t relu, uint32_t* bits_out_or_null, void* stream) {
+    ARL_REQUIRE(!bits_out_or_null || (geom && geom->out_c % 32 == 0 && ((uintptr_t)bits_out_or_null & 3) == 0), ARL_E_RANGE,
+                "packed rectifier bits: out_c % 32 == 0, 4-byte aligned");
+    bool emitted = false;
+    int rc = u8_fwd_launch(obs, obs_rows, idx_or_null, scale, w, bias_or_null, y, geom, relu, stream, bits_out_or_null, &emitted);
+    if (rc || !bits_out_or_null || emitted) return rc;
+    const int64_t ho = (geom->in_h - geom->kh) / geom->stride + 1, wo = (geom->in_w - geom->kw) / geom->stride + 1;
+    return launch_pack(y, geom->batch * ho * wo * geom->out_c, bits_out_or_null, (hipStream_t)stream);
+}
+
+namespace {
+int u8_fwd_launch(const uint8_t* obs, int64_t obs_rows, const int32_t* idx_or_null, float scale, const float* w,
+                  const float* bias_or_null, float* y, const arl_conv_geom* geom, int32_t relu, void* stream,
+                  uint32_t* bits_out, bool* emitted) {
     ARL_REQUIRE(w && y, ARL_E_ARG, "null pointer");
     U8Geom g;
     int rc = check_u8(obs, obs_rows, geom, &g);
@@ -566,8 +657,8 @@
                 "16-byte alignment");
     if (!g_trace) {
         rc = launch_conv1_img(obs, obs_rows, idx_or_null, scale, w, bias_or_null, y, g.batch, g.C, g.H, g.W, g.K, g.kh, g.kw, g.stride,
-                              g.Ho, g.Wo, relu, (hipStream_t)stream);
-        if (rc >= 0) return rc;
+                              g.Ho, g.Wo, relu, (hipStream_t)stream, nullptr, 0, nullptr, bits_out);
+        if (rc >= 0) { *emitted = bits_out != nullptr; return rc; }
     }
     GemmArgs a = {};
     fill_u8(&a.g, obs, obs_rows, idx_or_null, scale, g);
@@ -598,6 +689,7 @@
         hipLaunchKernelGGL((igemm_u8_kernel<4, 1, 1, 1, BK, false>), grid, dim3(256), lds, (hipStream_t)stream, a);
     }
     return arl::check_launch("igemm_u8_kernel");
+}
 }
 
 namespace {
@@ -668,7 +760,7 @@
 int pair_impl(const float* dy, const float* w, const float* wt_or_null, const float* mask_or_null, float* dx, const float* x,
               float* dw, const arl_conv_geom* geom, void* workspace, int64_t workspace_bytes, arl_fold_item* item,
               float* dbias_or_null, arl_fold_item* bias_item_or_null, const arl_corun_job* job_or_null,
-              int32_t* job_taken_or_null, WgradPlan* defer, void* stream) {
+              int32_t* job_taken_or_null, WgradPlan* defer, void* stream, const uint32_t* mask_bits = nullptr) {
     ARL_REQUIRE(item && geom && (!dbias_or_null || bias_item_or_null), ARL_E_ARG, "null pointer");
     if (job_taken_or_null) *job_taken_or_null = 0;
     ARL_ROUTE_SCOPE(geom, job_or_null);
@@ -678,7 +770,7 @@
     int splits = 1;
     int64_t total = 0;
     float* bias_part = nullptr;
-    int rc = dgrad_impl(dy, w, mask_or_null, dx, geom, &dp, stream);
+    int rc = dgrad_impl(dy, w, mask_or_null, dx, geom, &dp, stream, nullptr, 0, nullptr, mask_bits);
     if (rc) return rc;
     rc = wgrad_impl(dy, x, dw, geom, workspace, workspace_bytes, &splits, &total,
                     dbias_or_null ? &bias_part : nullptr, &wp, stream);
@@ -690,13 +782,14 @@
     if (!paired) {
         const int64_t half = (workspace_bytes / 2) & ~(int64_t)15;
         rc = dgrad_impl(dy, w, mask_or_null, dx, geom, nullptr, stream, (char*)workspace + half, workspace_bytes - half,
-                        wt_or_null);
+                        wt_or_null, mask_bits);
         if (job_taken_or_null) *job_taken_or_null = t_ctx.corun_taken ? 1 : 0;
         if (rc) return rc;
         return wgrad_parts_impl(dy, x, dw, geom, workspace, half, item, dbias_or_null, bias_item_or_null, stream, defer);
     }
     hipStream_t s = (hipStream_t)stream;
-    if (g_split) rc = launch_pair<2, 2, 2, 2, 2, 2, 2, 2, 16>(dp, wp, has_pad, s);
+    if (g_split && dp.a.o.mask_bits) rc = launch_pair<2, 2, 2, 2, 2, 2, 2, 2, 16, ARL_BITS_MASK>(dp, wp, has_pad, s);
+    else if (g_split) rc = launch_pair<2, 2, 2, 2, 2, 2, 2, 2, 16>(dp, wp, has_pad, s);
     else rc = launch_pair<2, 2, 2, 2, 2, 2, 2, 2>(dp, wp, has_pad, s);
     item->part = (const float*)workspace; item->out = dw; item->total = wp.total;
     item->splits = wp.splits > 1 ? wp.splits : 0;
@@ -724,6 +817,28 @@
     *plan = arl_wgrad_plan{};
     return pair_impl(dy, w, wt_or_null, mask_or_null, dx, x, dw, geom, workspace, workspace_bytes, item, dbias_or_null,
                      bias_item_or_null, job_or_null, job_taken_or_null, reinterpret_cast<WgradPlan*>(plan), stream);
+}
+
+extern "C" int arl_conv2d_bwd_pair_bits(const float* dy, const float* w, const float* wt_or_null, const float* mask_or_null,
+                                        const uint32_t* mask_bits_or_null, float* dx, const float* x, float* dw,
+                                        const arl_conv_geom* geom, void* workspace, int64_t workspace_bytes,
+                                        arl_fold_item* item, float* dbias_or_null, arl_fold_item* bias_item_or_null,
+                                        const arl_corun_job* job_or_null, int32_t* job_taken_or_null, void* stream) {
+    return pair_impl(dy, w, wt_or_null, mask_or_null, dx, x, dw, geom, workspace, workspace_bytes, item, dbias_or_null,
+                     bias_item_or_null, job_or_null, job_taken_or_null, nullptr, stream, mask_bits_or_null);
+}
+
+extern "C" int arl_conv2d_bwd_pair_plan_bits(const float* dy, const float* w, const float* wt_or_null,
+                                             const float* mask_or_null, const uint32_t* mask_bits_or_null, float* dx,
+                                             const float* x, float* dw, const arl_conv_geom* geom, void* workspace,
+                                             int64_t workspace_bytes, arl_fold_item* item, float* dbias_or_null,
+                                             arl_fold_item* bias_item_or_null, const arl_corun_job* job_or_null,
+                                             int32_t* job_taken_or_null, arl_wgrad_plan* plan, void* stream) {
+    ARL_REQUIRE(plan, ARL_E_ARG, "null pointer");
+    *plan = arl_wgrad_plan{};
+    return pair_impl(dy, w, wt_or_null, mask_or_null, dx, x, dw, geom, workspace, workspace_bytes, item, dbias_or_null,
+                     bias_item_or_null, job_or_null, job_taken_or_null, reinterpret_cast<WgradPlan*>(plan), stream,
+                     mask_bits_or_null);
 }
 
 extern "C" int arl_conv2d_bwd_weight_group(const arl_wgrad_plan* plans, int32_t n, void* stream) {
diff --git a/accel_rl_amd/csrc/mfma_conv_p10.hip b/accel_rl_amd/csrc/mfma_conv_p10.hip
--- /dev/null
+++ b/accel_rl_amd/csrc/mfma_conv_p10.hip
@@ -0,0 +1,2 @@
+#define ARL_CONV_PART 10
+#include "mfma_conv_impl.h"
diff --git a/accel_rl_amd/csrc/mfma_conv_p9.hip b/accel_rl_amd/csrc/mfma_conv_p9.hip
--- /dev/null
+++ b/accel_rl_amd/csrc/mfma_conv_p9.hip
@@ -0,0 +1,2 @@
+#define ARL_CONV_PART 9
+#include "mfma_conv_impl.h"
diff --git a/accel_rl_amd/csrc/mfma_dispatch.h b/accel_rl_amd/csrc/mfma_dispatch.h
--- a/accel_rl_amd/csrc/mfma_dispatch.h
+++ b/accel_rl_amd/csrc/mfma_dispatch.h
@@ -116,7 +116,7 @@
 #define ARL_BY_MODE(X1, X6, X9) do { if (g_split == 1) { X1; } else if (g_split == 6) { X6; } else { X9; } } while (0)
 #endif
 
-template <int WGM, int WGN, int TM, int TN, int BK, bool B_KC, bool U8, int MINW>
+template <int WGM, int WGN, int TM, int TN, int BK, bool B_KC, bool U8, int MINW, int BITS = 0>
 int launch_igemm_split(const GemmArgs& a, bool multi_tap, bool has_pad, hipStream_t s, int splits = 1) {
     constexpr int BM = WGM * TM * 32, BN = WGN * TN * 32;
     const int npl = planes_of(g_split);
@@ -128,7 +128,7 @@
     int rc = 0;
 #define ARL_SPLIT_K(MT, HP, SPL, CO, AD)                                                                   \
     do {                                                                                                   \
-        auto k = igemm_split_kernel<WGM, WGN, TM, TN, BK, B_KC, MT, HP, U8, SPL, MINW, CO, AD>;            \
+        auto k = igemm_split_kernel<WGM, WGN, TM, TN, BK, B_KC, MT, HP, U8, SPL, MINW, CO, AD, BITS>;      \
         const size_t lds_k = (AD) ? lds_dir : lds;                                                         \
         rc = allow_big_lds(k, lds_k + (CO ? 64 : 0));                                                      \
         if (!rc) hipLaunchKernelGGL(k, grid, dim3(256), lds_k, s, a, c);                                   \
@@ -145,16 +145,22 @@
     if constexpr (U8) {
         ARL_SPLIT_MODE(false, false, false);
     } else {
-        if constexpr (!B_KC || (WGM == 4 && WGN == 1 && TM == 1)) {
+        if constexpr ((!B_KC || (WGM == 4 && WGN == 1 && TM == 1)) && BITS != ARL_BITS_OUT) {
             if (!multi_tap && corun_take(&c, &grid)) {
                 if (has_pad) ARL_SPLIT_MODE(false, true, true); else ARL_SPLIT_MODE(false, false, true);
                 return rc ? rc : arl::check_launch("igemm_split_kernel (co-run)");
             }
         }
+        if constexpr (BITS != 0) {
+            if (multi_tap) { arl::set_error("packed rectifier bits: one tap per k-tile"); return ARL_E_RANGE; }
+            if (has_pad) ARL_SPLIT_MODE(false, true, false);
+            else ARL_SPLIT_MODE(false, false, false);
+        } else {
         if (multi_tap && has_pad) ARL_SPLIT_MODE(true, true, false);
         else if (multi_tap) ARL_SPLIT_MODE(true, false, false);
         else if (has_pad) ARL_SPLIT_MODE(false, true, false);
         else ARL_SPLIT_MODE(false, false, false);
+        }
     }
 #undef ARL_SPLIT_PIN
 #undef ARL_SPLIT_MODE
@@ -265,7 +271,7 @@
 constexpr int WPLAN_F32 = 1, WPLAN_U8 = 2;
 struct WgradPlan { WgradArgs a; bool fast, has_pad; int cfg, splits; int64_t total; int kind, route; };
 
-template <int DWGM, int DWGN, int DTM, int DTN, int WWGM, int WWGN, int WTM, int WTN, int BK = 32>
+template <int DWGM, int DWGN, int DTM, int DTN, int WWGM, int WWGN, int WTM, int WTN, int BK = 32, int BITS = 0>
 int launch_pair(const DgradPlan& d, const WgradPlan& w, bool has_pad, hipStream_t s) {
     constexpr int DBM = DWGM * DTM * 32, DBN = DWGN * DTN * 32, WBM = WWGM * WTM * 32, WBN = WWGN * WTN * 32;
     const size_t lds_d = (size_t)2 * (DBM * (BK + 4) + BK * DBN) * sizeof(float);
@@ -279,13 +285,16 @@
         const size_t lds_s = (size_t)2 * planes_of(g_split) * ((DBM + DBN) > (WBM + WBN) ? (DBM + DBN) : (WBM + WBN)) * BK * 2;
 #define ARL_PSPLIT(HP, SPL)                                                                                \
     do {                                                                                                   \
-        auto k = bwd_pair_kernel<DWGM, DWGN, DTM, DTN, WWGM, WWGN, WTM, WTN, BK, HP, SPL>;                 \
+        auto k = bwd_pair_kernel<DWGM, DWGN, DTM, DTN, WWGM, WWGN, WTM, WTN, BK, HP, SPL, BITS>;           \
         rc = allow_big_lds(k, lds_s + 4096);                                                               \
         if (!rc) hipLaunchKernelGGL(k, dim3(n_ig + n_wg), dim3(256), lds_s, s, d.a, w.a, dgx, dgy, n_ig, wgx, wgy); \
     } while (0)
         if (has_pad) ARL_BY_MODE(ARL_PSPLIT(true, 1), ARL_PSPLIT(true, 6), ARL_PSPLIT(true, 9));
         else ARL_BY_MODE(ARL_PSPLIT(false, 1), ARL_PSPLIT(false, 6), ARL_PSPLIT(false, 9));
 #undef ARL_PSPLIT
+    } else if (BITS) {
+        arl::set_error("packed rectifier bits: the pair launch reads them on the bf16-split routes");
+        return ARL_E_RANGE;
     } else if (has_pad) {
         auto k = bwd_pair_kernel<DWGM, DWGN, DTM, DTN, WWGM, WWGN, WTM, WTN, BK, true>;
         rc = allow_big_lds(k, lds + 4096);
@@ -301,7 +310,8 @@
 
 int launch_conv1_img(const unsigned char* obs, int64_t obs_rows, const int32_t* idx, float scale, const float* w, const float* bias, float* y,
                      int64_t batch, int C, int H, int W, int K, int kh, int kw, int stride, int Ho, int Wo, int relu,
-                     hipStream_t s, unsigned char* copy_out = nullptr, long long copy_stride = 0, int* zero_word = nullptr);
+                     hipStream_t s, unsigned char* copy_out = nullptr, long long copy_stride = 0, int* zero_word = nullptr,
+                     uint32_t* bits_out = nullptr);
 
 #define ARL_GA const GemmArgs&, bool, bool, hipStream_t, int
 #define ARL_P1(T) \
@@ -343,6 +353,15 @@
     T int launch_wgrad_fast<2, 2, 1, 1, 32, false>(const WgradArgs&, int, bool, hipStream_t); \
     T int launch_wgrad_fast<1, 4, 1, 1, 32, false>(const WgradArgs&, int, bool, hipStream_t); \
     T int launch_wgrad_fast<1, 4, 1, 1, 32, true>(const WgradArgs&, int, bool, hipStream_t);
+#define ARL_P9(T) \
+    T int launch_igemm_split<4, 1, 1, 2, 32, true, false, 2, ARL_BITS_OUT>(ARL_GA); \
+    T int launch_igemm_split<4, 1, 1, 1, 32, true, false, 2, ARL_BITS_OUT>(ARL_GA); \
+    T int launch_pair<2, 2, 2, 2, 2, 2, 2, 2, 16, ARL_BITS_MASK>(const DgradPlan&, const WgradPlan&, bool, hipStream_t);
+#define ARL_P10(T) \
+    T int launch_igemm_split<4, 1, 1, 2, 32, true, false, 2, ARL_BITS_MASK>(ARL_GA); \
+    T int launch_igemm_split<4, 1, 1, 1, 32, true, false, 2, ARL_BITS_MASK>(ARL_GA); \
+    T int launch_igemm_split<4, 1, 1, 2, 32, false, false, 2, ARL_BITS_MASK>(ARL_GA); \
+    T int launch_igemm_split<4, 1, 1, 1, 32, false, false, 2, ARL_BITS_MASK>(ARL_GA);
 #ifndef ARL_CONV_PART
 #define ARL_CONV_PART 0
 #endif
@@ -398,5 +417,24 @@
 #else
 ARL_P7(ARL_T_EXT)
 #endif
-
-}
+#if ARL_CONV_PART == 9
+ARL_P9(ARL_T_DEF)
+#else
+ARL_P9(ARL_T_EXT)
+#endif
+#if ARL_CONV_PART == 10
+ARL_P10(ARL_T_DEF)
+#else
+ARL_P10(ARL_T_EXT)
+#endif
+
+template <int TN, bool B_KC>
+int launch_row_tiles(const GemmArgs& a, bool multi_tap, bool has_pad, hipStream_t s, int splits = 1) {
+    if constexpr (B_KC) {
+        if (a.o.bits_out) return launch_igemm_split<4, 1, 1, TN, 32, B_KC, false, 2, ARL_BITS_OUT>(a, multi_tap, has_pad, s, splits);
+    }
+    if (a.o.mask_bits) return launch_igemm_split<4, 1, 1, TN, 32, B_KC, false, 2, ARL_BITS_MASK>(a, multi_tap, has_pad, s, splits);
+    return launch_igemm_split<4, 1, 1, TN, 32, B_KC, false, 2>(a, multi_tap, has_pad, s, splits);
+}
+
+}
diff --git a/accel_rl_amd/csrc/mfma_igemm.h b/accel_rl_amd/csrc/mfma_igemm.h
--- a/accel_rl_amd/csrc/mfma_igemm.h
+++ b/accel_rl_amd/csrc/mfma_igemm.h
@@ -4,7 +4,7 @@
 namespace arlc {
 
 template <int WGM, int WGN, int TM, int TN, int BK, bool B_KC, bool MULTI_TAP, bool HAS_PAD, bool N16 = false,
-          bool U8 = false, int SPLIT = 0, bool ADIR = false>
+          bool U8 = false, int SPLIT = 0, bool ADIR = false, int BITS = 0>
 __device__ __forceinline__ void igemm_body(const GemmArgs& a, const int bx, const int by, const int bz, float* smem) {
     constexpr bool SP = SPLIT != 0;
     static_assert(!ADIR || (SP && WGN == 1 && !MULTI_TAP), "direct operand: split kernels, one wave per row tile");
@@ -13,6 +13,7 @@
     constexpr int LDA = BK + 4;
     constexpr int LDB = B_KC ? BK + 4 : (N16 ? BN + 4 : BN);
     static_assert(!N16 || (TN == 1 && BK % 16 == 0), "16-wide tiles: one column tile per wave");
+    static_assert(!BITS || !N16, "packed rectifier bits: 32-wide tiles");
     static_assert(!SP || (!N16 && BK % 16 == 0), "split products: 32-wide tiles, two LDS stages");
     constexpr int ROWS_PER_PASS = 256 / CH;
     constexpr int RA = (BM + ROWS_PER_PASS - 1) / ROWS_PER_PASS;
@@ -378,7 +379,26 @@
     constexpr bool PRE_MASK = TN == 1 && TM <= 2;
     if (PRE_MASK) decode_out_rows();
     float4 mk_pre[4][TM];
+    unsigned mb_pre[TM][TN];
+    constexpr bool PRE_BITS = !(WGN == 1 && TM * TN == 2);
+    auto load_mask_bits = [&]() {
+        {
+            const __amdgpu_buffer_rsrc_t rsM = make_rsrc(reinterpret_cast<const float*>(a.o.mask_bits), a.o.bits_bytes);
+            if (!PRE_MASK) decode_out_rows();
+#pragma unroll
+            for (int i = 0; i < TM; ++i) {
+                const unsigned bvoff = row_off[i] >= 0 ? (unsigned)((row_off[i] + n0 + wn * TN * 32) >> 5) << 2 : OOB;
+#pragma unroll
+                for (int j = 0; j < TN; ++j)
+                    mb_pre[i][j] = buf_ld1s(rsM, n0 + wn * TN * 32 + j * 32 < a.N ? bvoff + 4u * j : OOB, 0);
+            }
+        }
+    };
     auto issue_mask_loads = [&]() {
+        if (BITS == ARL_BITS_MASK && a.o.mask_bits) {
+            if (PRE_BITS) load_mask_bits();
+            return;
+        }
         if (!(PRE_MASK && a.o.mask)) return;
 #pragma unroll
         for (int q = 0; q < (N16 ? 1 : 4); ++q)
@@ -612,6 +632,14 @@
                 __builtin_amdgcn_raw_buffer_store_b128(raw, rsO, ok ? (unsigned)((row_off[i] + n) << 2) : OOB, 0, 0);
             }
         } else {
+            if constexpr (BITS == ARL_BITS_MASK && !PRE_BITS) {
+                if (a.o.mask_bits) load_mask_bits();
+            }
+            if constexpr (BITS != 0)
+                store_tiles_quads<TM, TN, U8, BITS>(acc, rsO, row_off, a.N, n0 + wn * TN * 32, lane, bias_q, a.o.mask, a.o.relu,
+                                                    PRE_MASK ? mk_pre : nullptr, g.scale, mb_pre, a.o.mask_bits != nullptr,
+                                                    a.o.bits_out, a.o.bits_bytes);
+            else
             store_tiles_quads<TM, TN, U8>(acc, rsO, row_off, a.N, n0 + wn * TN * 32, lane, bias_q, a.o.mask, a.o.relu,
                                           PRE_MASK ? mk_pre : nullptr, g.scale);
         }
@@ -638,7 +666,7 @@
 }
 
 template <int WGM, int WGN, int TM, int TN, int BK, bool B_KC, bool MULTI_TAP, bool HAS_PAD, bool U8, int SPLIT, int MINW,
-          bool CORUN = false, bool ADIR = false>
+          bool CORUN = false, bool ADIR = false, int BITS = 0>
 __global__ __launch_bounds__(256, MINW) void igemm_split_kernel(const GemmArgs a, const arl::OptSeg c) {
     extern __shared__ __attribute__((aligned(16))) float smem[];
     pin_gemm_args(a);
@@ -661,7 +689,7 @@
         const int u = t / gx;
         by = u % gy; bz = u / gy;
     }
-    igemm_body<WGM, WGN, TM, TN, BK, B_KC, MULTI_TAP, HAS_PAD, false, U8, SPLIT, ADIR>(a, bx, by, bz, smem);
+    igemm_body<WGM, WGN, TM, TN, BK, B_KC, MULTI_TAP, HAS_PAD, false, U8, SPLIT, ADIR, BITS>(a, bx, by, bz, smem);
 }
 
 template <int WGM, int WGN, int TM, int TN, int BK, bool B_KC, bool MULTI_TAP, bool HAS_PAD, bool N16, int MINW, bool CORUN = false,
diff --git a/accel_rl_amd/csrc/mfma_pair.h b/accel_rl_amd/csrc/mfma_pair.h
--- a/accel_rl_amd/csrc/mfma_pair.h
+++ b/accel_rl_amd/csrc/mfma_pair.h
@@ -4,7 +4,8 @@
 
 namespace arlc {
 
-template <int DWGM, int DWGN, int DTM, int DTN, int WWGM, int WWGN, int WTM, int WTN, int BK, bool HAS_PAD, int SPLIT = 0>
+template <int DWGM, int DWGN, int DTM, int DTN, int WWGM, int WWGN, int WTM, int WTN, int BK, bool HAS_PAD, int SPLIT = 0,
+          int BITS = 0>
 __global__ __launch_bounds__(256) void bwd_pair_kernel(const GemmArgs a, const WgradArgs w, const int dgx, const int dgy,
                                                        const int n_ig, const int wgx, const int wgy) {
     extern __shared__ __attribute__((aligned(16))) float smem[];
@@ -12,7 +13,7 @@
     if (a.xcd) id = xcd_chunk(id, (int)gridDim.x);
     if (id < n_ig) {
         const int bx = id % dgx, t = id / dgx;
-        igemm_body<DWGM, DWGN, DTM, DTN, BK, false, false, HAS_PAD, false, false, SPLIT>(a, bx, t % dgy, t / dgy, smem);
+        igemm_body<DWGM, DWGN, DTM, DTN, BK, false, false, HAS_PAD, false, false, SPLIT, false, BITS>(a, bx, t % dgy, t / dgy, smem);
     } else {
         id -= n_ig;
         if (a.xcd) {
diff --git a/accel_rl_amd/policies/atari_cnn_policy.py b/accel_rl_amd/policies/atari_cnn_policy.py
--- a/accel_rl_amd/policies/atari_cnn_policy.py
+++ b/accel_rl_amd/policies/atari_cnn_policy.py
@@ -243,17 +243,22 @@
             gs = self._geoms[key] = (conv, dense)
         return gs
 
-    def _trunk(self, x, w=None, tag=""):
+    def _trunk(self, x, w=None, tag="", relu_bits=False):
         b = x.shape[0]
         w = self._w if w is None else w
         conv_g, dense_g = self._layer_geoms(b)
         acts, a = [], x
+        self._act_bits = {}
         for i, (nf, ci, sz, st, pad, ho, wo) in enumerate(self._conv_geom):
             z = self._buffer(("act" + tag, i, b), (b, ho, wo, nf))
+            bits = None
+            if relu_bits and nf % 32 == 0:
+                bits = self._buffer(("act_bits" + tag, i, b), (b * ho * wo * nf // 32,), dtype=torch.int32)
+                self._act_bits[id(z)] = bits
             if isinstance(a, ObsRows):
-                _lib.conv2d_u8_fwd(a.obs, a.idx, self._scale, w[0], w[1], z, conv_g[0], True)
+                _lib.conv2d_u8_fwd(a.obs, a.idx, self._scale, w[0], w[1], z, conv_g[0], True, bits=bits)
             else:
-                _lib.conv2d_fwd(a, w[2 * i], w[2 * i + 1], z, conv_g[i], True, self._conv_ws)
+                _lib.conv2d_fwd(a, w[2 * i], w[2 * i + 1], z, conv_g[i], True, self._conv_ws, bits=bits)
             acts.append(z)
             a = z
         hids, k = [], 2 * self._n_conv
@@ -342,7 +347,7 @@
                                                       lr_mult, inv_count, tie_rule)
             x = self._scaled(mb["observations"], idx)
             b = x.shape[0]
-            acts, hids = self._trunk(x)
+            acts, hids = self._trunk(x, relu_bits=_lib.relu_bits_enabled())
             g, k_head = self.grads, self._k_head
             hid = self._hid_geom[-1][0]
             dout = self._buffer(("dout", b), (b, self.n_act + 1))
@@ -360,6 +365,7 @@
                                      dense_w_hook=mb.get("dense_w_hook"))
             finally:
                 self._wt_fresh = False
+                self._act_bits = {}
             return loss4
 
     max_rows_per_pass = None
@@ -464,7 +470,8 @@
                                               self._fold_ws(("dw", k)), dbias=dbias, defer=defer)
         elif d_in is not None:
             done = folds.conv2d_bwd_pair(d, self._w[k], inp, d_in, inp, self._g[k], geom, self._fold_ws(("dw", k)),
-                                         dbias=dbias, corun=corun, wt=wt, defer=defer)
+                                         dbias=dbias, corun=corun, wt=wt, defer=defer,
+                                         mask_bits=getattr(self, "_act_bits", {}).get(id(inp)))
         else:
             done = folds.conv2d_bwd_weight(d, inp, self._g[k], geom, self._fold_ws(("dw", k)), dbias=dbias, defer=defer)
         if not done:
diff --git a/include/accel_rl_hip.h b/include/accel_rl_hip.h
--- a/include/accel_rl_hip.h
+++ b/include/accel_rl_hip.h
@@ -300,6 +300,27 @@
                              int32_t* job_taken_or_null, arl_wgrad_plan* plan, void* stream);
 int arl_conv2d_bwd_weight_group(const arl_wgrad_plan* plans, int32_t n, void* stream);
 
+int arl_relu_bits_pack(const float* y, int64_t rows, int32_t n, uint32_t* bits, void* stream);
+int arl_conv2d_fwd_bits(const float* x, const float* w, const float* bias_or_null, float* y, const arl_conv_geom* geom,
+                        int32_t relu, void* workspace, uint32_t* bits_out_or_null, void* stream);
+int arl_conv2d_u8_fwd_bits(const uint8_t* obs, int64_t obs_rows, const int32_t* idx_or_null, float scale, const float* w,
+                           const float* bias_or_null, float* y, const arl_conv_geom* geom, int32_t relu,
+                           uint32_t* bits_out_or_null, void* stream);
+int arl_conv2d_bwd_data_bits(const float* dy, const float* w, const float* wt_or_null, const float* mask_or_null,
+                             const uint32_t* mask_bits_or_null, float* dx, const arl_conv_geom* geom,
+                             const struct arl_corun_job* job_or_null, int32_t* job_taken_or_null, void* stream);
+int arl_conv2d_bwd_pair_bits(const float* dy, const float* w, const float* wt_or_null, const float* mask_or_null,
+                             const uint32_t* mask_bits_or_null, float* dx, const float* x, float* dw,
+                             const arl_conv_geom* geom, void* workspace, int64_t workspace_bytes, arl_fold_item* item,
+                             float* dbias_or_null, arl_fold_item* bias_item_or_null,
+                             const struct arl_corun_job* job_or_null, int32_t* job_taken_or_null, void* stream);
+int arl_conv2d_bwd_pair_plan_bits(const float* dy, const float* w, const float* wt_or_null, const float* mask_or_null,
+                                  const uint32_t* mask_bits_or_null, float* dx, const float* x, float* dw,
+                                  const arl_conv_geom* geom, void* workspace, int64_t workspace_bytes, arl_fold_item* item,
+                                  float* dbias_or_null, arl_fold_item* bias_item_or_null,
+                                  const struct arl_corun_job* job_or_null, int32_t* job_taken_or_null,
+                                  arl_wgrad_plan* plan, void* stream);
+
 
 #define ARL_REPLAY_MAX_HORIZON 16
 
```

Result: no change. 388,300 env-steps/s (median of 6 runs) (+0.6%).
